# bystrogenomics/bystro-vcf

Hardware: AMD Instinct MI355X
Metric: variants/sec (higher is better)
Workload: dtype u8; 1 GPU; BASELINE configs[2]: 1KG-Phase3 chr1-shaped, 2504 samples, biallelic SNPs; rows_per_block=311296, resident_blocks_per_gpu=8, n_samples=2504, input=resident in HBM, blocks_in_flight=3, flags=default (--allowFilter PASS,.), class maps on

## Files before the change

### bystro-vcf_amd/__init__.py

```python
import ctypes as C
import os

import numpy as np

try:
    import torch
except ImportError:
    torch = None

_HERE = os.path.dirname(os.path.abspath(__file__))
LIB_PATH = os.environ.get("BVCF_LIB") or os.path.join(_HERE, "libbvcf.so")

if not os.path.exists(LIB_PATH):
    raise ImportError(
        "bystro-vcf_amd: %s not built (run `python -c 'import __graft_entry__ as g; g.build()'` "
        "or `make -C bystro-vcf_amd/csrc`); there is no fallback path" % LIB_PATH)

lib = C.CDLL(LIB_PATH)

ABI_VERSION = 9
DEVICE_PAD = 64
NO_CMAP = 0xFFFFFFFF

OK, E_ARG, E_HIP, E_NODEV, E_BUSY, E_EMPTY, E_TOO_BIG, E_CAPACITY, E_NOMEM, E_FATAL = 0, -1, -2, -3, -4, -5, -6, -7, -8, -9
LINE_OK, LINE_FIELDS, LINE_FILTER, LINE_NOALLELE = 0, 1, 2, 3
SITE_NAMES = ["SNP", "INS", "DEL", "MNP", "MULTIALLELIC"]
ALT_BASE, ALT_INS, ALT_DEL = 0, 1, 2
CLS_NONE, CLS_HET, CLS_HOM, CLS_MISSING = 0, 1, 2, 3
SAMPLE_STATS_COLUMNS = ["sample", "het", "hom", "missing", "transitions", "transversions", "heterozygosity", "homozygosity",
                        "missingness", "trTv"]

BENCH_EXPORTS = ["bvcf_bench_device", "bvcf_bench_device_slots", "bvcf_bench_stream_kernel"]

PLAN_EXPORTS = ["bvcf_plan_text_ranges", "bvcf_plan_bgzf_ranges", "bvcf_cut_text_range", "bvcf_find_bgzf_chain",
                "bvcf_plan_threads", "bvcf_plan_fd"]

EXPORTS = [
    "bvcf_create", "bvcf_destroy", "bvcf_last_error", "bvcf_version", "bvcf_reserve", "bvcf_set_sample_names", "bvcf_set_row_format", "bvcf_alloc_pinned", "bvcf_alloc_pinned_near", "bvcf_warmup",
    "bvcf_free_pinned", "bvcf_submit", "bvcf_submit_device", "bvcf_submit_bgzf", "bvcf_collect", "bvcf_sample_stats", "bvcf_counters", "bvcf_sum_counters",
    "bvcf_allreduce_counters", "bvcf_device_count", "bvcf_device_pci_bus_id", "bvcf_path", "bvcf_config_defaults", "bvcf_string_header", "bvcf_format_tsv", "bvcf_run_buffer", "bvcf_run_fd", "bvcf_decompress_fd", "bvcf_bgzf_inflate_device", "bvcf_bgzf_deflate_device", "bvcf_free",
    "bvcf_arrow_open", "bvcf_arrow_append", "bvcf_arrow_close",
]


class Params(C.Structure):
    _fields_ = [
        ("abi_version", C.c_uint32), ("device", C.c_int32), ("n_header_fields", C.c_uint32),
        ("eol_chars", C.c_uint32), ("eol_byte", C.c_uint8), ("want_class_maps", C.c_uint8),
        ("want_dosage", C.c_uint8), ("want_name_lists", C.c_uint8), ("allow_filter", C.c_char_p), ("exclude_filter", C.c_char_p),
        ("max_batch_bytes", C.c_uint64), ("max_lines", C.c_uint32), ("max_alleles", C.c_uint32),
        ("cmap_bytes", C.c_uint64), ("n_slots", C.c_uint32), ("path", C.c_uint32),
        ("packed_sites", C.c_uint32), ("render_sites", C.c_uint32), ("want_sample_stats", C.c_uint32),
        ("min_gq", C.c_uint32), ("min_dp", C.c_uint32),
    ]


class Config(C.Structure):
    _fields_ = [
        ("empty_field", C.c_char_p), ("field_delimiter", C.c_char_p), ("allow_filter", C.c_char_p),
        ("exclude_filter", C.c_char_p), ("keep_id", C.c_uint8), ("keep_info", C.c_uint8),
        ("keep_pos", C.c_uint8), ("keep_qual", C.c_uint8), ("normalize_header", C.c_uint8),
        ("leave_teardown_to_exit", C.c_uint8), ("reserved", C.c_uint8 * 2), ("device", C.c_int32), ("n_format_threads", C.c_uint32),
        ("max_batch_bytes", C.c_uint64), ("sample_list_path", C.c_char_p),
        ("dosage_path", C.c_char_p), ("no_out", C.c_uint8), ("out_bgzf", C.c_uint8), ("reserved3", C.c_uint8 * 2),
        ("n_devices", C.c_uint32), ("devices", C.POINTER(C.c_int32)), ("sample_stats_path", C.c_char_p),
        ("min_gq", C.c_uint32), ("min_dp", C.c_uint32),
    ]


class Result(C.Structure):
    _fields_ = [
        ("batch_seq", C.c_uint64), ("status", C.c_int32), ("n_lines", C.c_uint32), ("n_alleles", C.c_uint32),
        ("n_errs", C.c_uint32), ("n_cmap_bytes", C.c_uint64), ("cmap_stride", C.c_uint32),
        ("n_samples", C.c_uint32), ("lines", C.c_void_p), ("alleles", C.c_void_p), ("errs", C.c_void_p),
        ("cmap", C.c_void_p), ("need_lines", C.c_uint64), ("need_alleles", C.c_uint64),
        ("need_cmap_bytes", C.c_uint64), ("kernel_ms", C.c_float), ("reserved", C.c_uint32),
        ("n_lines_seen", C.c_uint64), ("dosage", C.c_void_p), ("dosage_stride", C.c_uint32), ("reserved2", C.c_uint32),
        ("name_lists", C.c_void_p), ("names", C.c_void_p), ("n_name_bytes", C.c_uint64),
        ("text", C.c_void_p), ("n_text_bytes", C.c_uint64), ("head_off", C.c_void_p),
        ("sites", C.c_void_p), ("n_full_lines", C.c_uint32), ("n_row_cuts", C.c_uint32),
        ("rows", C.c_void_p), ("n_row_bytes", C.c_uint64), ("row_cuts", C.c_void_p), ("n_ok_sites", C.c_uint64),
    ]


ROW_CUT_DTYPE = np.dtype([("line", "<u4"), ("slot", "<u4"), ("off", "<u8"), ("text_off", "<u4"), ("reserved", "<u4")])
NO_TEXT_OFF = 0xFFFFFFFF
LINE_DTYPE = np.dtype([
    ("off", "<u4"), ("len", "<u4"), ("fend", "<u4", (9,)), ("rec_first", "<u4"), ("n_rec", "<u4"),
    ("n_fields", "<u4"), ("gt_task", "<u4"), ("status", "u1"), ("site_type", "u1"), ("pad", "u1", (2,))])
ALLELE_DTYPE = np.dtype([
    ("pos", "<i8"), ("line", "<u4"), ("alt_idx", "<u4"), ("alt_off", "<u4"), ("alt_len", "<u4"), ("ac", "<u4"),
    ("an", "<u4"), ("n_het", "<u4"), ("n_hom", "<u4"), ("n_miss", "<u4"), ("cmap_off", "<u4"), ("ref", "u1"),
    ("alt_base", "u1"), ("kind", "u1"), ("site_type", "u1"), ("trtv", "u1"), ("flags", "u1"), ("pad", "u1", (2,)),
    ("gt_task", "<u4"), ("pad2", "<u4")])
ERR_DTYPE = np.dtype([("line", "<u4"), ("alt_no", "<u4"), ("code", "<u4"), ("pad", "<u4")])
SITE_DTYPE = np.dtype([("off", "<u4"), ("len", "<u4"), ("fend", "u1", (8,)), ("ref", "u1"), ("alt_base", "u1"), ("trtv", "u1"),
                       ("status", "u1"), ("full_idx", "<u4"), ("n_fields", "<u4"), ("reserved", "<u4")])
SITE_FULL = 0x80
NAMES_DTYPE = np.dtype([("off", "<u4", (3,)), ("len", "<u4", (3,))])
assert LINE_DTYPE.itemsize == 64 and ALLELE_DTYPE.itemsize == 64 and ERR_DTYPE.itemsize == 16 and SITE_DTYPE.itemsize == 32

lib.bvcf_create.argtypes = [C.POINTER(C.c_void_p), C.POINTER(Params)]
lib.bvcf_create.restype = C.c_int
lib.bvcf_destroy.argtypes = [C.c_void_p]
lib.bvcf_destroy.restype = None
lib.bvcf_last_error.argtypes = [C.c_void_p]
lib.bvcf_last_error.restype = C.c_char_p
lib.bvcf_version.restype = C.c_char_p
lib.bvcf_reserve.argtypes = [C.c_void_p, C.c_uint64, C.c_uint64, C.c_uint64]
lib.bvcf_set_sample_names.argtypes = [C.c_void_p, C.POINTER(C.c_char_p), C.POINTER(C.c_uint32), C.c_uint32, C.c_char_p]
lib.bvcf_alloc_pinned.argtypes = [C.c_size_t]
lib.bvcf_alloc_pinned.restype = C.c_void_p
lib.bvcf_free_pinned.argtypes = [C.c_void_p]
lib.bvcf_submit.argtypes = [C.c_void_p, C.c_void_p, C.c_size_t, C.c_uint64]
lib.bvcf_submit_device.argtypes = [C.c_void_p, C.c_void_p, C.c_size_t, C.c_uint64]
lib.bvcf_submit_bgzf.argtypes = [C.c_void_p, C.c_char_p, C.c_size_t, C.c_size_t, C.c_int, C.c_uint32, C.c_uint64]
lib.bvcf_collect.argtypes = [C.c_void_p, C.POINTER(Result)]
lib.bvcf_bench_device.argtypes = [C.c_void_p, C.POINTER(C.c_void_p), C.POINTER(C.c_size_t), C.c_int, C.c_int,
                                  C.POINTER(C.c_float), C.POINTER(C.c_float), C.POINTER(C.c_uint64)]
lib.bvcf_bench_device_slots.argtypes = [C.c_void_p, C.POINTER(C.c_void_p), C.POINTER(C.c_size_t), C.c_int, C.c_int,
                                        C.c_uint32, C.POINTER(C.c_float), C.POINTER(C.c_float), C.POINTER(C.c_uint64)]
lib.bvcf_counters.argtypes = [C.c_void_p, C.POINTER(C.c_uint64)]
lib.bvcf_path.argtypes = [C.c_void_p]
lib.bvcf_sum_counters.argtypes = [C.POINTER(C.c_void_p), C.c_int, C.POINTER(C.c_uint64)]
lib.bvcf_allreduce_counters.argtypes = [C.POINTER(C.c_void_p), C.c_int, C.POINTER(C.c_uint64), C.POINTER(C.c_int)]
lib.bvcf_device_count.restype = C.c_int
lib.bvcf_config_defaults.argtypes = [C.POINTER(Config)]
lib.bvcf_config_defaults.restype = None
lib.bvcf_string_header.argtypes = [C.POINTER(Config), C.c_char_p, C.c_size_t]
lib.bvcf_string_header.restype = C.c_size_t
lib.bvcf_format_tsv.argtypes = [C.POINTER(Config), C.POINTER(Result), C.c_void_p, C.POINTER(C.c_char_p),
                                C.POINTER(C.c_uint32), C.POINTER(C.c_void_p), C.POINTER(C.c_size_t),
                                C.POINTER(C.c_void_p), C.POINTER(C.c_size_t)]
lib.bvcf_run_buffer.argtypes = [C.POINTER(Config), C.c_char_p, C.c_size_t, C.POINTER(C.c_void_p),
                                C.POINTER(C.c_size_t), C.POINTER(C.c_void_p), C.POINTER(C.c_size_t),
                                C.POINTER(C.c_uint64)]
lib.bvcf_run_fd.argtypes = [C.POINTER(Config), C.c_int, C.c_int, C.c_int, C.POINTER(C.c_uint64)]
lib.bvcf_decompress_fd.argtypes = [C.c_int, C.c_int, C.c_uint32, C.c_char_p]
lib.bvcf_free.argtypes = [C.c_void_p]
lib.bvcf_free.restype = None


class RangePlan(C.Structure):
    _fields_ = [("data_off", C.c_uint64), ("range_bytes", C.c_uint64), ("spare_bytes", C.c_uint64), ("n_ranges", C.c_uint64)]


class TextCut(C.Structure):
    _fields_ = [("kind", C.c_int32), ("reserved", C.c_uint32), ("start", C.c_uint64), ("end", C.c_uint64), ("long_start", C.c_uint64)]


class ThreadBudget(C.Structure):
    _fields_ = [("readers", C.c_uint32), ("copy_threads", C.c_uint32), ("format_threads", C.c_uint32), ("busy_total", C.c_uint32)]


class PlanBlock(C.Structure):
    _fields_ = [("worker", C.c_uint32), ("piece", C.c_uint32), ("range", C.c_uint64), ("file_off", C.c_uint64),
                ("nbytes", C.c_uint64), ("own", C.c_uint64), ("first_off", C.c_uint32), ("bgzf", C.c_uint8),
                ("bgzf_flags", C.c_uint8), ("last_piece", C.c_uint8), ("reserved", C.c_uint8)]


CUT_LINES, CUT_NONE, CUT_LONG = 0, 1, 2
MODE_STREAM, MODE_TEXT_RANGES, MODE_BGZF_RANGES = 0, 1, 2
BGZF_SKIP_FIRST_LINE, BGZF_END_OF_STREAM = 1, 2
lib.bvcf_plan_text_ranges.argtypes = [C.c_uint64, C.c_uint64, C.c_uint64, C.c_uint64, C.POINTER(RangePlan)]
lib.bvcf_plan_bgzf_ranges.argtypes = [C.c_uint64, C.c_uint64, C.c_uint32, C.c_uint64, C.POINTER(RangePlan)]
lib.bvcf_cut_text_range.argtypes = [C.c_char_p, C.c_uint64, C.c_uint64, C.c_int, C.c_int, C.c_uint8, C.POINTER(TextCut)]
lib.bvcf_find_bgzf_chain.argtypes = [C.c_char_p, C.c_size_t, C.c_size_t]
lib.bvcf_find_bgzf_chain.restype = C.c_long
lib.bvcf_plan_threads.argtypes = [C.c_uint32, C.c_uint32, C.c_int, C.POINTER(ThreadBudget)]
lib.bvcf_plan_fd.argtypes = [C.c_int, C.c_int, C.c_uint32, C.c_uint64, C.c_int, C.POINTER(PlanBlock), C.c_size_t,
                             C.POINTER(C.c_size_t), C.POINTER(C.c_int), C.POINTER(RangePlan)]


def plan_fd(fd_in, n_workers, max_batch_bytes=0, device_inflate=1, fd_err=2, cap=1 << 16):
    out = (PlanBlock * cap)()
    n = C.c_size_t(0)
    mode = C.c_int(-1)
    plan = RangePlan()
    rc = lib.bvcf_plan_fd(fd_in, fd_err, n_workers, max_batch_bytes, device_inflate, out, cap, C.byref(n), C.byref(mode), C.byref(plan))
    assert n.value <= cap, "more blocks than room"
    return rc, mode.value, plan, [out[i] for i in range(n.value)]


class BvcfError(RuntimeError):
    def __init__(self, rc, msg):
        super().__init__("bvcf error %d: %s" % (rc, msg))
        self.rc = rc


def make_config(cfg=None, device=0, max_batch_bytes=0, n_format_threads=0):
    cfg = cfg or {}
    c = Config()
    lib.bvcf_config_defaults(C.byref(c))
    keep = [cfg.get("emptyField", "!").encode(), cfg.get("fieldDelimiter", ";").encode(),
            cfg.get("allow", "PASS,.").encode(), cfg.get("exclude", "").encode()]
    c.empty_field, c.field_delimiter, c.allow_filter, c.exclude_filter = keep
    c.keep_id = int(cfg.get("keepId", False))
    c.keep_info = int(cfg.get("keepInfo", False))
    c.keep_pos = int(cfg.get("keepPos", False))
    c.normalize_header = int(cfg.get("normalizeHeader", True))
    c.device = device
    c.max_batch_bytes = max_batch_bytes
    c.n_format_threads = n_format_threads
    if cfg.get("sample"):
        keep.append(cfg["sample"].encode())
        c.sample_list_path = keep[-1]
    if cfg.get("dosageOutput"):
        keep.append(str(cfg["dosageOutput"]).encode())
        c.dosage_path = keep[-1]
    c.no_out = int(cfg.get("noOut", False))
    c.out_bgzf = int(cfg.get("compressOutput", "none") == "bgzf")
    if cfg.get("devices"):
        arr = (C.c_int32 * len(cfg["devices"]))(*cfg["devices"])
        keep.append(arr)
        c.devices = arr
        c.n_devices = len(cfg["devices"])
    if cfg.get("sampleStats"):
        keep.append(str(cfg["sampleStats"]).encode())
        c.sample_stats_path = keep[-1]
    c.min_gq = int(cfg.get("minGQ", 0))
    c.min_dp = int(cfg.get("minDP", 0))
    c._keep = keep
    return c


def string_header(cfg=None):
    c = make_config(cfg)
    buf = C.create_string_buffer(512)
    n = lib.bvcf_string_header(C.byref(c), buf, len(buf))
    return buf.raw[:n].decode()


def run_buffer(vcf_bytes, cfg=None, device=0, max_batch_bytes=0, n_format_threads=0):
    c = make_config(cfg, device, max_batch_bytes, n_format_threads)
    out, log = C.c_void_p(), C.c_void_p()
    n_out, n_log, n_lines = C.c_size_t(), C.c_size_t(), C.c_uint64()
    rc = lib.bvcf_run_buffer(C.byref(c), vcf_bytes, len(vcf_bytes), C.byref(out), C.byref(n_out), C.byref(log),
                             C.byref(n_log), C.byref(n_lines))
    o = C.string_at(out, n_out.value) if out.value else b""
    e = C.string_at(log, n_log.value).decode(errors="replace") if log.value else ""
    lib.bvcf_free(out)
    lib.bvcf_free(log)
    return rc, o, e, n_lines.value


def run_fd(fd_in, fd_out, fd_err, cfg=None, device=0, max_batch_bytes=0):
    c = make_config(cfg, device, max_batch_bytes)
    n_lines = C.c_uint64()
    rc = lib.bvcf_run_fd(C.byref(c), fd_in, fd_out, fd_err, C.byref(n_lines))
    return rc, n_lines.value


def allreduce_counters(ctxs):
    arr = (C.c_void_p * len(ctxs))(*[x.h for x in ctxs])
    out = (C.c_uint64 * 8)()
    used = C.c_int(0)
    rc = lib.bvcf_allreduce_counters(arr, len(ctxs), out, C.byref(used))
    if rc:
        raise BvcfError(rc, lib.bvcf_last_error(ctxs[0].h).decode())
    return list(out), bool(used.value)


lib.bvcf_bgzf_inflate_device.argtypes = [C.c_int, C.c_char_p, C.c_size_t, C.c_void_p, C.c_size_t, C.POINTER(C.c_size_t)]


def bgzf_inflate_device(comp, cap=None, device=0):
    cap = cap if cap is not None else max(64, 66000 * (comp.count(b"\x1f\x8b\x08\x04") + 1))
    buf = C.create_string_buffer(cap)
    n = C.c_size_t()
    rc = lib.bvcf_bgzf_inflate_device(device, comp, len(comp), buf, cap, C.byref(n))
    return rc, (buf.raw[:n.value] if rc == 0 else b""), n.value


lib.bvcf_bgzf_deflate_device.argtypes = [C.c_int, C.c_char_p, C.c_size_t, C.c_int, C.c_void_p, C.c_size_t,
                                         C.POINTER(C.c_size_t)]
PIECE = 65280
BGZF_EOF = bytes.fromhex("1f8b08040000000000ff0600424302001b0003000000000000000000")


def bgzf_bound(n):
    return (n + PIECE - 1) // PIECE * 65311 + 28


def bgzf_deflate_device(data, add_eof=True, device=0):
    data = bytes(data)
    cap = bgzf_bound(len(data))
    buf = C.create_string_buffer(cap)
    n = C.c_size_t()
    rc = lib.bvcf_bgzf_deflate_device(device, data, len(data), int(bool(add_eof)), buf, cap, C.byref(n))
    if rc:
        raise BvcfError(rc, "bvcf_bgzf_deflate_device")
    return buf.raw[:n.value]


def decompress(data, n_threads=0):
    import tempfile
    with tempfile.TemporaryFile() as fi, tempfile.TemporaryFile() as fo:
        fi.write(data)
        fi.flush()
        fi.seek(0)
        kind = C.create_string_buffer(8)
        rc = lib.bvcf_decompress_fd(fi.fileno(), fo.fileno(), n_threads, kind)
        fo.seek(0)
        return rc, fo.read(), kind.value.decode()


def decompress_pipe(data, n_threads=16, piece=0, seed=0):
    import random
    import tempfile
    import threading
    r, w = os.pipe()
    rng = random.Random(seed)

    def feed():
        try:
            mv, off = memoryview(data), 0
            while off < len(mv):
                n = piece or rng.choice([1, 7, 4096, 65536, 100_000, 1 << 20, 3 << 20])
                off += os.write(w, mv[off:off + n])
        finally:
            os.close(w)

    t = threading.Thread(target=feed)
    t.start()
    try:
        with tempfile.TemporaryFile() as fo:
            kind = C.create_string_buffer(8)
            rc = lib.bvcf_decompress_fd(r, fo.fileno(), n_threads, kind)
            fo.seek(0)
            return rc, fo.read(), kind.value.decode()
    finally:
        os.close(r)
        t.join()

# ... 91 lines not shown
        L = self.lines[i]
        n = int(L["n_rec"])
        return [] if n == 0 else [i] + [int(L["rec_first"]) + j - 1 for j in range(1, n)]

    def line_head(self, i):
        L = self.lines[i]
        if self.head_off is None:
            return self.text[int(L["off"]):int(L["off"]) + int(L["len"])]
        n = min(int(L["fend"][7]), int(L["len"]))
        return self.text[int(self.head_off[i]):int(self.head_off[i]) + n]

    def name_list(self, slot, q):
        nl = self.name_lists[slot]
        return self.names[int(nl["off"][q]):int(nl["off"][q]) + int(nl["len"][q])]

    def classes(self, allele_row):
        off = int(allele_row["cmap_off"])
        ns = self.n_samples
        if int(allele_row["flags"]) & 2:
            words = self.cmap[off:off + 64].view("<u4")
            m = np.zeros((ns + 3) // 4, dtype=np.uint8)
            for e in words[1:1 + int(words[0])]:
                m[int(e) >> 8] = int(e) & 0xFF
        else:
            m = self.cmap[off:off + (ns + 3) // 4]
        return ((m[:, None] >> np.array([0, 2, 4, 6], dtype=np.uint8)) & 3).reshape(-1)[:ns]


class Ctx:

    def __init__(self, n_header_fields, allow="PASS,.", exclude="", device=0, eol_chars=1, eol_byte=b"\n",
                 max_batch_bytes=0, max_lines=0, max_alleles=0, cmap_bytes=0, n_slots=0, want_class_maps=True,
                 path=0, want_dosage=False, sample_names=None, delimiter=";", packed_sites=False, render_sites=False,
                 empty_field="!", keep_pos=False, keep_id=False, keep_info=False, sample_stats=False,
                 min_gq=0, min_dp=0):
        p = Params()
        p.abi_version = ABI_VERSION
        p.device = device
        p.n_header_fields = n_header_fields
        p.eol_chars = eol_chars
        p.eol_byte = eol_byte[0]
        p.want_class_maps = int(want_class_maps)
        p.want_dosage = int(want_dosage)
        self._keep = [allow.encode(), exclude.encode()]
        p.allow_filter, p.exclude_filter = self._keep
        p.max_batch_bytes = max_batch_bytes
        p.max_lines = max_lines
        p.max_alleles = max_alleles
        p.cmap_bytes = cmap_bytes
        p.n_slots = n_slots
        p.path = path
        p.packed_sites = int(packed_sites or render_sites)
        p.render_sites = int(render_sites)
        p.want_name_lists = int(sample_names is not None)
        p.want_sample_stats = int(sample_stats)
        p.min_gq = min_gq
        p.min_dp = min_dp
        self.n_samples = max(n_header_fields - 9, 0)
        self.h = C.c_void_p()
        rc = lib.bvcf_create(C.byref(self.h), C.byref(p))
        if rc:
            raise BvcfError(rc, lib.bvcf_last_error(None).decode())
        if render_sites:
            lib.bvcf_set_row_format.argtypes = [C.c_void_p, C.c_char_p, C.c_int, C.c_int, C.c_int]
            self._check(lib.bvcf_set_row_format(self.h, empty_field.encode(), int(keep_pos), int(keep_id), int(keep_info)))
        if sample_names is not None:
            enc = [x.encode() if isinstance(x, str) else x for x in sample_names]
            ptrs = (C.c_char_p * max(len(enc), 1))(*enc)
            lens = (C.c_uint32 * max(len(enc), 1))(*[len(x) for x in enc])
            self._check(lib.bvcf_set_sample_names(self.h, ptrs, lens, len(enc), delimiter.encode()))

    def close(self):
        if self.h:
            lib.bvcf_destroy(self.h)
            self.h = C.c_void_p()

    def __del__(self):
        try:
            self.close()
        except Exception:
            pass

    def _check(self, rc):
        if rc:
            raise BvcfError(rc, lib.bvcf_last_error(self.h).decode())

    def submit(self, block, seq=0):
        self._blk = block
        self._check(lib.bvcf_submit(self.h, block, len(block), seq))

    def submit_bgzf(self, comp, n_own, skip_first_line, first_off=0, seq=0):
        self._blk = comp
        self._check(lib.bvcf_submit_bgzf(self.h, comp, len(comp), n_own, int(skip_first_line), first_off, seq))

    def submit_device(self, dptr, nbytes, seq=0):
        self._check(lib.bvcf_submit_device(self.h, dptr, nbytes, seq))

    def reserve(self, lines, alleles, cmap_bytes):
        self._check(lib.bvcf_reserve(self.h, lines, alleles, cmap_bytes))

    def collect(self, tsv=None):
        r = Result()
        rc = lib.bvcf_collect(self.h, C.byref(r))
        if rc == E_CAPACITY:
            raise BvcfError(rc, "capacity: need lines=%d alleles=%d cmap=%d" % (r.need_lines, r.need_alleles, r.need_cmap_bytes))
        self._check(rc)
        if tsv is None:
            return Batch(r)
        block, cfg, names = tsv
        c = cfg if isinstance(cfg, Config) else make_config(cfg)
        buf = np.frombuffer(block, dtype=np.uint8)
        enc = [x.encode() if isinstance(x, str) else x for x in (names or [])]
        ptrs = (C.c_char_p * max(len(enc), 1))(*enc)
        lens = (C.c_uint32 * max(len(enc), 1))(*[len(x) for x in enc])
        out, log = C.c_void_p(), C.c_void_p()
        n_out, n_log = C.c_size_t(), C.c_size_t()
        rc = lib.bvcf_format_tsv(C.byref(c), C.byref(r), buf.ctypes.data if len(buf) else None, ptrs, lens, C.byref(out),
                                 C.byref(n_out), C.byref(log), C.byref(n_log))
        try:
            if rc:
                raise BvcfError(rc, "bvcf_format_tsv")
            text = C.string_at(out, n_out.value) if out.value else b""
            log_text = C.string_at(log, n_log.value).decode(errors="replace") if log.value else ""
        finally:
            lib.bvcf_free(out)
            lib.bvcf_free(log)
        b = Batch(r)
        b.tsv, b.log = text, log_text
        return b

    def process(self, block):
        self.submit(block)
        return self.collect()

    def bench_device(self, dptrs, nbytes, iters, slots=0):
        n = len(dptrs)
        ptrs = (C.c_void_p * n)(*dptrs)
        sizes = (C.c_size_t * n)(*nbytes)
        chain = (C.c_float * iters)()
        scan = (C.c_float * iters)()
        counts = (C.c_uint64 * 5)()
        self._check(lib.bvcf_bench_device_slots(self.h, ptrs, sizes, n, iters, slots, chain, scan, counts))
        return list(chain), list(scan), list(counts)

    def path(self):
        return lib.bvcf_path(self.h)

    def stream_kernel(self):
        lib.bvcf_bench_stream_kernel.argtypes = [C.c_void_p]
        lib.bvcf_bench_stream_kernel.restype = C.c_int
        k = lib.bvcf_bench_stream_kernel(self.h)
        return None if k < 0 else ("k_stream_gen" if k else "k_stream")

    def sample_stats(self, reset=False):
        out = np.zeros(6 * self.n_samples, dtype=np.uint64)
        lib.bvcf_sample_stats.argtypes = [C.c_void_p, C.c_void_p, C.c_int]
        self._check(lib.bvcf_sample_stats(self.h, out.ctypes.data if self.n_samples else None, int(reset)))
        return out.reshape(6, self.n_samples).T.copy()

    def counters(self):
        out = (C.c_uint64 * 8)()
        self._check(lib.bvcf_counters(self.h, out))
        return list(out)
```

### bystro-vcf_amd/csrc/bvcf_common.hip.h

```cpp
#pragma once

#include <hip/hip_runtime.h>
#include <stdint.h>

#include "../../include/bvcf.h"

namespace bvcf_dev {


constexpr int kWave = 64;
constexpr int kWavesPerWg = 4;
constexpr int kWgThreads = kWave * kWavesPerWg;
constexpr uint32_t kChunk = 1024;
constexpr uint32_t kMaxProducerWaves = 32768;
constexpr uint32_t kScanGroup = 1024;

typedef uint32_t u32x4 __attribute__((ext_vector_type(4)));
typedef u32x4 u32x4_u __attribute__((aligned(1)));

struct FilterTable {
  uint32_t allow_nil, allow_n;
  uint32_t deny_nil, deny_n;
  uint16_t allow_off[32], allow_len[32];
  uint16_t deny_off[32], deny_len[32];
  uint8_t text[2048];
};

struct BatchCounters {
  uint32_t n_lines;
  uint32_t n_alleles;
  uint32_t n_errs;
  uint32_t n_tasks;
  uint32_t lines_seen;
  uint32_t cmap_maps;
  uint32_t pad[2];
  uint32_t n_finish;
  uint32_t n_full;
  uint32_t n_real;
  uint32_t n_other_shape;
};

struct StreamEntry {
  uint32_t ls, len;
  uint32_t ac, an, n_het, n_hom, n_miss;
  uint32_t cmap_off;
};

struct GtTask {
  uint32_t line;
  uint32_t allele;
  uint32_t s_begin;
  uint32_t cend;
  uint32_t cmap_off;
  uint32_t pad[3];
};

struct GtResult {
  uint32_t ac, an, n_het, n_hom, n_miss;
  uint32_t n_fields;
  uint32_t regular;
  uint32_t pad;
};

struct KernelArgs {
  const uint8_t *buf;
  uint32_t nbytes;
  uint32_t cap;
  uint32_t n_header;
  uint32_t n_samples;
  uint32_t eol_chars;
  uint32_t eol_byte;
  uint32_t want_cmap;
  int8_t *dosage;
  uint32_t dosage_stride;
  uint32_t cmap_stride;
  uint32_t max_lines, max_alleles, max_errs, max_tasks;
  unsigned long long max_cmap;
  const FilterTable *filters;
  uint32_t *census;
  uint32_t *group_base;
  uint32_t *run_lines;
  uint32_t prod_waves;
  uint32_t *s2_groups;
  uint32_t *s2_groups_next;
  uint32_t *line_off;
  bvcf_line *lines;
  bvcf_allele *alleles;
  bvcf_site *sites;
  bvcf_err *errs;
  uint8_t *cmap;
  GtTask *tasks;
  GtResult *results;
  BatchCounters *counters;
  uint32_t fused;
  uint32_t gen_stream;
  uint32_t wide;
  uint32_t win_bytes;
  uint32_t win_tabs_cap;
  uint32_t *win_tabs;
  uint32_t tile_bytes;
  uint32_t tile_quota;
  uint32_t n_tiles;
  StreamEntry *entries;
  uint32_t *line_len;
  uint32_t *line_cmap;
  uint16_t *head_bits;
  uint32_t *line_bits;
  uint32_t *finish_items;
  uint32_t *real_tasks;
  uint32_t s1_fmode;
  uint32_t s1_fkey[4], s1_flen[4];
};
constexpr uint32_t kHasHeadBits = 0x80000000u;
constexpr uint32_t kNotRegular = 0x40000000u;


__device__ __forceinline__ int lane_id() { return threadIdx.x & (kWave - 1); }

__device__ __forceinline__ uint32_t wave_incl_scan(uint32_t v) {
  v += (uint32_t)__builtin_amdgcn_update_dpp(0, (int)v, 0x111, 0xF, 0xF, true);
  v += (uint32_t)__builtin_amdgcn_update_dpp(0, (int)v, 0x112, 0xF, 0xF, true);
  v += (uint32_t)__builtin_amdgcn_update_dpp(0, (int)v, 0x114, 0xF, 0xF, true);
  v += (uint32_t)__builtin_amdgcn_update_dpp(0, (int)v, 0x118, 0xF, 0xF, true);
  v += (uint32_t)__builtin_amdgcn_update_dpp(0, (int)v, 0x142, 0xA, 0xF, false);
  v += (uint32_t)__builtin_amdgcn_update_dpp(0, (int)v, 0x143, 0xC, 0xF, false);
  return v;
}

__device__ __forceinline__ uint32_t wave_incl_scan_max(uint32_t v) {
  v = max(v, (uint32_t)__builtin_amdgcn_update_dpp(0, (int)v, 0x111, 0xF, 0xF, true));
  v = max(v, (uint32_t)__builtin_amdgcn_update_dpp(0, (int)v, 0x112, 0xF, 0xF, true));
  v = max(v, (uint32_t)__builtin_amdgcn_update_dpp(0, (int)v, 0x114, 0xF, 0xF, true));
  v = max(v, (uint32_t)__builtin_amdgcn_update_dpp(0, (int)v, 0x118, 0xF, 0xF, true));
  v = max(v, (uint32_t)__builtin_amdgcn_update_dpp(0, (int)v, 0x142, 0xA, 0xF, false));
  v = max(v, (uint32_t)__builtin_amdgcn_update_dpp(0, (int)v, 0x143, 0xC, 0xF, false));
  return v;
}

__device__ __forceinline__ uint32_t lane_value(uint32_t v, int src) {
  return (uint32_t)__builtin_amdgcn_readlane((int)v, src);
}

__device__ __forceinline__ uint32_t wave_sum(uint32_t v) { return lane_value(wave_incl_scan(v), kWave - 1); }

__device__ __forceinline__ void wave_sum3(uint32_t a, uint32_t b, uint32_t c, uint32_t limit, uint32_t *sa,
                                          uint32_t *sb, uint32_t *sc) {
  if (limit < 65536u) {
    const uint32_t ab = wave_sum(a | (b << 16));
    *sa = ab & 0xFFFFu;
    *sb = ab >> 16;
  } else {
    *sa = wave_sum(a);
    *sb = wave_sum(b);
  }
  *sc = wave_sum(c);
}

__device__ __forceinline__ uint32_t wave_excl_scan(uint32_t v, uint32_t *total) {
  const uint32_t inc = wave_incl_scan(v);
  *total = lane_value(inc, kWave - 1);
  return inc - v;
}

__device__ __forceinline__ uint32_t bcast0(uint32_t v) { return (uint32_t)__builtin_amdgcn_readfirstlane((int)v); }

__device__ __forceinline__ uint32_t wave_in_wg() { return bcast0(threadIdx.x >> 6); }
__device__ __forceinline__ uint32_t wave_in_grid() { return blockIdx.x * kWavesPerWg + wave_in_wg(); }

__device__ __forceinline__ u32x4 load16(const uint8_t *buf, uint32_t off, uint32_t cap) {
  u32x4 v = {0u, 0u, 0u, 0u};
  if (off + 16u <= cap) v = *reinterpret_cast<const u32x4_u *>(buf + off);
  return v;
}

__device__ __forceinline__ u32x4 ld_stream(const uint8_t *p) {
  return __builtin_nontemporal_load(reinterpret_cast<const u32x4_u *>(p));
}

__device__ __forceinline__ u32x4 realign(u32x4 v, uint32_t next0, uint32_t r) {
  const uint32_t w4 = (uint32_t)__builtin_amdgcn_update_dpp((int)next0, (int)v.x, 0x130, 0xF, 0xF, false);
  u32x4 o;
  o.x = __builtin_amdgcn_alignbyte(v.y, v.x, r);
  o.y = __builtin_amdgcn_alignbyte(v.z, v.y, r);
  o.z = __builtin_amdgcn_alignbyte(v.w, v.z, r);
  o.w = __builtin_amdgcn_alignbyte(w4, v.w, r);
  return o;
}

__device__ __forceinline__ uint32_t zero_bytes(uint32_t x) {
  uint32_t t = (x & 0x7F7F7F7Fu) + 0x7F7F7F7Fu;
  return ~(t | x | 0x7F7F7F7Fu);
}

__device__ __forceinline__ uint32_t eq_mask4(uint32_t d, uint32_t c4) {
  uint32_t z = zero_bytes(d ^ c4) >> 7;
  return ((z * 0x00204081u) >> 21) & 0xFu;
}

__device__ __forceinline__ uint32_t eq_mask16(u32x4 v, uint32_t c) {
  const uint32_t c4 = c * 0x01010101u;
  uint32_t lo = __builtin_amdgcn_udot4(zero_bytes(v.x ^ c4), 0x08040201u, 0u, false);
  lo = __builtin_amdgcn_udot4(zero_bytes(v.y ^ c4), 0x80402010u, lo, false);
  uint32_t hi = __builtin_amdgcn_udot4(zero_bytes(v.z ^ c4), 0x08040201u, 0u, false);
  hi = __builtin_amdgcn_udot4(zero_bytes(v.w ^ c4), 0x80402010u, hi, false);
  return (lo >> 7) | (hi << 1);
}

__device__ __forceinline__ uint32_t bits_until(uint32_t end, uint32_t off) {
  const uint32_t n = min(end - min(end, off), 16u);
  return (1u << n) - 1u;
}


__device__ __forceinline__ uint32_t cmap_of(const KernelArgs &a, uint32_t mi, bool want) {
  return (want && ((unsigned long long)mi + 1ull) * a.cmap_stride <= a.max_cmap) ? mi * a.cmap_stride : BVCF_NO_CMAP;
}

}
```

### bystro-vcf_amd/csrc/bvcf_core.hip

```cpp
#include "bvcf_device.hip.h"
#include "../../include/bvcf_bench.h"
#include "bvcf_bgzf.h"
#include "bvcf_bgzf_out.h"

#include <dlfcn.h>
#include <rccl/rccl.h>
#include <stdio.h>
#include <stdlib.h>
#include <string.h>

#include <algorithm>
#include <mutex>
#include <string>
#include <thread>
#include <vector>

using namespace bvcf_dev;

namespace {

struct Slot {
  hipStream_t stream = nullptr;
  bool used_gen = false;
  hipEvent_t ev_k0 = nullptr, ev_k1 = nullptr, ev_ctr = nullptr;
  hipEvent_t ev_in = nullptr, ev_scan = nullptr;
  uint8_t *d_in = nullptr;
  uint32_t *d_census = nullptr, *d_group = nullptr, *d_line_off = nullptr;
  uint32_t group_words = 0;
  uint32_t *d_s2_groups = nullptr;
  uint32_t s2_parity = 0;
  bvcf_line *d_lines = nullptr;
  bvcf_allele *d_alleles = nullptr;
  bvcf_site *d_sites = nullptr, *h_sites = nullptr;
  uint64_t hcap_recs = 0, hcap_errs = 0;
  uint8_t *d_rows = nullptr, *h_rows = nullptr;
  uint64_t cap_rows = 0;
  bvcf_row_cut *d_row_cuts = nullptr, *h_row_cuts = nullptr;
  uint32_t cap_row_cuts = 0, cap_render_groups = 0;
  uint64_t cap_host_cuts = 0;
  unsigned long long *d_rgroup_bytes = nullptr, *d_rtotals = nullptr, *h_rtotals = nullptr;
  unsigned long long *d_rgroup_ctext = nullptr;
  uint8_t *d_cut_text = nullptr;
  uint64_t cap_cut_text = 0;
  bool cut_text_on = false;
  uint32_t *d_rgroup_full = nullptr;
  bvcf_err *d_errs = nullptr;
  uint8_t *d_cmap = nullptr;
  int8_t *d_dosage = nullptr;
  GtTask *d_tasks = nullptr;
  GtResult *d_results = nullptr;
  uint32_t *d_win_tabs = nullptr;
  uint32_t win_tabs_cap = 0;
  StreamEntry *d_entries = nullptr;
  uint32_t *d_line_len = nullptr, *d_line_cmap = nullptr, *d_line_bits = nullptr, *d_finish_items = nullptr;
  uint16_t *d_head_bits = nullptr;
  bvcf_names *d_name_lists = nullptr, *h_name_lists = nullptr;
  uint32_t *d_name_tot = nullptr;
  uint8_t *d_names = nullptr;
  char *h_names = nullptr;
  unsigned long long *d_name_total = nullptr, *h_name_total = nullptr;
  uint64_t cap_names = 0;
  uint8_t *d_comp = nullptr;
  uint64_t cap_comp = 0;
  uint32_t *d_bgzf = nullptr, *h_bgzf = nullptr;
  uint64_t cap_bgzf_blocks = 0;
  uint32_t *d_cuts = nullptr, *h_cuts = nullptr;
  uint8_t *h_text = nullptr;
  uint64_t cap_h_text = 0;
  uint32_t *d_head_off = nullptr, *h_head_off = nullptr;
  uint8_t *d_heads = nullptr;
  unsigned long long *d_head_total = nullptr, *h_head_total = nullptr;
  uint64_t cap_head_lines = 0;
  bool heads = false;
  hipEvent_t ev_cut = nullptr;
  bool await_cuts = false;
  bool is_bgzf = false;
  int bgzf_rc = 0;
  const char *bgzf_err = nullptr;
  uint32_t text_start = 0, text_total = 0;
  BatchCounters *d_counters = nullptr;
  BatchCounters *h_counters = nullptr;
  bvcf_line *h_lines = nullptr;
  bvcf_allele *h_alleles = nullptr;
  bvcf_err *h_errs = nullptr;
  uint8_t *h_cmap = nullptr;
  int8_t *h_dosage = nullptr;
  uint2 *d_ss_dense = nullptr, *d_ss_sparse = nullptr;
  uint64_t cap_ss_list = 0;
  uint32_t *d_ss_ctr = nullptr, *d_ss_part = nullptr, *d_ss_sp = nullptr;
  unsigned long long *d_ss_acc = nullptr;
  uint64_t cap_lines = 0, cap_alleles = 0, cap_cmap = 0, cap_census = 0;
  bool busy = false;
  uint64_t seq = 0;
  size_t nbytes = 0;
  const uint8_t *src = nullptr;
};

}

struct bvcf_ctx {
  bvcf_params p{};
  int device = 0;
  int n_cu = 0;
  int gt_grid = 0, stream_grid = 0;
  int gt_filter_grid = 0;
  hipStream_t scan_stream = nullptr;
  uint32_t stream_lds_pad = 0;
  bool fused = false;
  bool gen_mode = false;
  uint32_t last_real = 0xFFFFFFFFu, last_finish = 0xFFFFFFFFu;
  bool shape_seen = false;
  int gen_policy = -1;
  uint32_t gen_grid = 0;
  bool wide = false;
  bool gt_filter = false;
  uint64_t avg_line_bytes = 0;
  bool names_on = false;
  uint32_t *d_name_off = nullptr;
  uint8_t *d_name_text = nullptr;
  NameTable name_table{};
  bool sites = false;
  bool sites1 = false;
  bool sites2 = false;
  bool packed = false;
  bool sites2_tile_census = true;
  uint32_t s2_groups_cap = 0;
  int sites_grid = 0, sites1_grid = 0;
  uint32_t win_bytes = 64u << 10;
  uint32_t tile_bytes = 0, tile_quota = 0;
  bool render = false, row_fmt_set = false;
  uint8_t *d_row_fmt = nullptr;
  uint32_t row_tail_len = 0, row_keep_pos = 0, row_keep_id = 0, row_keep_info = 0;
  uint32_t n_samples = 0;
  uint32_t cmap_stride = 0;
  uint32_t dosage_stride = 0;
  bool ss_on = false;
  uint32_t ss_ns_pad = 0, ss_max_runs = 0, ss_stripes = 0;
  uint64_t max_lines = 0, max_alleles = 0, max_cmap = 0;
  uint64_t need_extras = 0;
  FilterTable *d_filters = nullptr;
  uint32_t s1_fmode = 0, s1_fkey[4] = {0, 0, 0, 0}, s1_flen[4] = {0, 0, 0, 0};
  std::vector<Slot> slots;
  size_t head = 0, tail = 0, in_flight = 0;
  uint64_t totals[8] = {0, 0, 0, 0, 0, 0, 0, 0};
  std::string err;
};

namespace {

thread_local std::string g_create_err;
thread_local std::string *g_err_sink = nullptr;

constexpr uint64_t kMaxBlockBytes = 0xFFF00000ull;

#define HIP_TRY(ctx, expr)                                                               \
  do {                                                                                   \
    hipError_t e_ = (expr);                                                              \
    if (e_ != hipSuccess) {                                                              \
      *(g_err_sink ? g_err_sink : &(ctx)->err) = std::string(#expr) + ": " + hipGetErrorString(e_); \
      return BVCF_E_HIP;                                                                 \
    }                                                                                    \
  } while (0)

bool is_space(char c) { return c == ' ' || c == '\t' || c == '\n' || c == '\v' || c == '\f' || c == '\r'; }

int fill_filter(const char *text, bool star_is_nil, uint32_t *nil, uint32_t *n, uint16_t *off, uint16_t *len,
                uint8_t *pool, uint32_t *pool_used) {
  *nil = 1;
  *n = 0;
  if (!text || !*text) return 0;
  if (star_is_nil && strcmp(text, "*") == 0) return 0;
  *nil = 0;
  size_t L = strlen(text), start = 0;
  for (size_t i = 0; i <= L; i++) {
    if (i != L && text[i] != ',') continue;
    size_t a = start, e = i;
    while (a < e && is_space(text[a])) a++;
    while (e > a && is_space(text[e - 1])) e--;
    if (*n >= 32 || *pool_used + (e - a) > 2048) return -1;
    off[*n] = (uint16_t)*pool_used;
    len[*n] = (uint16_t)(e - a);
    memcpy(pool + *pool_used, text + a, e - a);
    *pool_used += (uint32_t)(e - a);
    (*n)++;
    start = i + 1;
  }
  return 0;
}

void free_slot(Slot &s) {
  if (s.stream) hipStreamSynchronize(s.stream);
  hipFree(s.d_in);
  hipFree(s.d_census);
  hipFree(s.d_group);
  hipFree(s.d_s2_groups);
  hipFree(s.d_line_off);
  hipFree(s.d_lines);
  hipFree(s.d_alleles);
  hipFree(s.d_sites);
  hipHostFree(s.h_sites);
  hipFree(s.d_rows);
  hipHostFree(s.h_rows);
  hipFree(s.d_row_cuts);
  hipHostFree(s.h_row_cuts);
  hipFree(s.d_rgroup_bytes);
  hipFree(s.d_rgroup_full);
  hipFree(s.d_rgroup_ctext);
  hipFree(s.d_cut_text);
  hipFree(s.d_rtotals);
  hipHostFree(s.h_rtotals);
  hipFree(s.d_errs);
  hipFree(s.d_cmap);
  hipFree(s.d_dosage);
  hipFree(s.d_tasks);
  hipFree(s.d_results);
  hipFree(s.d_win_tabs);
  hipFree(s.d_entries);
  hipFree(s.d_line_len);
  hipFree(s.d_line_cmap);
  hipFree(s.d_line_bits);
  hipFree(s.d_finish_items);
  hipFree(s.d_head_bits);
  hipFree(s.d_name_lists);
  hipFree(s.d_name_tot);
  hipFree(s.d_names);
  hipFree(s.d_name_total);
  hipHostFree(s.h_name_lists);
  hipHostFree(s.h_names);
  hipHostFree(s.h_name_total);
  hipFree(s.d_comp);
  hipFree(s.d_bgzf);
  hipHostFree(s.h_bgzf);
  hipFree(s.d_cuts);
  hipHostFree(s.h_cuts);
  hipHostFree(s.h_text);
  hipFree(s.d_head_off);
  hipHostFree(s.h_head_off);
  hipFree(s.d_heads);
  hipFree(s.d_head_total);
  hipHostFree(s.h_head_total);
  if (s.ev_cut) hipEventDestroy(s.ev_cut);
  hipFree(s.d_counters);
  hipHostFree(s.h_counters);
  hipHostFree(s.h_lines);
  hipHostFree(s.h_alleles);
  hipHostFree(s.h_errs);
  hipHostFree(s.h_cmap);
  hipHostFree(s.h_dosage);
  hipFree(s.d_ss_dense);
  hipFree(s.d_ss_sparse);
  hipFree(s.d_ss_ctr);
  hipFree(s.d_ss_part);
  hipFree(s.d_ss_sp);
  hipFree(s.d_ss_acc);
  if (s.ev_k0) hipEventDestroy(s.ev_k0);
  if (s.ev_k1) hipEventDestroy(s.ev_k1);
  if (s.ev_in) hipEventDestroy(s.ev_in);
  if (s.ev_scan) hipEventDestroy(s.ev_scan);
  if (s.ev_ctr) hipEventDestroy(s.ev_ctr);
  if (s.stream) hipStreamDestroy(s.stream);
  s = Slot{};
}

int alloc_name_arena(bvcf_ctx *c, Slot &s, uint64_t want_bytes) {
  if (want_bytes <= s.cap_names) return BVCF_OK;
  hipFree(s.d_names);
  hipHostFree(s.h_names);
  s.d_names = nullptr;
  s.h_names = nullptr;
  s.cap_names = 0;
  HIP_TRY(c, hipMalloc(&s.d_names, want_bytes + 64));
  HIP_TRY(c, hipHostMalloc(&s.h_names, want_bytes + 64, hipHostMallocDefault));
  s.cap_names = want_bytes;
  return BVCF_OK;
}

int alloc_names(bvcf_ctx *c, Slot &s, uint64_t want_bytes) {
  if (!c->names_on) return BVCF_OK;
  hipFree(s.d_name_lists);
  hipFree(s.d_name_tot);
  hipHostFree(s.h_name_lists);
  s.d_name_lists = nullptr;
  s.d_name_tot = nullptr;
  s.h_name_lists = nullptr;
  HIP_TRY(c, hipMalloc(&s.d_name_lists, c->max_alleles * sizeof(bvcf_names)));
  HIP_TRY(c, hipMalloc(&s.d_name_tot, (c->max_alleles + 1) * sizeof(uint32_t)));
  HIP_TRY(c, hipHostMalloc(&s.h_name_lists, c->max_alleles * sizeof(bvcf_names), hipHostMallocDefault));
  if (!s.d_name_total) {
    HIP_TRY(c, hipMalloc(&s.d_name_total, sizeof(unsigned long long)));
    HIP_TRY(c, hipHostMalloc(&s.h_name_total, sizeof(unsigned long long), hipHostMallocDefault));
  }
  return alloc_name_arena(c, s, want_bytes);
}

NameArgs make_name_args(bvcf_ctx *c, Slot &s) {
  NameArgs na{};
  na.nt = c->name_table;
  na.lists = s.d_name_lists;
  na.tot = s.d_name_tot;
  na.out = s.d_names;
  na.cap = s.cap_names;
  na.total = s.d_name_total;
  return na;
}

int alloc_results(bvcf_ctx *c, Slot &s) {
  if (s.cap_lines == c->max_lines && s.cap_alleles == c->max_alleles && s.cap_cmap == c->max_cmap) return BVCF_OK;
  hipFree(s.d_line_off);
  hipFree(s.d_lines);
  hipFree(s.d_alleles);
  hipFree(s.d_sites);
  hipHostFree(s.h_sites);
  s.d_sites = nullptr;
  s.h_sites = nullptr;
  hipFree(s.d_errs);
  hipFree(s.d_cmap);
  hipFree(s.d_dosage);
  hipFree(s.d_tasks);
  hipFree(s.d_results);
  hipFree(s.d_win_tabs);
  s.d_win_tabs = nullptr;
  hipFree(s.d_line_len);
  hipFree(s.d_line_cmap);
  hipFree(s.d_line_bits);
  hipFree(s.d_finish_items);
  s.d_line_bits = nullptr;
  s.d_finish_items = nullptr;
  hipHostFree(s.h_lines);
  hipHostFree(s.h_alleles);
  hipHostFree(s.h_errs);
  hipHostFree(s.h_cmap);
  hipHostFree(s.h_dosage);
  s.d_dosage = nullptr;
  s.h_dosage = nullptr;
  s.d_line_off = nullptr;
  s.d_lines = nullptr;
  s.d_alleles = nullptr;
  s.d_errs = nullptr;
  s.d_cmap = nullptr;
  s.d_tasks = nullptr;
  s.d_results = nullptr;
  s.d_line_len = nullptr;
  s.d_line_cmap = nullptr;
  s.h_lines = nullptr;
  s.h_alleles = nullptr;
  s.h_errs = nullptr;
  s.h_cmap = nullptr;
  s.cap_lines = s.cap_alleles = s.cap_cmap = 0;
  HIP_TRY(c, hipMalloc(&s.d_line_off, (c->max_lines + 1) * sizeof(uint32_t)));
  HIP_TRY(c, hipMalloc(&s.d_lines, c->max_lines * sizeof(bvcf_line)));
  HIP_TRY(c, hipMalloc(&s.d_alleles, c->max_alleles * sizeof(bvcf_allele)));
  if (c->packed) {
    HIP_TRY(c, hipMalloc(&s.d_sites, (c->max_lines + 64) * sizeof(bvcf_site)));
    if (!c->render)
      HIP_TRY(c, hipHostMalloc(&s.h_sites, (c->max_lines + 64) * sizeof(bvcf_site), hipHostMallocDefault));
  }
  HIP_TRY(c, hipMalloc(&s.d_errs, c->max_alleles * sizeof(bvcf_err)));
  HIP_TRY(c, hipMalloc(&s.d_cmap, c->max_cmap + 64));
  HIP_TRY(c, hipMalloc(&s.d_tasks, c->max_alleles * sizeof(GtTask)));
  HIP_TRY(c, hipMalloc(&s.d_results, c->max_alleles * sizeof(GtResult)));
  if (c->wide) {
    s.win_tabs_cap = (uint32_t)std::min<uint64_t>(2 * (c->p.max_batch_bytes / c->win_bytes) + c->max_lines + 64, 0x7FFFFFFFu);
    HIP_TRY(c, hipMalloc(&s.d_win_tabs, (size_t)s.win_tabs_cap * sizeof(uint32_t)));
  }
  HIP_TRY(c, hipMalloc(&s.d_line_len, c->max_lines * sizeof(uint32_t)));
  HIP_TRY(c, hipMalloc(&s.d_line_cmap, c->max_lines * sizeof(uint32_t)));
  if (c->fused) {
    HIP_TRY(c, hipMalloc(&s.d_line_bits, c->max_lines * 8 * sizeof(uint32_t)));
    HIP_TRY(c, hipMalloc(&s.d_finish_items, (c->max_lines + c->max_alleles) * sizeof(uint32_t)));
  }
  if (c->packed) {
    s.hcap_recs = std::max<uint64_t>(4096, c->max_lines / 16);
    s.hcap_errs = std::max<uint64_t>(4096, c->max_lines / 16);
    HIP_TRY(c, hipHostMalloc(&s.h_lines, s.hcap_recs * sizeof(bvcf_line), hipHostMallocDefault));
    HIP_TRY(c, hipHostMalloc(&s.h_alleles, 2 * s.hcap_recs * sizeof(bvcf_allele), hipHostMallocDefault));
    HIP_TRY(c, hipHostMalloc(&s.h_errs, s.hcap_errs * sizeof(bvcf_err), hipHostMallocDefault));
    HIP_TRY(c, hipHostMalloc(&s.h_cmap, 4096, hipHostMallocDefault));
  } else {
    s.hcap_recs = s.hcap_errs = 0;
    HIP_TRY(c, hipHostMalloc(&s.h_lines, c->max_lines * sizeof(bvcf_line), hipHostMallocDefault));
    HIP_TRY(c, hipHostMalloc(&s.h_alleles, c->max_alleles * sizeof(bvcf_allele), hipHostMallocDefault));
    HIP_TRY(c, hipHostMalloc(&s.h_errs, c->max_alleles * sizeof(bvcf_err), hipHostMallocDefault));
    HIP_TRY(c, hipHostMalloc(&s.h_cmap, c->max_cmap + 64, hipHostMallocDefault));
  }
  if (c->dosage_stride) {
    HIP_TRY(c, hipMalloc(&s.d_dosage, c->max_alleles * c->dosage_stride + 64));
    HIP_TRY(c, hipHostMalloc(&s.h_dosage, c->max_alleles * c->dosage_stride + 64, hipHostMallocDefault));
  }
  {
    const int rc = alloc_names(c, s, std::max<uint64_t>(s.cap_names, c->p.max_batch_bytes / 2 + (1u << 20)));
    if (rc) return rc;
  }
  if (c->ss_on) {
    hipFree(s.d_ss_dense);
    hipFree(s.d_ss_sparse);
    s.d_ss_dense = s.d_ss_sparse = nullptr;
    s.cap_ss_list = 0;
    HIP_TRY(c, hipMalloc(&s.d_ss_dense, c->max_alleles * sizeof(uint2)));
    HIP_TRY(c, hipMalloc(&s.d_ss_sparse, c->max_alleles * sizeof(uint2)));
    s.cap_ss_list = c->max_alleles;
  }
  s.cap_lines = c->max_lines;
  s.cap_alleles = c->max_alleles;
  s.cap_cmap = c->max_cmap;
  return BVCF_OK;
}

int alloc_slot(bvcf_ctx *c, Slot &s) {
  HIP_TRY(c, hipStreamCreateWithFlags(&s.stream, hipStreamNonBlocking));
  HIP_TRY(c, hipEventCreate(&s.ev_k0));
  HIP_TRY(c, hipEventCreate(&s.ev_k1));
  HIP_TRY(c, hipEventCreateWithFlags(&s.ev_in, hipEventDisableTiming));
  HIP_TRY(c, hipEventCreateWithFlags(&s.ev_scan, hipEventDisableTiming));
  HIP_TRY(c, hipEventCreate(&s.ev_ctr));
  const uint64_t in_cap = c->p.max_batch_bytes + BVCF_DEVICE_PAD;
  HIP_TRY(c, hipMalloc(&s.d_in, in_cap));
  s.cap_census = std::max<uint64_t>((c->p.max_batch_bytes + kChunk - 1) / kChunk + 1, s1_state_words((uint32_t)c->p.max_batch_bytes));
  {
    const uint32_t nt = s2_n_tiles((uint32_t)c->p.max_batch_bytes) + 1u;
    s.cap_census = std::max<uint64_t>(s.cap_census, (uint64_t)s2_bundle_off(nt) + s2_n_bundles(nt) + 64u);
    c->s2_groups_cap = s2_n_groups(nt) + 2u;
  }
  HIP_TRY(c, hipMalloc(&s.d_census, s.cap_census * sizeof(uint32_t)));
  s.group_words = ((uint32_t)(s.cap_census / kScanGroup) + 2u + 3u) & ~3u;
  HIP_TRY(c, hipMalloc(&s.d_group, ((size_t)s.group_words + kMaxProducerWaves) * sizeof(uint32_t)));
  HIP_TRY(c, hipMalloc(&s.d_s2_groups, 2ull * c->s2_groups_cap * sizeof(uint32_t)));
  HIP_TRY(c, hipMemset(s.d_s2_groups, 0, 2ull * c->s2_groups_cap * sizeof(uint32_t)));
  s.s2_parity = 0;
  HIP_TRY(c, hipMalloc(&s.d_counters, sizeof(BatchCounters)));
  HIP_TRY(c, hipHostMalloc(&s.h_counters, sizeof(BatchCounters), hipHostMallocDefault));
  if (c->fused) {
    const uint64_t max_tiles = (c->p.max_batch_bytes + c->tile_bytes - 1) / c->tile_bytes + 1;
    HIP_TRY(c, hipMalloc(&s.d_entries, max_tiles * c->tile_quota * sizeof(StreamEntry)));
    HIP_TRY(c, hipMalloc(&s.d_head_bits, max_tiles * c->tile_quota * 16 * sizeof(uint16_t)));
  }
  if (c->ss_on) {
    const size_t table = (size_t)kSsCols * c->ss_ns_pad;
    HIP_TRY(c, hipMalloc(&s.d_ss_ctr, 4 * sizeof(uint32_t)));
    HIP_TRY(c, hipMalloc(&s.d_ss_part, (size_t)c->ss_max_runs * table * sizeof(uint32_t)));
    HIP_TRY(c, hipMalloc(&s.d_ss_sp, table * sizeof(uint32_t)));
    HIP_TRY(c, hipMalloc(&s.d_ss_acc, 6ull * c->ss_ns_pad * sizeof(unsigned long long)));
    HIP_TRY(c, hipMemset(s.d_ss_acc, 0, 6ull * c->ss_ns_pad * sizeof(unsigned long long)));
  }
  return alloc_results(c, s);
}

KernelArgs make_args(bvcf_ctx *c, Slot &s, const uint8_t *d_src, size_t nbytes) {
  KernelArgs a{};
  a.buf = d_src;
  a.nbytes = (uint32_t)nbytes;
  a.cap = (uint32_t)(nbytes + BVCF_DEVICE_PAD);
  a.n_header = c->p.n_header_fields;
  a.n_samples = c->n_samples;
  a.eol_chars = c->p.eol_chars;
  a.eol_byte = c->p.eol_byte;
  a.want_cmap = c->p.want_class_maps || c->ss_on;
  a.cmap_stride = c->cmap_stride;
  a.max_lines = (uint32_t)c->max_lines;
  a.max_alleles = (uint32_t)c->max_alleles;
  a.max_errs = (uint32_t)c->max_alleles;
  a.max_tasks = (uint32_t)c->max_alleles;
  a.max_cmap = c->max_cmap;
  a.filters = c->d_filters;
  a.census = s.d_census;
  a.group_base = s.d_group;
  a.run_lines = s.d_group + s.group_words;
  a.s2_groups = s.d_s2_groups + (s.s2_parity & 1u) * c->s2_groups_cap;
  a.s2_groups_next = s.d_s2_groups + ((s.s2_parity & 1u) ^ 1u) * c->s2_groups_cap;
  a.line_off = s.d_line_off;
  a.lines = s.d_lines;
  a.alleles = s.d_alleles;
  a.sites = c->packed ? s.d_sites : nullptr;
  a.errs = s.d_errs;
  a.cmap = s.d_cmap;
  a.dosage = s.d_dosage;
  a.dosage_stride = c->dosage_stride;
  a.tasks = s.d_tasks;
  a.results = s.d_results;
  a.counters = s.d_counters;
  a.fused = c->fused ? 1u : 0u;
  a.gen_stream = c->gen_mode ? 1u : 0u;
  a.prod_waves = (uint32_t)(c->gen_mode ? c->gen_grid : c->stream_grid) * kWavesPerWg;
  a.wide = c->wide ? 1u : 0u;
  a.win_bytes = c->win_bytes;
  a.win_tabs = s.d_win_tabs;
  a.win_tabs_cap = s.d_win_tabs ? s.win_tabs_cap : 0u;
  a.tile_bytes = c->tile_bytes;
  a.tile_quota = c->tile_quota;
  a.n_tiles = c->fused ? (uint32_t)((nbytes + c->tile_bytes - 1) / c->tile_bytes) : 0u;
  a.entries = s.d_entries;
  a.line_len = s.d_line_len;
  a.line_cmap = s.d_line_cmap;
  a.head_bits = s.d_head_bits;
  a.line_bits = s.d_line_bits;
  a.finish_items = s.d_finish_items;
  a.real_tasks = s.d_finish_items ? s.d_finish_items + c->max_lines : nullptr;
  a.s1_fmode = c->s1_fmode;
  for (int i = 0; i < 4; i++) {
    a.s1_fkey[i] = c->s1_fkey[i];
    a.s1_flen[i] = c->s1_flen[i];
  }
  return a;
}

void launch_names(bvcf_ctx *c, const KernelArgs &a, const NameArgs &na, hipStream_t st) {
  hipLaunchKernelGGL(k_name_len, dim3(c->n_cu * 4), dim3(kWgThreads), 0, st, a, na);
  hipLaunchKernelGGL(k_name_scan, dim3(1), dim3(1024), 0, st, a, na);
  hipLaunchKernelGGL(k_name_write, dim3(c->n_cu * 4), dim3(kWgThreads), 0, st, a, na);
}

void adapt_stream_kernel(bvcf_ctx *c, bool was_gen, const BatchCounters &ctr) {
  c->last_real = ctr.n_real;
  c->last_finish = ctr.n_finish;
  if (c->gen_policy >= 0 || !c->fused || ctr.n_lines < 16) return;
  c->shape_seen = true;
  if ((uint64_t)ctr.n_other_shape * 2u > ctr.n_lines) c->gen_mode = !was_gen;
}

SampleStatsArgs make_ss_args(bvcf_ctx *c, Slot &s) {
  SampleStatsArgs sa{};
  sa.dense = s.d_ss_dense;
  sa.sparse = s.d_ss_sparse;
  sa.ctr = s.d_ss_ctr;
  sa.part = s.d_ss_part;
  sa.sp = s.d_ss_sp;
  sa.acc = s.d_ss_acc;
  sa.list_cap = (uint32_t)s.cap_ss_list;
  sa.ns_pad = c->ss_ns_pad;
  sa.max_runs = c->ss_max_runs;
  sa.n_stripes = c->ss_stripes;
  return sa;
}

void launch_sample_stats(bvcf_ctx *c, const KernelArgs &a, hipStream_t st, Slot *slot) {
  if (!c->ss_on || !slot || !slot->d_ss_dense) return;
  const SampleStatsArgs sa = make_ss_args(c, *slot);
  hipMemsetAsync(sa.ctr, 0, 4 * sizeof(uint32_t), st);
  hipMemsetAsync(sa.sp, 0, (size_t)kSsCols * sa.ns_pad * sizeof(uint32_t), st);
  hipLaunchKernelGGL(k_ss_list, dim3(c->n_cu * kSsListWgs), dim3(kWgThreads), 0, st, a, sa);
  const uint32_t waves = c->ss_stripes * c->ss_max_runs;
  hipLaunchKernelGGL(k_ss_dense, dim3((waves + kWavesPerWg - 1) / kWavesPerWg), dim3(kWgThreads), 0, st, a, sa);
  hipLaunchKernelGGL(k_ss_sparse, dim3(c->n_cu * 8), dim3(kWgThreads), 0, st, a, sa);
}

void launch_chain(bvcf_ctx *c, const KernelArgs &a, hipStream_t st, hipEvent_t ev_gt0, hipEvent_t ev_gt1, Slot *slot = nullptr) {
  if (a.fused) {
    const bool split = c->scan_stream && slot && slot->ev_in && slot->ev_scan;
    hipStream_t ss = split ? c->scan_stream : st;
    if (split) {
      hipEventRecord(slot->ev_in, st);
      hipStreamWaitEvent(ss, slot->ev_in, 0);
    }
    hipMemsetAsync(a.counters, 0, sizeof(BatchCounters), ss);
    if (ev_gt0) hipEventRecord(ev_gt0, ss);
    if (a.gen_stream)
      hipLaunchKernelGGL(k_stream_gen, dim3(c->gen_grid), dim3(kWgThreads), gen_lds_bytes(a.n_samples), ss, a);
    else
      hipLaunchKernelGGL(k_stream, dim3(c->stream_grid), dim3(kWgThreads), c->stream_lds_pad, ss, a);
    if (ev_gt1) hipEventRecord(ev_gt1, ss);
    if (split) {
      hipEventRecord(slot->ev_scan, ss);
      hipStreamWaitEvent(st, slot->ev_scan, 0);
    }
    hipLaunchKernelGGL(k_order, dim3(c->n_cu * 4), dim3(kWgThreads), 0, st, a);
#ifdef BVCF_EXPERIMENTS
    static const int skip = getenv("BVCF_EXP_SKIP") ? atoi(getenv("BVCF_EXP_SKIP")) : 0;
    static const int head_wgs = getenv("BVCF_EXP_HEAD_WGS") ? atoi(getenv("BVCF_EXP_HEAD_WGS")) : 4;
    static const int gt_div = getenv("BVCF_EXP_GT_DIV") ? atoi(getenv("BVCF_EXP_GT_DIV")) : 1;
#else
    constexpr int skip = 0, head_wgs = 4, gt_div = 1;
#endif
    if (skip & 1) {
    } else if (c->p.n_slots > 1)
      hipLaunchKernelGGL(k_head_lean, dim3(c->n_cu * head_wgs), dim3(kWgThreads), 0, st, a);
    else
      hipLaunchKernelGGL(k_head, dim3(c->n_cu * head_wgs), dim3(kWgThreads), 0, st, a);
    const uint32_t gt_full = (uint32_t)c->gt_grid / (uint32_t)gt_div;
    const uint32_t gt_wgs = c->last_real == 0xFFFFFFFFu ? gt_full
                            : std::min<uint32_t>(gt_full, std::max<uint32_t>((uint32_t)c->n_cu / 4u, c->last_real / (2u * kWavesPerWg) + 1u));
    const uint32_t fin_full = (uint32_t)c->n_cu * 4u;
    const uint32_t fin_wgs = c->last_finish == 0xFFFFFFFFu ? fin_full
                             : std::min<uint32_t>(fin_full, std::max<uint32_t>((uint32_t)c->n_cu / 4u, c->last_finish / kWgThreads + 1u));
    if (!(skip & 2)) hipLaunchKernelGGL(k_gt, dim3(gt_wgs), dim3(kWgThreads), 0, st, a);
    if (!(skip & 4)) hipLaunchKernelGGL(k_finish, dim3(fin_wgs), dim3(kWgThreads), 0, st, a);
    if (a.dosage) hipLaunchKernelGGL(k_dosage, dim3(c->gt_grid), dim3(kWgThreads), 0, st, a);
    launch_sample_stats(c, a, st, slot);
    return;
  }
#ifdef BVCF_EXPERIMENTS
  if (c->sites1) {
    const uint32_t n_words = s1_state_words(a.nbytes);
    hipLaunchKernelGGL(k_s1_zero, dim3(std::min<uint32_t>((n_words + 255u) / 256u, (uint32_t)c->n_cu)), dim3(256), 0, st, a, n_words);
    if (ev_gt0) hipEventRecord(ev_gt0, st);
    const uint32_t n_tiles = s1_n_tiles(a.nbytes);
    static const uint32_t stagger_us = [] {
      const char *e = getenv("BVCF_S1_STAGGER_US");
      return e ? (uint32_t)atoi(e) : 0u;
    }();
    if (n_tiles)
      hipLaunchKernelGGL(k_sites1, dim3(s1_n_wgs(n_tiles)), dim3(kS1Threads), 0, st, a, n_tiles, (uint32_t)c->sites1_grid, stagger_us * 100u);
    if (ev_gt1) hipEventRecord(ev_gt1, st);
    return;
  }
#endif
  const uint32_t n_chunks = (a.nbytes + kChunk - 1) / kChunk;
  const uint32_t n_groups = (n_chunks + kScanGroup - 1) / kScanGroup;
  const uint32_t stream_grid = (uint32_t)std::min<uint64_t>((n_chunks + kWavesPerWg - 1) / kWavesPerWg,
                                                            (uint64_t)c->n_cu * 8);
  if (c->sites2 && c->sites2_tile_census) {
    const uint32_t n_tiles = s2_n_tiles(a.nbytes);
    if (a.sites) {
      const uint32_t grid = s2_n_bundles(n_tiles);
      hipLaunchKernelGGL(k_census_tiles, dim3(grid ? grid : 1), dim3(kWgThreads), 0, st, a, n_tiles, c->s2_groups_cap);
    } else {
      const uint32_t grid = (uint32_t)std::min<uint64_t>((n_tiles + kWavesPerWg - 1) / kWavesPerWg, (uint64_t)c->n_cu * 8);
      hipLaunchKernelGGL(k_count_tiles, dim3(grid ? grid : 1), dim3(kWgThreads), 0, st, a, n_tiles);
      hipLaunchKernelGGL(k_scan_flat, dim3(1), dim3(1024), 0, st, a, n_tiles);
    }
    if (ev_gt0) hipEventRecord(ev_gt0, st);
    if (a.sites)
      hipLaunchKernelGGL(k_sites2p, dim3(c->sites1_grid), dim3(kS1Threads), 0, st, a, n_tiles, 0u);
    else
      hipLaunchKernelGGL(k_sites2, dim3(c->sites1_grid), dim3(kS1Threads), 0, st, a, n_tiles, 0u);
    if (ev_gt1) hipEventRecord(ev_gt1, st);
    return;
  }
  hipLaunchKernelGGL(k_count_eol, dim3(stream_grid ? stream_grid : 1), dim3(kWgThreads), 0, st, a, n_chunks);
  hipLaunchKernelGGL(k_scan_groups, dim3(n_groups ? n_groups : 1), dim3(kWgThreads), 0, st, a, n_chunks);
  hipLaunchKernelGGL(k_scan_top, dim3(1), dim3(1024), 0, st, a, n_groups);
  if (c->sites2) {
    if (ev_gt0) hipEventRecord(ev_gt0, st);
    if (a.sites)
      hipLaunchKernelGGL(k_sites2p, dim3(c->sites1_grid), dim3(kS1Threads), 0, st, a, s2_n_tiles(a.nbytes), n_chunks);
    else
      hipLaunchKernelGGL(k_sites2, dim3(c->sites1_grid), dim3(kS1Threads), 0, st, a, s2_n_tiles(a.nbytes), n_chunks);
    if (ev_gt1) hipEventRecord(ev_gt1, st);
    return;
  }
#ifdef BVCF_EXPERIMENTS
  if (c->sites) {
    if (ev_gt0) hipEventRecord(ev_gt0, st);
    hipLaunchKernelGGL(k_sites, dim3(c->sites_grid), dim3(kSitesThreads), 0, st, a, n_chunks);
    if (ev_gt1) hipEventRecord(ev_gt1, st);
    return;
  }
#endif
  hipLaunchKernelGGL(k_scatter_eol, dim3(stream_grid ? stream_grid : 1), dim3(kWgThreads), 0, st, a, n_chunks);
  if (c->p.n_slots > 1)
    hipLaunchKernelGGL(k_head_lean, dim3(c->n_cu * 4), dim3(kWgThreads), 0, st, a);
  else
    hipLaunchKernelGGL(k_head, dim3(c->n_cu * 4), dim3(kWgThreads), 0, st, a);
  if (a.n_samples) {
    if (ev_gt0) hipEventRecord(ev_gt0, st);
    if (c->gt_filter) {
      const GtFilterArgs fa = {c->p.min_gq, c->p.min_dp};
      hipLaunchKernelGGL(k_gt_filter, dim3(c->gt_filter_grid), dim3(kWgThreads), 0, st, a, fa);
      if (ev_gt1) hipEventRecord(ev_gt1, st);
      hipLaunchKernelGGL(k_finish, dim3(c->n_cu * 4), dim3(kWgThreads), 0, st, a);
      if (a.dosage) hipLaunchKernelGGL(k_dosage_filter, dim3(c->gt_filter_grid), dim3(kWgThreads), 0, st, a, fa);
      launch_sample_stats(c, a, st, slot);
      return;
    }
    if (c->wide) {
      hipMemsetAsync(a.results, 0, (size_t)a.max_tasks * sizeof(GtResult), st);
      hipLaunchKernelGGL(k_gt_wide, dim3(c->gt_grid), dim3(kWgThreads), 0, st, a);
      if (a.win_tabs) {
        hipLaunchKernelGGL(k_tabs_wide, dim3(c->gt_grid), dim3(kWgThreads), 0, st, a);
        hipLaunchKernelGGL(k_gt_wide_general, dim3(c->gt_grid), dim3(kWgThreads), 0, st, a);
      }
    }
    hipLaunchKernelGGL(k_gt, dim3(c->gt_grid), dim3(kWgThreads), 0, st, a);
    if (ev_gt1) hipEventRecord(ev_gt1, st);
    hipLaunchKernelGGL(k_finish, dim3(c->n_cu * 4), dim3(kWgThreads), 0, st, a);
    if (a.dosage) hipLaunchKernelGGL(k_dosage, dim3(c->gt_grid), dim3(kWgThreads), 0, st, a);
    if (a.dosage && c->wide && a.win_tabs) hipLaunchKernelGGL(k_dosage_wide, dim3(c->gt_grid), dim3(kWgThreads), 0, st, a);
    launch_sample_stats(c, a, st, slot);
  } else {
    if (ev_gt0) hipEventRecord(ev_gt0, st);
    if (ev_gt1) hipEventRecord(ev_gt1, st);
  }
}

static const CrcTabs *crc_tabs_on_device() {
  static std::mutex mu;
  static const CrcTabs *on_dev[64] = {};
  int dev = 0;
  if (hipGetDevice(&dev) != hipSuccess || dev < 0 || dev >= 64) return nullptr;
  std::lock_guard<std::mutex> lk(mu);
  if (on_dev[dev]) return on_dev[dev];
  auto mul = [](uint32_t a, uint32_t b) {
    uint32_t p = 0;
    for (int i = 31; i >= 0; i--) {
      if ((a >> i) & 1u) p ^= b;
      b = (b & 1u) ? (b >> 1) ^ 0xEDB88320u : b >> 1;
    }
    return p;
  };
  auto xpow = [&](uint64_t n) {
    uint32_t r = 0x80000000u, b = 0x40000000u;
    for (; n; n >>= 1) {
      if (n & 1u) r = mul(r, b);
      b = mul(b, b);
    }
    return r;
  };
  static CrcTabs t;
  for (uint32_t i = 0; i < 256; i++) {
    uint32_t c = i;
    for (int k = 0; k < 8; k++) c = (c >> 1) ^ (0xEDB88320u & (0u - (c & 1u)));
    t.std4[0][i] = c;
  }
  for (uint32_t i = 0; i < 256; i++) {
    uint32_t c = t.std4[0][i];
    for (int j = 1; j < 4; j++) {
      c = t.std4[0][c & 0xFFu] ^ (c >> 8);
      t.std4[j][i] = c;
    }
  }
  const uint32_t k1008 = xpow(8u * 1008u);
  for (int j = 0; j < 4; j++)
    for (uint32_t i = 0; i < 256; i++) t.jump[j][i] = mul(k1008, t.std4[j][i]);
  for (uint32_t L = 0; L < 64; L++) t.lane_k[L] = xpow(8u * 16u * (63u - L));
  CrcTabs *d = nullptr;
  if (hipMalloc(&d, sizeof t) != hipSuccess) return nullptr;
  if (hipMemcpy(d, &t, sizeof t, hipMemcpyHostToDevice) != hipSuccess) {
    hipFree(d);
    return nullptr;
  }
  on_dev[dev] = d;
// ... 319 lines not shown
  if (kernel_ms) *kernel_ms = 0;
  if (n > r->max_text) return BVCF_E_ARG;
  if (!n) return BVCF_OK;
  const uint32_t np = (uint32_t)((n + kPiece - 1) / kPiece);
  hipError_t e;
  auto hip_fail = [&](const char *what) {
    *err = std::string(what) + ": " + hipGetErrorString(e);
    return BVCF_E_HIP;
  };
  if ((e = hipSetDevice(r->device)) != hipSuccess) return hip_fail("hipSetDevice");
  if ((e = hipMemcpyAsync(r->d_text, text, n, hipMemcpyHostToDevice, r->st)) != hipSuccess) return hip_fail("text to the device");
  hipEventRecord(r->e0, r->st);
  const uint32_t grid = std::min<uint32_t>(np, (uint32_t)r->grid);
  hipLaunchKernelGGL(k_deflate, dim3(grid), dim3(kDefThreads), 0, r->st, (const uint8_t *)r->d_text, (uint64_t)n, np, r->d_scratch,
                     r->d_slots, r->d_info, r->d_desc);
  hipLaunchKernelGGL(k_crc32, dim3(std::min<uint32_t>(np, (uint32_t)r->n_cu * 16u)), dim3(kWave), 0, r->st, (const uint8_t *)r->d_text,
                     (const BgzfDesc *)r->d_desc, np, r->crc_tabs, r->d_crc);
  hipLaunchKernelGGL(k_bgzf_scan, dim3(1), dim3(kDefThreads), 0, r->st, (const uint32_t *)r->d_info, np, r->d_offs);
  hipLaunchKernelGGL(k_bgzf_pack, dim3(std::min<uint32_t>(np, (uint32_t)r->n_cu * 8u)), dim3(kDefThreads), 0, r->st,
                     (const uint8_t *)r->d_text, (uint64_t)n, np, (const uint8_t *)r->d_slots, (const uint32_t *)r->d_info,
                     (const uint32_t *)r->d_crc, (const uint64_t *)r->d_offs, r->d_out);
  hipEventRecord(r->e1, r->st);
  if ((e = hipGetLastError()) != hipSuccess) return hip_fail("compressor kernels");
  if ((e = hipMemcpyAsync(r->h_total, r->d_offs + np, sizeof(uint64_t), hipMemcpyDeviceToHost, r->st)) != hipSuccess ||
      (e = hipStreamSynchronize(r->st)) != hipSuccess)
    return hip_fail("compressor");
  const uint64_t total = *r->h_total;
  *n_out = (size_t)total;
  if (kernel_ms) {
    float ms = 0;
    hipEventElapsedTime(&ms, r->e0, r->e1);
    *kernel_ms = ms;
  }
  if (total > cap) return BVCF_E_TOO_BIG;
  if ((e = hipMemcpyAsync(out, r->d_out, total, hipMemcpyDeviceToHost, r->st)) != hipSuccess ||
      (e = hipStreamSynchronize(r->st)) != hipSuccess)
    return hip_fail("members to the host");
  return BVCF_OK;
}

}

extern "C" {

#ifdef BVCF_EXPERIMENTS
const char *bvcf_version(void) { return "bvcf-mi355x 0.1 (gfx950) +experiments"; }
#else
const char *bvcf_version(void) { return "bvcf-mi355x 0.1 (gfx950)"; }
#endif

const char *bvcf_last_error(const bvcf_ctx *ctx) { return ctx ? ctx->err.c_str() : g_create_err.c_str(); }

void *bvcf_alloc_pinned(size_t nbytes) {
  void *p = nullptr;
  if (hipHostMalloc(&p, nbytes ? nbytes : 1, hipHostMallocPortable) != hipSuccess) return nullptr;
  return p;
}

void *bvcf_alloc_pinned_near(int device, size_t nbytes) {
  int n_dev = 0, was = -1;
  if (hipGetDeviceCount(&n_dev) != hipSuccess || device < 0 || device >= n_dev) return nullptr;
  if (hipGetDevice(&was) != hipSuccess) was = -1;
  if (hipSetDevice(device) != hipSuccess) return nullptr;
  void *p = bvcf_alloc_pinned(nbytes);
  if (was >= 0 && was != device) hipSetDevice(was);
  return p;
}

int bvcf_device_pci_bus_id(int device, char *out, int cap) {
  if (!out || cap < 16) return BVCF_E_ARG;
  int n_dev = 0;
  if (hipGetDeviceCount(&n_dev) != hipSuccess || device < 0 || device >= n_dev) return BVCF_E_NODEV;
  return hipDeviceGetPCIBusId(out, cap, device) == hipSuccess ? BVCF_OK : BVCF_E_HIP;
}

__global__ void k_warm(uint32_t *p) {
  if (p) *p = 1u;
}

int bvcf_warmup(int device) {
  int n_dev = 0;
  if (hipGetDeviceCount(&n_dev) != hipSuccess || n_dev <= 0 || device < 0 || device >= n_dev) return BVCF_E_NODEV;
  if (hipSetDevice(device) != hipSuccess || hipFree(nullptr) != hipSuccess) return BVCF_E_HIP;
  int per_cu = 0;
  if (hipOccupancyMaxActiveBlocksPerMultiprocessor(&per_cu, k_finish, kWgThreads, 0) != hipSuccess) return BVCF_E_HIP;
  hipLaunchKernelGGL(k_warm, dim3(1), dim3(64), 0, 0, (uint32_t *)nullptr);
  return hipDeviceSynchronize() == hipSuccess ? BVCF_OK : BVCF_E_HIP;
}

void bvcf_free_pinned(void *p) {
  if (p) hipHostFree(p);
}

void bvcf_destroy(bvcf_ctx *c) {
  if (!c) return;
  hipSetDevice(c->device);
  for (auto &s : c->slots) free_slot(s);
  if (c->scan_stream) hipStreamDestroy(c->scan_stream);
  hipFree(c->d_filters);
  hipFree(c->d_row_fmt);
  hipFree(c->d_name_off);
  hipFree(c->d_name_text);
  delete c;
}

int bvcf_create(bvcf_ctx **out, const bvcf_params *p) {
  if (!out || !p) return BVCF_E_ARG;
  *out = nullptr;
  if (p->abi_version != BVCF_ABI_VERSION || p->n_header_fields < 1 || p->eol_chars < 1 || p->eol_chars > 2) {
    g_create_err = "bad bvcf_params";
    return BVCF_E_ARG;
  }
  if (p->min_gq > BVCF_MAX_THRESHOLD || p->min_dp > BVCF_MAX_THRESHOLD) {
    g_create_err = "bad bvcf_params: min_gq / min_dp above 999999999";
    return BVCF_E_ARG;
  }
  int n_dev = 0;
  if (hipGetDeviceCount(&n_dev) != hipSuccess || n_dev <= 0 || p->device < 0 || p->device >= n_dev) {
    g_create_err = "no usable HIP device (libbvcf has no CPU fallback)";
    return BVCF_E_NODEV;
  }
  bvcf_ctx *c = new bvcf_ctx();
  c->p = *p;
  c->device = p->device;
  if (!c->p.max_batch_bytes) c->p.max_batch_bytes = 64ull << 20;
  if (c->p.max_batch_bytes >= kMaxBlockBytes) c->p.max_batch_bytes = kMaxBlockBytes - 1;
  if (!c->p.n_slots) c->p.n_slots = 3;
  if (!c->p.eol_byte) c->p.eol_byte = '\n';
  c->n_samples = p->n_header_fields > 9 ? p->n_header_fields - 9 : 0;
  c->cmap_stride = ((c->n_samples + 3) / 4 + 15) & ~15u;
  c->dosage_stride = p->want_dosage && c->n_samples ? ((c->n_samples + 15) & ~15u) : 0u;
  const uint64_t min_line = std::max<uint64_t>(48, 2ull * p->n_header_fields);
  const uint64_t slack = std::min<uint64_t>(4096, std::max<uint64_t>(64, (32ull << 20) / std::max<uint32_t>(c->cmap_stride, 1u)));
  c->max_lines = p->max_lines ? p->max_lines : c->p.max_batch_bytes / min_line + slack;
  c->max_alleles = p->max_alleles ? p->max_alleles : 2 * c->max_lines + 1024;
  if (c->max_alleles < c->max_lines + 64) c->max_alleles = c->max_lines + 64;
  c->max_cmap = p->cmap_bytes ? p->cmap_bytes : (c->max_lines + c->max_lines / 2) * (uint64_t)c->cmap_stride + (1ull << 20);
  if (c->max_cmap > 0xFFFFFF00ull) c->max_cmap = 0xFFFFFF00ull;
  if (c->max_cmap < 4096) c->max_cmap = 4096;
  c->max_cmap = (c->max_cmap + 63) & ~63ull;
  c->tile_bytes = 64u << 10;
  if (const char *e = getenv("BVCF_TILE_KB")) {
    const unsigned kb = (unsigned)atoi(e);
    if (kb >= 4 && kb <= 1024) c->tile_bytes = kb << 10;
  }
  uint32_t path = p->path;
  if (const char *e = getenv("BVCF_PATH")) path = (uint32_t)atoi(e);
  c->gt_filter = c->n_samples > 0 && (p->min_gq != 0 || p->min_dp != 0);
  if (c->gt_filter) path = 1;
  const bool many_samples = c->n_samples >= kWideSamples;
  c->fused = c->n_samples > 0 && (path == 2 || path == 3 || (path == 0 && p->n_header_fields >= 256 && !many_samples));
  c->wide = !c->fused && many_samples;
  if (const char *e = getenv("BVCF_GEN_STREAM")) c->gen_policy = atoi(e) != 0 ? 1 : 0;
  if (!c->fused || c->n_samples > 4u * kStageBytes) c->gen_policy = 0;
  c->gen_mode = c->gen_policy == 1;
  if (path == 3 && c->gen_policy < 0) {
    c->gen_mode = true;
    c->shape_seen = true;
  }
  if (const char *e = getenv("BVCF_WIDE")) c->wide = !c->fused && c->n_samples > 0 && atoi(e) != 0;
  if (c->gt_filter) c->wide = false;
  if (const char *e = getenv("BVCF_WIDE_WIN")) {
    const long v = atol(e);
    if (v >= 64 && v <= (64l << 20)) c->win_bytes = (uint32_t)v;
  }
  c->tile_quota = c->tile_bytes / (p->n_header_fields - 1 + p->eol_chars) + 2;
  auto fail = [&](int rc) {
    g_create_err = c->err;
    bvcf_destroy(c);
    return rc;
  };
  if (hipSetDevice(c->device) != hipSuccess) {
    c->err = "hipSetDevice failed";
    return fail(BVCF_E_HIP);
  }
  hipDeviceProp_t prop;
  if (hipGetDeviceProperties(&prop, c->device) != hipSuccess) {
    c->err = "hipGetDeviceProperties failed";
    return fail(BVCF_E_HIP);
  }
  c->n_cu = prop.multiProcessorCount;
  int per_cu = 0;
  if (hipOccupancyMaxActiveBlocksPerMultiprocessor(&per_cu, k_gt, kWgThreads, 0) != hipSuccess || per_cu < 1)
    per_cu = 4;
  c->gt_grid = c->n_cu * per_cu;
  per_cu = 0;
  if (hipOccupancyMaxActiveBlocksPerMultiprocessor(&per_cu, k_gt_filter, kWgThreads, 0) != hipSuccess || per_cu < 1)
    per_cu = 4;
  c->gt_filter_grid = c->n_cu * per_cu;
  per_cu = 0;
  if (hipOccupancyMaxActiveBlocksPerMultiprocessor(&per_cu, k_stream, kWgThreads, 0) != hipSuccess || per_cu < 1)
    per_cu = 3;
  if (c->p.n_slots > 1 && per_cu > 2) per_cu = 2;
#ifdef BVCF_EXPERIMENTS
  if (const char *e = getenv("BVCF_STREAM_WGS")) {
    const int w = atoi(e);
    if (w >= 1 && w <= 4) per_cu = w;
  }
#endif
  c->stream_grid = c->n_cu * per_cu;
#ifdef BVCF_EXPERIMENTS
  if (c->p.n_slots > 1 && getenv("BVCF_SCAN_STREAM") && atoi(getenv("BVCF_SCAN_STREAM")) == 1 &&
      hipStreamCreateWithFlags(&c->scan_stream, hipStreamNonBlocking) != hipSuccess) {
    c->err = "hipStreamCreate failed";
    return fail(BVCF_E_HIP);
  }
  if (const char *e = getenv("BVCF_EXP_STREAM_LDS")) c->stream_lds_pad = (uint32_t)atoi(e);
#endif
  per_cu = 0;
  if (hipOccupancyMaxActiveBlocksPerMultiprocessor(&per_cu, k_stream_gen, kWgThreads, gen_lds_bytes(c->n_samples)) != hipSuccess || per_cu < 1)
    per_cu = 2;
  per_cu = std::min(per_cu, 6);
#ifdef BVCF_EXPERIMENTS
  if (const char *e = getenv("BVCF_GEN_WGS")) {
    const int w = atoi(e);
    if (w >= 1 && w <= 8) per_cu = std::min(per_cu, w);
  }
#endif
  c->gen_grid = c->n_cu * per_cu;
  c->sites = c->n_samples == 0;
  c->sites2 = c->sites;
  if (const char *e = getenv("BVCF_SITES")) {
    const int m = atoi(e);
#ifdef BVCF_EXPERIMENTS
    c->sites = c->sites && m != 0;
    c->sites2 = c->sites && m == 2;
    c->sites1 = c->sites && m == 3;
#else
    c->sites = c->sites2 = c->sites && m != 0;
#endif
  }
  if (const char *e = getenv("BVCF_S2_CENSUS")) c->sites2_tile_census = strcmp(e, "chunk") != 0;
  c->packed = c->sites2 && p->packed_sites != 0;
  c->render = c->packed && p->render_sites != 0;
  per_cu = 0;
#ifdef BVCF_EXPERIMENTS
  if (hipOccupancyMaxActiveBlocksPerMultiprocessor(&per_cu, k_sites, kSitesThreads, 0) != hipSuccess || per_cu < 1)
    per_cu = 3;
  c->sites_grid = c->n_cu * per_cu;
  per_cu = 0;
#endif
  if (hipOccupancyMaxActiveBlocksPerMultiprocessor(&per_cu, k_sites2, kS1Threads, 0) != hipSuccess || per_cu < 1)
    per_cu = 2;
#ifdef BVCF_EXPERIMENTS
  if (const char *e = getenv("BVCF_SITES1_WGS")) {
    const int w = atoi(e);
    if (w >= 1 && w <= 8) per_cu = std::min(per_cu, w);
  }
  if (const char *e = getenv("BVCF_S2_WGS")) {
    const int w = atoi(e);
    if (w >= 1 && w <= 4) per_cu = std::min(per_cu, w);
  }
#endif
  c->sites1_grid = c->n_cu * per_cu;
  c->ss_on = p->want_sample_stats != 0 && c->n_samples > 0;
  if (c->ss_on) {
    c->ss_ns_pad = 4u * c->cmap_stride;
    c->ss_stripes = (c->ss_ns_pad + kSsStripeSamples - 1u) / kSsStripeSamples;
    c->ss_max_runs = (uint32_t)std::min<uint64_t>(4096, std::max<uint64_t>(1, (16ull << 20) / (4ull * kSsCols * c->ss_ns_pad)));
  }
  if (!p->cmap_bytes) {
    c->max_cmap += (uint64_t)c->stream_grid * kWavesPerWg * 2u * c->cmap_stride + c->max_lines / 16 * (uint64_t)c->cmap_stride;
    c->max_cmap = std::min<uint64_t>((c->max_cmap + 63) & ~63ull, 0xFFFFFF00ull);
  }

  FilterTable ft;
  memset(&ft, 0, sizeof ft);
  uint32_t used = 0;
  if (fill_filter(p->allow_filter, true, &ft.allow_nil, &ft.allow_n, ft.allow_off, ft.allow_len, ft.text, &used) ||
      fill_filter(p->exclude_filter, false, &ft.deny_nil, &ft.deny_n, ft.deny_off, ft.deny_len, ft.text, &used)) {
    c->err = "too many / too long FILTER values (32 values, 2048 bytes)";
    return fail(BVCF_E_ARG);
  }
  if (ft.deny_nil) {
    if (ft.allow_nil) {
      c->s1_fmode = 2;
    } else if (ft.allow_n <= 4) {
      c->s1_fmode = 1;
      for (uint32_t i = 0; i < ft.allow_n; i++) {
        const uint32_t l = ft.allow_len[i];
        if (l == 0 || l > 4) {
          c->s1_fmode = 0;
          break;
        }
        uint32_t k = 0;
        for (uint32_t q = 0; q < l; q++) k |= (uint32_t)ft.text[ft.allow_off[i] + q] << (8 * q);
        c->s1_fkey[i] = k;
        c->s1_flen[i] = l;
      }
      if (!c->s1_fmode)
        for (int i = 0; i < 4; i++) c->s1_flen[i] = 0;
    }
  }
  if (hipMalloc(&c->d_filters, sizeof ft) != hipSuccess ||
      hipMemcpy(c->d_filters, &ft, sizeof ft, hipMemcpyHostToDevice) != hipSuccess) {
    c->err = "filter table upload failed";
    return fail(BVCF_E_HIP);
  }
  c->slots.resize(c->p.n_slots);
  {
    std::vector<int> rcs(c->slots.size(), BVCF_OK);
    std::vector<std::string> errs(c->slots.size());
    std::vector<std::thread> th;
    for (size_t i = 1; i < c->slots.size(); i++)
      th.emplace_back([c, i, &rcs, &errs]() {
        g_err_sink = &errs[i];
// ... 486 lines not shown
    if (text_bytes > s.cap_h_text) {
      hipHostFree(s.h_text);
      s.h_text = nullptr;
      s.cap_h_text = 0;
      const uint64_t want = c->p.max_batch_bytes + BVCF_DEVICE_PAD;
      if (hipHostMalloc(&s.h_text, want, hipHostMallocDefault) != hipSuccess) {
        s.h_text = nullptr;
        c->err = "hipHostMalloc failed (text copy of a BGZF batch)";
        release();
        return BVCF_E_NOMEM;
      }
      s.cap_h_text = want;
    }
    HIP_TRY(c, hipMemcpyAsync(s.h_text, s.src, s.nbytes, hipMemcpyDeviceToHost, s.stream));
  }
  const bool names = c->names_on && s.d_name_lists;
  uint64_t name_bytes = 0;
  if (names && n_alleles) {
    name_bytes = *s.h_name_total;
    if (name_bytes >= 0xFFFFFFF0ull) {
      c->err = "the sample-name lists of one batch pass 4 GiB: submit smaller blocks";
      release();
      return BVCF_E_TOO_BIG;
    }
    if (name_bytes > s.cap_names) {
      const int rc = alloc_name_arena(c, s, name_bytes + name_bytes / 4 + (1u << 20));
      if (rc) {
        release();
        return rc;
      }
      KernelArgs a = make_args(c, s, s.src, s.nbytes);
      hipLaunchKernelGGL(k_name_write, dim3(c->n_cu * 4), dim3(kWgThreads), 0, s.stream, a, make_name_args(c, s));
    }
    HIP_TRY(c, hipMemcpyAsync(s.h_name_lists, s.d_name_lists, n_alleles * sizeof(bvcf_names), hipMemcpyDeviceToHost, s.stream));
    if (name_bytes) HIP_TRY(c, hipMemcpyAsync(s.h_names, s.d_names, name_bytes, hipMemcpyDeviceToHost, s.stream));
  }
  e = hipStreamSynchronize(s.stream);
  if (e != hipSuccess) {
    c->err = std::string("result copy failed: ") + hipGetErrorString(e);
    release();
    return BVCF_E_HIP;
  }
  auto verdict_of = [&](uint32_t i) -> uint32_t {
    if (!c->packed) return s.h_lines[i].status;
    if (c->render) {
      const bvcf_row_cut *lo = s.h_row_cuts, *hi = s.h_row_cuts + n_row_cuts;
      const bvcf_row_cut *it = std::lower_bound(lo, hi, i, [](const bvcf_row_cut &q, uint32_t v) { return q.line < v; });
      if (it == hi || it->line != i || it->slot >= n_first) return (uint32_t)BVCF_LINE_FIELDS;
      return s.h_lines[it->slot].status;
    }
    const bvcf_site &st = s.h_sites[i];
    if (!(st.status & BVCF_SITE_FULL)) return st.status;
    return st.full_idx < n_first ? s.h_lines[st.full_idx].status : (uint32_t)BVCF_LINE_FIELDS;
  };
  if (c->packed)
    for (uint32_t j = 0; j < n_first; j++)
      if (s.h_lines[j].rec_first >= extras_at) s.h_lines[j].rec_first = s.h_lines[j].rec_first - (uint32_t)extras_at + n_first;
  uint32_t n_errs = 0;
  for (uint32_t i = 0; i < ctr.n_errs; i++) {
    const bvcf_err &er = s.h_errs[i];
    if (er.line < ctr.n_lines && verdict_of(er.line) != BVCF_LINE_FIELDS) s.h_errs[n_errs++] = er;
  }
  r->status = BVCF_OK;
  r->n_lines = ctr.n_lines;
  r->n_alleles = c->packed ? n_first + ctr.n_alleles : (uint32_t)n_alleles;
  r->n_errs = n_errs;
  r->n_cmap_bytes = cmap_bytes;
  r->n_lines_seen = ctr.lines_seen;
  r->lines = s.h_lines;
  r->alleles = s.h_alleles;
  r->errs = s.h_errs;
  r->cmap = (c->ss_on && !c->p.want_class_maps) ? nullptr : s.h_cmap;
  r->dosage = c->dosage_stride ? s.h_dosage : nullptr;
  r->dosage_stride = c->dosage_stride;
  r->text = was_bgzf ? s.h_text : nullptr;
  r->n_text_bytes = was_bgzf ? text_bytes : 0;
  r->head_off = (was_bgzf && s.heads) ? s.h_head_off : nullptr;
  r->sites = (c->packed && !c->render) ? s.h_sites : nullptr;
  r->n_full_lines = c->packed ? n_first : 0u;
  r->rows = c->render ? s.h_rows : nullptr;
  r->n_row_bytes = row_bytes;
  r->row_cuts = c->render ? s.h_row_cuts : nullptr;
  r->n_row_cuts = (uint32_t)n_row_cuts;
  r->n_ok_sites = n_ok_sites;
  r->name_lists = names ? s.h_name_lists : nullptr;
  r->names = names ? s.h_names : nullptr;
  r->n_name_bytes = name_bytes;

  uint64_t ok = 0, ac0 = 0, recs = 0;
  if (c->render) {
    ok += n_ok_sites;
    recs += n_ok_sites;
  } else if (c->packed)
    for (uint32_t i = 0; i < ctr.n_lines; i++) {
      const bvcf_site &st = s.h_sites[i];
      if (!(st.status & BVCF_SITE_FULL)) {
        ok += st.status == BVCF_LINE_OK;
        recs += st.status == BVCF_LINE_OK;
      }
    }
  for (uint32_t i = 0; i < n_first; i++) {
    const bvcf_line &L = s.h_lines[i];
    if (L.status != BVCF_LINE_OK) continue;
    ok++;
    recs += L.n_rec;
    if (c->n_samples)
      for (uint32_t j = 0; j < L.n_rec; j++) ac0 += s.h_alleles[j ? L.rec_first + j - 1 : i].ac == 0;
  }
  if (ctr.lines_seen) c->avg_line_bytes = s.nbytes / ctr.lines_seen;
  c->totals[0] += ctr.lines_seen;
  c->totals[1] += ok;
  c->totals[2] += recs;
  c->totals[3] += ac0;
  c->totals[4] += n_errs;
  c->totals[5] += s.nbytes;
  c->totals[6] += r->n_cmap_bytes;
  c->totals[7] += (uint64_t)(ms * 1e6);
  release();
  return BVCF_OK;
}

int bvcf_sample_stats(bvcf_ctx *c, uint64_t *out, int reset) {
  if (!c) return BVCF_E_ARG;
  if (!c->p.want_sample_stats) {
    c->err = "bvcf_sample_stats: the ctx was created without bvcf_params.want_sample_stats";
    return BVCF_E_ARG;
  }
  const uint32_t ns = c->n_samples;
  if (out) memset(out, 0, 6ull * ns * sizeof(uint64_t));
  if (!c->ss_on) return BVCF_OK;
  HIP_TRY(c, hipSetDevice(c->device));
  std::vector<unsigned long long> t((size_t)6 * c->ss_ns_pad);
  for (auto &s : c->slots) {
    if (!s.d_ss_acc) continue;
    HIP_TRY(c, hipStreamSynchronize(s.stream));
    if (out) {
      HIP_TRY(c, hipMemcpyAsync(t.data(), s.d_ss_acc, t.size() * sizeof(unsigned long long), hipMemcpyDeviceToHost, s.stream));
      HIP_TRY(c, hipStreamSynchronize(s.stream));
      for (uint32_t col = 0; col < kSsCols; col++)
        for (uint32_t i = 0; i < ns; i++) out[(size_t)col * ns + i] += t[(size_t)col * c->ss_ns_pad + i];
      for (uint32_t i = 0; i < ns; i++) out[(size_t)kSsCols * ns + i] += t[(size_t)kSsCols * c->ss_ns_pad];
    }
    if (reset) {
      HIP_TRY(c, hipMemsetAsync(s.d_ss_acc, 0, t.size() * sizeof(unsigned long long), s.stream));
      HIP_TRY(c, hipStreamSynchronize(s.stream));
    }
  }
  return BVCF_OK;
}

int bvcf_path(const bvcf_ctx *c) { return c ? (c->fused ? 2 : 1) : BVCF_E_ARG; }
int bvcf_bench_stream_kernel(const bvcf_ctx *c) { return (c && c->fused) ? (c->gen_mode ? 1 : 0) : -1; }

int bvcf_counters(bvcf_ctx *c, uint64_t out[8]) {
  if (!c || !out) return BVCF_E_ARG;
  memcpy(out, c->totals, sizeof c->totals);
  return BVCF_OK;
}

int bvcf_sum_counters(bvcf_ctx *const *ctxs, int n, uint64_t out[8]) {
  if (!ctxs || n < 0 || !out) return BVCF_E_ARG;
  for (int k = 0; k < 8; k++) out[k] = 0;
  for (int i = 0; i < n; i++) {
    if (!ctxs[i]) return BVCF_E_ARG;
    for (int k = 0; k < 8; k++) out[k] += ctxs[i]->totals[k];
  }
  return BVCF_OK;
}

int bvcf_bgzf_inflate_device(int device, const uint8_t *comp, size_t n_comp, uint8_t *out, size_t cap, size_t *n_out) {
  if ((!comp && n_comp) || !n_out || (!out && cap)) return BVCF_E_ARG;
  *n_out = 0;
  int n_dev = 0;
  if (hipGetDeviceCount(&n_dev) != hipSuccess || device < 0 || device >= n_dev) return BVCF_E_NODEV;
  std::vector<bvcf_bgzf::Block> blocks;
  const long used = bvcf_bgzf::scan(comp, n_comp, &blocks);
  if (used < 0 || (size_t)used != n_comp) return BVCF_E_FATAL;
  if (n_comp >= 0xFFF00000ull) return BVCF_E_TOO_BIG;
  std::vector<BgzfDesc> desc(blocks.size());
  uint64_t total = 0;
  for (size_t i = 0; i < blocks.size(); i++) {
    desc[i].in_off = blocks[i].in_off;
    desc[i].in_len = blocks[i].in_len;
    desc[i].out_off = (uint32_t)total;
    desc[i].isize = blocks[i].isize;
    total += blocks[i].isize;
  }
  *n_out = (size_t)total;
  if (total > cap || total >= 0xFFF00000ull) return BVCF_E_TOO_BIG;
  if (blocks.empty()) return BVCF_OK;
  if (hipSetDevice(device) != hipSuccess) return BVCF_E_HIP;
  hipDeviceProp_t prop;
  if (hipGetDeviceProperties(&prop, device) != hipSuccess) return BVCF_E_HIP;
  uint8_t *d_comp = nullptr, *d_text = nullptr;
  BgzfDesc *d_desc = nullptr;
  uint32_t *d_status = nullptr, *d_crc = nullptr;
  const size_t nb = blocks.size();
  int rc = BVCF_OK;
  std::vector<uint32_t> status(nb), crc(nb);
  if (hipMalloc(&d_comp, n_comp + 64) != hipSuccess || hipMalloc(&d_text, total + 64) != hipSuccess ||
      hipMalloc(&d_desc, nb * sizeof(BgzfDesc)) != hipSuccess || hipMalloc(&d_status, nb * 4) != hipSuccess ||
      hipMalloc(&d_crc, nb * 4) != hipSuccess) {
    rc = BVCF_E_NOMEM;
  } else if (hipMemcpy(d_comp, comp, n_comp, hipMemcpyHostToDevice) != hipSuccess ||
             hipMemcpy(d_desc, desc.data(), nb * sizeof(BgzfDesc), hipMemcpyHostToDevice) != hipSuccess) {
    rc = BVCF_E_HIP;
  } else {
    if (!launch_inflate(prop.multiProcessorCount, d_comp, d_desc, (uint32_t)nb, d_text, d_status, d_crc, nullptr, false)) rc = BVCF_E_NOMEM;
    if (rc || hipDeviceSynchronize() != hipSuccess || hipMemcpy(status.data(), d_status, nb * 4, hipMemcpyDeviceToHost) != hipSuccess ||
        hipMemcpy(crc.data(), d_crc, nb * 4, hipMemcpyDeviceToHost) != hipSuccess ||
        (total && hipMemcpy(out, d_text, total, hipMemcpyDeviceToHost) != hipSuccess))
      rc = rc ? rc : BVCF_E_HIP;
  }
  hipFree(d_comp);
  hipFree(d_text);
  hipFree(d_desc);
  hipFree(d_status);
  hipFree(d_crc);
  if (rc) return rc;
  for (size_t i = 0; i < nb; i++)
    if (status[i] != kInfOk || crc[i] != blocks[i].crc) return BVCF_E_FATAL;
  return BVCF_OK;
}

int bvcf_bgzf_deflate_device(int device, const uint8_t *text, size_t n, int add_eof, uint8_t *out, size_t cap, size_t *n_out) {
  if ((!text && n) || !n_out || (!out && cap)) return BVCF_E_ARG;
  *n_out = 0;
  int n_dev = 0;
  if (hipGetDeviceCount(&n_dev) != hipSuccess || device < 0 || device >= n_dev) return BVCF_E_NODEV;
  using namespace bvcf_bgzf_out;
  const size_t part = std::min<size_t>(std::max<size_t>(n, 1), 1028 * kPiece);
  std::string err;
  DeflateRun *r = deflate_open(device, part, &err);
  if (!r) return BVCF_E_HIP;
  std::vector<uint8_t> tmp;
  size_t total = 0;
  int rc = BVCF_OK;
  for (size_t at = 0; at < n && rc == BVCF_OK; at += part) {
    const size_t k = std::min(part, n - at);
    uint8_t *dst = out + total;
    size_t room = total < cap ? cap - total : 0, got = 0;
    if (room < bound(k)) {
      tmp.resize(bound(k));
      dst = tmp.data();
      room = tmp.size();
    }
    rc = deflate_run(r, text + at, k, dst, room, &got, nullptr, &err);
    if (rc == BVCF_OK && dst == tmp.data() && total + got <= cap) memcpy(out + total, tmp.data(), got);
    total += got;
  }
  deflate_close(r);
  if (rc) return rc;
  if (add_eof) {
    if (total + sizeof kEofBlock <= cap) memcpy(out + total, kEofBlock, sizeof kEofBlock);
    total += sizeof kEofBlock;
  }
  *n_out = total;
  return total > cap ? BVCF_E_TOO_BIG : BVCF_OK;
}

int bvcf_device_count(void) {
  int n = 0;
  if (hipGetDeviceCount(&n) != hipSuccess) return 0;
  return n;
}

int bvcf_allreduce_counters(bvcf_ctx *const *ctxs, int n, uint64_t out[8], int *used_rccl) {
  if (used_rccl) *used_rccl = 0;
  if (!ctxs || n < 0 || !out) return BVCF_E_ARG;
  for (int i = 0; i < n; i++)
    if (!ctxs[i]) return BVCF_E_ARG;
  bool distinct = true;
  for (int i = 0; i < n && distinct; i++)
    for (int j = 0; j < i; j++)
      if (ctxs[i]->device == ctxs[j]->device) distinct = false;
  const char *force = getenv("BVCF_RCCL");
  const bool want = distinct && (n >= 2 || (n == 1 && force && *force == '1'));
  if (!want) return bvcf_sum_counters(ctxs, n, out);

  bvcf_ctx *c0 = ctxs[0];
  static void *lib = dlopen("librccl.so.1", RTLD_NOW | RTLD_GLOBAL);
  if (!lib) {
    c0->err = std::string("dlopen librccl.so.1: ") + dlerror();
    return BVCF_E_HIP;
  }
  auto p_init = (decltype(&ncclCommInitAll))dlsym(lib, "ncclCommInitAll");
  auto p_destroy = (decltype(&ncclCommDestroy))dlsym(lib, "ncclCommDestroy");
  auto p_allreduce = (decltype(&ncclAllReduce))dlsym(lib, "ncclAllReduce");
  auto p_gstart = (decltype(&ncclGroupStart))dlsym(lib, "ncclGroupStart");
  auto p_gend = (decltype(&ncclGroupEnd))dlsym(lib, "ncclGroupEnd");
  auto p_errstr = (decltype(&ncclGetErrorString))dlsym(lib, "ncclGetErrorString");
  if (!p_init || !p_destroy || !p_allreduce || !p_gstart || !p_gend || !p_errstr) {
    c0->err = "librccl.so.1 lacks an expected symbol";
    return BVCF_E_HIP;
  }
  std::vector<int> devs(n);
  std::vector<ncclComm_t> comms(n, nullptr);
  std::vector<uint64_t *> d_buf(n, nullptr);
  for (int i = 0; i < n; i++) devs[i] = ctxs[i]->device;
  int rc = BVCF_OK;
  auto nccl_fail = [&](ncclResult_t r, const char *what) {
    c0->err = std::string(what) + ": " + p_errstr(r);
    rc = BVCF_E_HIP;
  };
  ncclResult_t r = p_init(comms.data(), n, devs.data());
  if (r != ncclSuccess) {
// ... 129 lines not shown
```

### bystro-vcf_amd/csrc/bvcf_head.hip.h

```cpp
#pragma once

#include "bvcf_common.hip.h"
#include "bvcf_alleles.hip.h"
#include "bvcf_gtscan.hip.h"
#include "bvcf_stream.hip.h"

namespace bvcf_dev {


constexpr int kGroup = 16;
constexpr int kGroupsPerWg = kWgThreads / kGroup;
constexpr uint32_t kWindow = kGroup * 16;
#ifndef BVCF_HEAD_STAGE
#define BVCF_HEAD_STAGE 64
#endif
constexpr uint32_t kHeadStage = BVCF_HEAD_STAGE;

__device__ __forceinline__ int glane() { return threadIdx.x & (kGroup - 1); }

__device__ __forceinline__ uint32_t group_sum(uint32_t v) {
  v += (uint32_t)__builtin_amdgcn_update_dpp(0, (int)v, 0x128, 0xF, 0xF, false);
  v += (uint32_t)__builtin_amdgcn_update_dpp(0, (int)v, 0x124, 0xF, 0xF, false);
  v += (uint32_t)__builtin_amdgcn_update_dpp(0, (int)v, 0x122, 0xF, 0xF, false);
  v += (uint32_t)__builtin_amdgcn_update_dpp(0, (int)v, 0x121, 0xF, 0xF, false);
  return v;
}

__device__ __forceinline__ uint32_t group_excl_scan(uint32_t v, uint32_t *total) {
  uint32_t inc = v;
  inc += (uint32_t)__builtin_amdgcn_update_dpp(0, (int)inc, 0x111, 0xF, 0xF, true);
  inc += (uint32_t)__builtin_amdgcn_update_dpp(0, (int)inc, 0x112, 0xF, 0xF, true);
  inc += (uint32_t)__builtin_amdgcn_update_dpp(0, (int)inc, 0x114, 0xF, 0xF, true);
  inc += (uint32_t)__builtin_amdgcn_update_dpp(0, (int)inc, 0x118, 0xF, 0xF, true);
  *total = group_sum(v);
  return inc - v;
}

__device__ __forceinline__ uint32_t gbcast0(uint32_t v) { return __shfl(v, 0, kGroup); }

template <class B>
__device__ inline bool filter_in(const B &buf, Span f, const uint16_t *off, const uint16_t *len, uint32_t n,
                                 const uint8_t *text) {
#pragma nounroll
  for (uint32_t i = 0; i < n; i++) {
    if (len[i] != f.len) continue;
    bool eq = true;
#pragma nounroll
    for (uint32_t k = 0; k < f.len && eq; k++) eq = buf[f.off + k] == text[off[i] + k];
    if (eq) return true;
  }
  return false;
}

__device__ inline void write_allele(const KernelArgs &a, uint32_t idx, uint32_t line, uint32_t alt_idx,
                                    const AlleleEval &e, long long pos, uint8_t ref, uint8_t alt_base,
                                    uint8_t site_type, uint32_t task, uint32_t cmap_off, const GtResult *gr = nullptr) {
  bvcf_allele r;
  r.pos = pos;
  r.line = line;
  r.alt_idx = alt_idx;
  r.alt_off = e.alt_off;
  r.alt_len = e.mnp ? 1u : e.alt_len;
  r.ac = gr ? gr->ac : 0u;
  r.an = gr ? gr->an : 0u;
  r.n_het = gr ? gr->n_het : 0u;
  r.n_hom = gr ? gr->n_hom : 0u;
  r.n_miss = gr ? gr->n_miss : 0u;
  const bool sparse = cmap_off != BVCF_NO_CMAP && (cmap_off & 1u);
  r.cmap_off = cmap_off != BVCF_NO_CMAP ? cmap_off & ~15u : cmap_off;
  r.ref = ref;
  r.alt_base = alt_base;
  r.kind = e.mnp ? (uint8_t)BVCF_ALT_BASE : e.kind;
  r.site_type = site_type;
  r.trtv = (site_type == BVCF_SITE_MULTI || r.kind != BVCF_ALT_BASE) ? 0 : trtv_of(ref, alt_base);
  r.flags = ((!e.mnp && e.pos_text) ? BVCF_ALLELE_POS_TEXT : 0) | (sparse ? BVCF_ALLELE_CMAP_SPARSE : 0);
  r.pad[0] = r.pad[1] = 0;
  r.gt_task = task;
  r.pad2 = 0;
  a.alleles[idx] = r;
}

constexpr uint32_t kNoTask = 0xFFFFFFFFu;

__device__ __forceinline__ bool further_listed(uint32_t cm) { return cm != BVCF_NO_CMAP && (cm & 15u) != 0u && (cm & 15u) != kRawEnc; }
__device__ __forceinline__ uint32_t further_kmax(uint32_t cm) { return (cm & 1u) ? ((cm >> 1) & 7u) + 1u : 1u; }

__device__ inline void put_task(const KernelArgs &a, uint32_t ti, uint32_t line, uint32_t allele, uint32_t s_begin,
                                uint32_t cend, uint32_t cmap_off, uint32_t kind = 0u, uint32_t n_rec = 0u, uint32_t rec0 = 0u,
                                uint32_t rec1 = 0u) {
  if (ti < a.max_tasks) {
    GtTask t;
    t.line = line;
    t.allele = allele;
    t.s_begin = s_begin;
    t.cend = cend;
    t.cmap_off = cmap_off;
    t.pad[0] = kind | (n_rec << kTaskRecShift);
    t.pad[1] = rec0;
    t.pad[2] = rec1;
    a.tasks[ti] = t;
    if (a.wide && allele != 0 && cend >= s_begin) atomicMax(&a.counters->pad[1], cend - s_begin);
  }
}


constexpr uint32_t kLinesPerStep = kWgThreads;
constexpr uint32_t kHeadRow = kHeadStage / 4 + 1;
constexpr uint32_t kTabRow = 11;

#ifdef BVCF_EXP_TIMES
__device__ unsigned long long g_head_t[6][8192];
#define HSTAMP(k)                                                  \
  {                                                                \
    const unsigned long long now_ = __builtin_readcyclecounter();  \
    hph_[k] += now_ - hlast_;                                      \
    hlast_ = now_;                                                 \
  }
#else
#define HSTAMP(k)
#endif
#if defined(BVCF_EXP_TIMES) && BVCF_EXP_TIMES + 0 == 3
#define HSTAMP_A(k)
#define HSTAMP_B(k) HSTAMP(k)
#else
#define HSTAMP_A(k) HSTAMP(k)
#define HSTAMP_B(k)
#endif
template <bool kAllWindows>
__device__ __forceinline__ void k_head_body(const KernelArgs &a) {
#ifdef BVCF_EXP_TIMES
  unsigned long long hph_[6] = {0, 0, 0, 0, 0, 0}, hlast_ = __builtin_readcyclecounter();
#endif
  __shared__ uint32_t s_head[kLinesPerStep * kHeadRow];
  __shared__ uint32_t s_tab[kLinesPerStep * kTabRow];
  __shared__ uint32_t s_ls[kLinesPerStep], s_len[kLinesPerStep], s_found[kLinesPerStep], s_staged[kLinesPerStep],
      s_extra[kLinesPerStep];
  __shared__ uint32_t s_wave[kWavesPerWg][4];
  __shared__ uint32_t s_base[5];
  __shared__ FilterTable s_ft;
  {
    const uint32_t *src = reinterpret_cast<const uint32_t *>(a.filters);
    uint32_t *dst = reinterpret_cast<uint32_t *>(&s_ft);
    for (uint32_t i = threadIdx.x; i < sizeof(FilterTable) / 4; i += kWgThreads) dst[i] = src[i];
  }
  const int gl = glane();
  const int g = threadIdx.x / kGroup;
  const int lane = lane_id();
  const int w = threadIdx.x >> 6;
  const uint32_t n_lines = min(a.counters->n_lines, a.max_lines);
  const uint32_t stride = gridDim.x * kLinesPerStep;
  const uint32_t need = min(9u, a.n_header - 1u);
  const uint32_t ns = a.n_samples;
  const bool maps = a.want_cmap && ns > 0;

  for (uint32_t line0 = blockIdx.x * kLinesPerStep; line0 < n_lines; line0 += stride) {
    __syncthreads();
    HSTAMP_A(0);

    uint32_t my_ls = 0, my_len = 0;
    uint32_t my_line_ls = 0, my_line_len = 0;
    if (!kAllWindows) {
      const uint32_t l = line0 + threadIdx.x;
      if (l < n_lines) {
        my_line_ls = a.line_off[l];
        if (a.fused) {
          my_line_len = a.line_len[l];
        } else {
          const uint32_t le = a.line_off[l + 1];
          my_line_len = le - my_line_ls >= a.eol_chars ? le - my_line_ls - a.eol_chars : 0u;
        }
      }
    } else {
      const uint32_t l = line0 + (uint32_t)gl * kGroupsPerWg + g;
      if (l < n_lines) {
        my_ls = a.line_off[l];
        if (a.fused) {
          my_len = a.line_len[l];
        } else {
          const uint32_t le = a.line_off[l + 1];
          my_len = le - my_ls >= a.eol_chars ? le - my_ls - a.eol_chars : 0u;
        }
      }
    }
    constexpr uint32_t kRounds = kLinesPerStep / kGroupsPerWg;
    u32x4 v_win[kAllWindows ? kRounds : 1u];
    uint32_t r_ls[kAllWindows ? kRounds : 1u], r_len[kAllWindows ? kRounds : 1u];
    if (kAllWindows) {
#pragma unroll
      for (uint32_t r = 0; r < kRounds; r++) {
        r_ls[r] = __shfl(my_ls, r, kGroup);
        r_len[r] = __shfl(my_len, r, kGroup);
        v_win[r] = *reinterpret_cast<const u32x4_u *>(a.buf + min(r_ls[r] + 16u * gl, a.cap - 16u));
      }
    }
    auto tokenise = [&](uint32_t r, uint32_t ls, uint32_t len_flag, const u32x4 &v_first) {
      const uint32_t ll = r * kGroupsPerWg + g;
      const uint32_t line = line0 + ll;
      if (line >= n_lines) return;
      const uint32_t len = len_flag & ~kHasHeadBits;
      if (len_flag & kHasHeadBits) {
        const uint32_t rel = 16u * gl;
        if (rel < kHeadStage) {
          uint32_t *row = &s_head[ll * kHeadRow + rel / 4];
          row[0] = v_first.x;
          row[1] = v_first.y;
          row[2] = v_first.z;
          row[3] = v_first.w;
        }
        if (gl == 0) {
          s_ls[ll] = ls;
          s_len[ll] = len_flag;
          s_found[ll] = 0;
          s_staged[ll] = min(len, kHeadStage);
          s_extra[ll] = 0;
        }
        return;
      }
      const uint32_t cend = ls + len;
      uint32_t found = 0, base = ls;
      for (; base < cend && found < need; base += kWindow) {
        const uint32_t off = base + 16u * gl;
        u32x4 v = base == ls ? v_first : load16(a.buf, off, a.cap);
        const uint32_t rel = off - ls;
        if (rel < kHeadStage) {
          uint32_t *row = &s_head[ll * kHeadRow + rel / 4];
          row[0] = v.x;
          row[1] = v.y;
          row[2] = v.z;
          row[3] = v.w;
        }
        uint32_t m = eq_mask16(v, '\t') & bits_until(cend, off);
        uint32_t tot;
        uint32_t rk = found + group_excl_scan(__popc(m), &tot);
        while (m && rk < need) {
          s_tab[ll * kTabRow + rk] = off + __ffs(m) - 1;
          m &= m - 1;
          rk++;
        }
        found += tot;
      }
      const uint32_t staged = min(base - ls, kHeadStage);
      uint32_t extra = 0;
      if (ns == 0 && found >= need) {
        for (; base < cend; base += kWindow) {
          const uint32_t off = base + 16u * gl;
          u32x4 v = load16(a.buf, off, a.cap);
          extra += __popc(eq_mask16(v, '\t') & bits_until(cend, off));
        }
        extra = group_sum(extra);
      }
      if (gl == 0) {
        s_ls[ll] = ls;
        s_len[ll] = len;
        s_found[ll] = found;
        s_staged[ll] = staged;
        s_extra[ll] = extra;
      }
    };
    u32x4 pre_b0 = {0u, 0u, 0u, 0u}, pre_b1 = {0u, 0u, 0u, 0u};
    GtResult pre_res = GtResult{};
    bool pre_res_ok = false;
    if (kAllWindows) {
#pragma unroll
      for (uint32_t r = 0; r < kRounds; r++) tokenise(r, r_ls[kAllWindows ? r : 0], r_len[kAllWindows ? r : 0], v_win[kAllWindows ? r : 0]);
    } else {
      constexpr uint32_t kLanesPerHead = kHeadStage / 16u, kLinesPerRound = kWgThreads / kLanesPerHead;
      constexpr uint32_t kHeadRounds = kLinesPerStep / kLinesPerRound;
      static_assert(kHeadStage % 16u == 0 && kWgThreads % kLanesPerHead == 0 && kLinesPerStep % kLinesPerRound == 0, "head staging");
      s_ls[threadIdx.x] = my_line_ls;
      s_len[threadIdx.x] = my_line_len;
      s_found[threadIdx.x] = 0;
      s_staged[threadIdx.x] = min(my_line_len & ~kHasHeadBits, kHeadStage);
      s_extra[threadIdx.x] = 0;
      __syncthreads();
      u32x4 hv[kHeadRounds];
      const uint32_t hq = threadIdx.x % kLanesPerHead;
#pragma unroll
      for (uint32_t r = 0; r < kHeadRounds; r++) {
        const uint32_t ll = r * kLinesPerRound + threadIdx.x / kLanesPerHead;
        hv[r] = u32x4{0u, 0u, 0u, 0u};
        if (line0 + ll < n_lines && (s_len[ll] & kHasHeadBits)) hv[r] = load16(a.buf, s_ls[ll] + 16u * hq, a.cap);
      }
      {
        const uint32_t line = line0 + threadIdx.x;
        if (line < n_lines && (my_line_len & kHasHeadBits)) {
          const u32x4 *bits = reinterpret_cast<const u32x4 *>(a.line_bits + (size_t)line * 8u);
          pre_b0 = bits[0];
          pre_b1 = bits[1];
        }
        if (line < n_lines && a.fused && ns > 0 && line < a.max_tasks) {
          pre_res = a.results[line];
          pre_res_ok = true;
        }
      }
#pragma unroll
      for (uint32_t r = 0; r < kHeadRounds; r++) {
        const uint32_t ll = r * kLinesPerRound + threadIdx.x / kLanesPerHead;
        if (line0 + ll < n_lines && (s_len[ll] & kHasHeadBits)) {
          uint32_t *row = &s_head[ll * kHeadRow + 4u * hq];
          row[0] = hv[r].x;
          row[1] = hv[r].y;
          row[2] = hv[r].z;
          row[3] = hv[r].w;
        }
      }
      auto wants = [&](uint32_t r) -> bool {
        const uint32_t ll = r * kGroupsPerWg + g;
        return r < kRounds && line0 + ll < n_lines && !(s_len[ll] & kHasHeadBits);
      };
      u32x4 v_next = {0u, 0u, 0u, 0u};
      if (wants(0)) v_next = load16(a.buf, s_ls[g] + 16u * gl, a.cap);
#pragma nounroll
      for (uint32_t r = 0; r < kRounds; r++) {
        const u32x4 v_first = v_next;
        if (wants(r + 1u)) v_next = load16(a.buf, s_ls[(r + 1u) * kGroupsPerWg + g] + 16u * gl, a.cap);
        if (wants(r)) {
          const uint32_t ll = r * kGroupsPerWg + g;
          tokenise(r, s_ls[ll], s_len[ll], v_first);
        }
      }
    }
    __syncthreads();

    HSTAMP_A(1);
    const uint32_t ll = threadIdx.x;
    const uint32_t line = line0 + ll;
    const bool active = line < n_lines;
    const uint32_t ls = active ? s_ls[ll] : 0u, len_flag = active ? s_len[ll] : 0u;
    const uint32_t len = len_flag & ~kHasHeadBits;
    uint32_t found = active ? s_found[ll] : 0u;
    const uint32_t cend = ls + len;
    uint32_t *tab = &s_tab[ll * kTabRow];
    if (len_flag & kHasHeadBits) {
      u32x4 b0 = pre_b0, b1 = pre_b1;
      if (kAllWindows) {
        const u32x4 *bits = reinterpret_cast<const u32x4 *>(a.line_bits + (size_t)line * 8u);
        b0 = bits[0];
        b1 = bits[1];
      }
      const uint32_t w[8] = {b0.x, b0.y, b0.z, b0.w, b1.x, b1.y, b1.z, b1.w};
      const uint32_t base = ls & ~3u;
      uint32_t k = 0;
#pragma unroll
      for (uint32_t q = 0; q < 8; q++) {
        uint32_t m = w[q];
        while (m && k < 9u) {
          tab[k++] = base + 32u * q + (uint32_t)__ffs(m) - 1u;
          m &= m - 1u;
        }
      }
      found = k;
    }
    Bytes hb;
    hb.g = a.buf;
    hb.lds = as_lds(&s_head[ll * kHeadRow]);
    hb.lo = ls;
    hb.sub = ls;
    hb.n = active ? s_staged[ll] : 0u;

    uint32_t status = BVCF_LINE_OK;
    uint32_t n_fields = 0;
    if (active && found < need) {
      status = BVCF_LINE_FIELDS;
      n_fields = found + 1;
    } else if (active && ns == 0) {
      n_fields = found + s_extra[ll] + 1;
      if (n_fields != a.n_header) status = BVCF_LINE_FIELDS;
    }

    auto fspan = [&](uint32_t i) -> Span {
      Span sp;
      sp.off = i == 0 ? ls : tab[i - 1] + 1;
      const uint32_t e = i < need ? tab[i] : cend;
      sp.len = e - sp.off;
      return sp;
    };

    uint32_t rec_first = 0, n_rec = 0, site_type = 0, first_task = line;
    bool task_written = false, primary_written = false;

    AlleleCtx c;
    uint32_t mode = 0, n_commas = 0, bound = 0, s_begin = cend;
    if (active && status == BVCF_LINE_OK && a.n_header > 6) {
      const FilterTable *ft = &s_ft;
      Span f = fspan(6);
      if (!ft->allow_nil && !filter_in(hb, f, ft->allow_off, ft->allow_len, ft->allow_n, ft->text))
        status = BVCF_LINE_FILTER;
      else if (!ft->deny_nil && filter_in(hb, f, ft->deny_off, ft->deny_len, ft->deny_n, ft->text))
        status = BVCF_LINE_FILTER;
    }
    const bool eval = active && status == BVCF_LINE_OK;
    if (eval) {
      c.buf = hb;
      c.chrom = fspan(0);
      c.pos = fspan(1);
      c.ref = fspan(3);
      c.alt = fspan(4);
      c.int_pos = 0;
      c.pos_bad = false;
      c.line = line;
      s_begin = need == 9 ? tab[8] + 1 : cend;
      bool same = c.alt.len == c.ref.len;
      uint32_t tl = 0, b2 = 0;
#pragma nounroll
      for (uint32_t i = 0; i <= c.alt.len; i++) {
        const uint8_t ch = i < c.alt.len ? hb[c.alt.off + i] : (uint8_t)',';
        if (i < c.alt.len && same) same = ch == hb[c.ref.off + i];
        if (ch == ',') {
          n_commas += i < c.alt.len;
          b2 += (tl == c.ref.len && c.ref.len > 1) ? c.ref.len : 1u;
          tl = 0;
        } else {
          tl++;
        }
      }
      mode = same ? 0u : (c.alt.len == 1 ? 1u : (c.ref.len == 0 ? 3u : 2u));
      bound = mode == 1 ? 1u : (mode == 2 ? b2 : 0u);
    }

    HSTAMP_A(2);
    const uint32_t want_rec = bound > 1 ? bound - 1 : 0u;
    uint32_t res_fields = 0, res_miss = 0;
    if (eval && a.fused && ns > 0 && line < a.max_tasks) {
      if (!kAllWindows && pre_res_ok) {
        res_fields = pre_res.n_fields;
        res_miss = pre_res.n_miss;
      } else {
        res_fields = a.results[line].n_fields;
        res_miss = a.results[line].n_miss;
      }
    }
    const bool deferred = eval && a.fused && ns > 0 && line < a.max_tasks && res_fields == kDeferred;
    const uint32_t want_task = ((eval && ns > 0 && mode == 2) ? n_commas : 0u) + (deferred ? 1u : 0u);
    uint32_t lcm = BVCF_NO_CMAP, want_real = 0;
    if (a.fused && want_task > 0) {
      if (deferred) {
        want_real = want_task;
      } else {
        if (maps) lcm = a.line_cmap[line];
        if (further_listed(lcm)) {
          const uint32_t kmax = further_kmax(lcm);
          if (res_miss != 0u && n_commas + 1u > kmax) want_real = n_commas + 1u - kmax;
        } else {
          want_real = n_commas;
        }
      }
    }
    const unsigned long long fin_mask = __ballot(a.fused && deferred);
    uint32_t wt_rec, wt_task, wt_real;
    uint32_t extra_base = wave_excl_scan(want_rec, &wt_rec);
    uint32_t task_base = wave_excl_scan(want_task, &wt_task);
    uint32_t real_base = wave_excl_scan(want_real, &wt_real);
    uint32_t fin_at = __builtin_amdgcn_mbcnt_hi((uint32_t)(fin_mask >> 32), __builtin_amdgcn_mbcnt_lo((uint32_t)fin_mask, 0u));
    if (lane == 0) {
      s_wave[w][0] = wt_rec;
      s_wave[w][1] = wt_task;
      s_wave[w][2] = (uint32_t)__popcll(fin_mask);
      s_wave[w][3] = wt_real;
    }
    __syncthreads();
    if (threadIdx.x < 5) {
      const uint32_t col = threadIdx.x == 4 ? 1u : threadIdx.x;
      uint32_t sum = 0;
      for (int k = 0; k < kWavesPerWg; k++) sum += s_wave[k][col];
      if (threadIdx.x == 4 && !(a.fused && maps)) sum = 0;
      uint32_t *ctr = threadIdx.x == 0 ? &a.counters->n_alleles : (threadIdx.x == 1 ? &a.counters->n_tasks :
                      (threadIdx.x == 2 ? &a.counters->n_finish : (threadIdx.x == 3 ? &a.counters->n_real : &a.counters->cmap_maps)));
      uint32_t got = 0;
      if (sum) got = atomicAdd(ctr, sum);
      s_base[threadIdx.x == 2 ? 3 : (threadIdx.x == 3 ? 4 : (threadIdx.x == 4 ? 2 : threadIdx.x))] = got;
    }
    __syncthreads();
    uint32_t task_rank = task_base;
    for (int k = 0; k < w; k++) {
      extra_base += s_wave[k][0];
      task_rank += s_wave[k][1];
      fin_at += s_wave[k][2];
      real_base += s_wave[k][3];
    }
    real_base += s_base[4];
    if (a.fused && deferred && s_base[3] + fin_at < a.max_lines + a.max_alleles) a.finish_items[s_base[3] + fin_at] = line;
    extra_base += n_lines + s_base[0];
    task_base = n_lines + s_base[1] + task_rank;
    const uint32_t map_base = a.fused ? s_base[2] + task_rank : task_base;

    HSTAMP_A(3);
    HSTAMP_B(0);
    const bool has_tok = eval && (mode == 1 || mode == 2);
    if (eval) {
      if (mode == 0) log_err(a, line, 0, BVCF_ERR_SAME);
      if (mode == 3) log_err(a, line, 0, BVCF_ERR_EMPTY_REF);
    }
    const bool fits = (unsigned long long)extra_base + want_rec <= a.max_alleles;
    uint32_t cm0 = BVCF_NO_CMAP;
    uint32_t task0 = line;
    uint32_t tasks_used = 0, emitted = 0, stype_line = 0;
    bool dropped = false;
    if (eval) {
      if (ns > 0 && !a.fused) {
        cm0 = cmap_of(a, line, maps && has_tok);
        put_task(a, line, line, 1, s_begin, cend, cm0);
        task_written = true;
      }
      if (ns > 0 && a.fused) {
        if (deferred) {
          task0 = task_base;
          cm0 = cmap_of(a, map_base, maps);
          put_task(a, task0, line, 1, s_begin, cend, cm0);
          if (real_base < a.max_tasks) a.real_tasks[real_base] = task0;
          tasks_used = 1;
        } else if (maps) {
          cm0 = a.line_cmap[line];
        }
      }
      first_task = task0;
    }
    const bool final0 = eval && a.fused && ns > 0 && !deferred && line < a.max_tasks;
    {
      const uint32_t n_tok = has_tok ? (mode == 1 ? 1u : n_commas + 1u) : 0u;
      uint32_t n_pairs;
      const uint32_t pair0 = wave_excl_scan(n_tok, &n_pairs);
      const uint32_t lflags = mode | (deferred ? 4u : 0u) | (fits ? 8u : 0u) | (final0 ? 16u : 0u);
      uint32_t *const s_mark = &s_found[(uint32_t)w * kWave];
#pragma nounroll
      for (uint32_t q0 = 0; q0 < n_pairs; q0 += kWave) {
        const bool mine = n_tok && pair0 < q0 + kWave && pair0 + n_tok > q0;
        const uint32_t seg0 = pair0 > q0 ? pair0 - q0 : 0u;
        s_mark[lane] = 0u;
        __builtin_amdgcn_fence(__ATOMIC_RELEASE, "wavefront");
        __builtin_amdgcn_wave_barrier();
        if (mine) s_mark[seg0] = (uint32_t)lane + 1u;
        __builtin_amdgcn_fence(__ATOMIC_RELEASE, "wavefront");
        __builtin_amdgcn_wave_barrier();
        const uint32_t n_here = min(n_pairs - q0, (uint32_t)kWave);
        const bool pl = (uint32_t)lane < n_here;
        const uint32_t mk = wave_incl_scan_max(s_mark[lane]);
        const uint32_t o = (pl && mk) ? mk - 1u : (uint32_t)lane;
        auto from_owner = [&](uint32_t v) -> uint32_t { return (uint32_t)__builtin_amdgcn_ds_bpermute((int)(o * 4u), (int)v); };
        const uint32_t o_pair0 = from_owner(pair0), o_flags = from_owner(lflags), o_commas = from_owner(n_commas);
        const uint32_t o_extra = from_owner(extra_base), o_task = from_owner(task_base), o_map = from_owner(map_base);
        const uint32_t o_task0 = from_owner(task0), o_cm0 = from_owner(cm0);
        const uint32_t o_real = from_owner(real_base), o_miss = from_owner(res_miss);
        GtResult o_res = GtResult{};
        if (!kAllWindows) {
          o_res.ac = from_owner(pre_res.ac);
          o_res.an = from_owner(pre_res.an);
          o_res.n_het = from_owner(pre_res.n_het);
          o_res.n_hom = from_owner(pre_res.n_hom);
          o_res.n_miss = from_owner(pre_res.n_miss);
          o_res.n_fields = from_owner(pre_res.n_fields);
          o_res.regular = 1;
        }
        const uint32_t o_emitted = from_owner(emitted), o_used = from_owner(tasks_used), o_dropped = from_owner(dropped ? 1u : 0u);
        HSTAMP_B(1);
        const uint32_t k = q0 + (uint32_t)lane - o_pair0;
        const uint32_t o_mode = o_flags & 3u;
        const bool o_deferred = (o_flags & 4u) != 0, o_fits = (o_flags & 8u) != 0, o_final0 = (o_flags & 16u) != 0;
        const uint32_t oll = (uint32_t)w * kWave + o, o_line = line0 + oll;
        const uint32_t o_ls = s_ls[oll], o_cend = o_ls + (s_len[oll] & ~kHasHeadBits);
        const uint32_t *otab = &s_tab[oll * kTabRow];
        AlleleCtx c;
        c.buf.g = a.buf;
        c.buf.lds = as_lds(&s_head[oll * kHeadRow]);
        c.buf.lo = o_ls;
        c.buf.sub = o_ls;
        c.buf.n = pl ? s_staged[oll] : 0u;
        const Bytes &ob = c.buf;
        c.chrom = Span{o_ls, otab[0] - o_ls};
        c.pos = Span{otab[0] + 1u, otab[1] - otab[0] - 1u};
        c.ref = Span{otab[2] + 1u, otab[3] - otab[2] - 1u};
        c.alt = Span{otab[3] + 1u, (need > 4u ? otab[4] : o_cend) - otab[3] - 1u};
        c.int_pos = 0;
        c.pos_bad = false;
        c.line = o_line;
        const uint32_t o_sbegin = need == 9 ? otab[8] + 1u : o_cend;

        AlleleEval e = AlleleEval{};
        Span t = c.alt;
        const bool snp = o_mode == 1 && c.ref.len == 1u;
        if (pl && (snp || !eval_token_row<kHeadStage>(as_lds_words(&s_head[oll * kHeadRow]), c.buf.n, o_ls, c, k, o_mode == 1, &t, e))) {
          if (o_mode == 1) {
            eval_single(c, e);
          } else {
            uint32_t i = 0, seen = 0, start = 0;
#pragma nounroll
            for (; i < c.alt.len && seen < k; i++)
              if (ob[c.alt.off + i] == ',') {
                seen++;
                start = i + 1u;
              }
            uint32_t end = start;
#pragma nounroll
            while (end < c.alt.len && ob[c.alt.off + end] != ',') end++;
            t.off = c.alt.off + start;
            t.len = end - start;
            eval_token(c, t, e);
          }
        }
        HSTAMP_B(2);
        const uint32_t seg_lane = o_pair0 > q0 ? o_pair0 - q0 : 0u;
        auto seg_excl = [&](uint32_t v) -> uint32_t {
          const uint32_t ex = wave_incl_scan(v) - v;
          return ex - (uint32_t)__builtin_amdgcn_ds_bpermute((int)(seg_lane * 4u), (int)ex);
        };
        const uint32_t stop_me = (pl && e.stop) ? 1u : 0u;
        const uint32_t stops_before = seg_excl(stop_me);
        const bool dropped_me = o_dropped != 0u || stops_before != 0u;
        const bool live = pl && !dropped_me;
        const uint32_t n_me = live ? e.n : 0u;
        const uint32_t tk_me = (live && ns > 0 && k > 0 && e.n > 0) ? 1u : 0u;
        const uint32_t emitted_before = o_emitted + seg_excl(n_me);
        const uint32_t used_before = o_used + seg_excl(tk_me);
        uint32_t stype_me = 0;
        HSTAMP_B(3);
        uint32_t real_at = kNoTask, real_task = kNoTask;
        if (pl && a.fused && ns > 0 && k > 0 && o_mode == 2u) {
          if (o_deferred)
            real_at = o_real + k;
          else if (!further_listed(o_cm0))
            real_at = o_real + k - 1u;
          else if (o_miss != 0u && k >= further_kmax(o_cm0))
            real_at = o_real + k - further_kmax(o_cm0);
        }

        if (live) {
          if (e.err) log_err(a, o_line, (e.err == BVCF_ERR_POS) ? 0u : k + 1u, e.err, k);
          if (e.n) {
            uint32_t task = o_task0, cm_off = o_cm0;
            GtResult g0 = GtResult{};
            if (o_final0 && ns > 0) g0 = kAllWindows ? a.results[o_line] : o_res;
            const GtResult *gr = (k == 0 && o_final0) ? &g0 : nullptr;
            GtResult r = GtResult{};
            if (ns > 0 && k > 0) {
              task = o_task + used_before;
              bool resolved = false;
              const bool raw = a.fused && !o_deferred && o_cm0 != BVCF_NO_CMAP && (o_cm0 & 15u) == kRawEnc;
              if (a.fused && !o_deferred && further_listed(o_cm0) && task < a.max_tasks) {
                const uint32_t kmax = further_kmax(o_cm0);
                r.ac = 0;
                r.an = g0.an;
                r.n_het = r.n_hom = 0;
                r.n_miss = g0.n_miss;
                r.n_fields = g0.n_fields;
                r.regular = 1;
                r.pad = 0;
                if (k + 1u <= kmax) {
                  cm_off = ((o_cm0 & ~15u) + 64u * k) | 1u;
                  const uint32_t *list = reinterpret_cast<const uint32_t *>(a.cmap + (cm_off & ~15u));
                  const uint32_t n = min(list[0], (uint32_t)BVCF_CMAP_SPARSE_MAX);
#pragma nounroll
                  for (uint32_t i = 0; i < n; i++) {
                    const uint32_t b = list[1u + i] & 0xFFu, lo = b & 0x55u, hi = (b >> 1) & 0x55u;
                    r.n_het += __popc(lo & ~hi);
                    r.n_hom += __popc(hi & ~lo);
                  }
                  r.ac = r.n_het + 2u * r.n_hom;
                  resolved = true;
                } else if (o_miss == 0u) {
                  cm_off = BVCF_NO_CMAP;
                  resolved = true;
                }
                if (resolved) {
                  a.results[task] = r;
                  put_task(a, task, o_line, 0, o_cend, o_cend, BVCF_NO_CMAP);
                  gr = &r;
                }
              }
              const uint32_t t_rec = (a.fused && !o_deferred && o_fits) ? e.n : 0u;
              const uint32_t rec0 = emitted_before == 0u ? o_line : o_extra + emitted_before - 1u, rec1 = o_extra + emitted_before;
              if (raw) {
                resolved = true;
                cm_off = cmap_of(a, o_map + used_before, maps);
                put_task(a, task, o_line, k + 1, (o_cm0 & ~15u) + a.cmap_stride, o_cend, cm_off, kRawTask, t_rec, rec0, rec1);
                real_task = task;
              }
              if (!resolved) {
                cm_off = cmap_of(a, o_map + used_before, maps);
                put_task(a, task, o_line, k + 1, o_sbegin, o_cend, cm_off, 0u, t_rec, rec0, rec1);
                real_task = task;
              }
            }
            if (ns == 0) task = kNoTask;
            if (o_fits) {
              uint8_t stype;
              if (o_commas > 0)
                stype = BVCF_SITE_MULTI;
              else if (!e.mnp && e.kind == BVCF_ALT_DEL)
                stype = BVCF_SITE_DEL;
              else if (!e.mnp && e.kind == BVCF_ALT_INS)
                stype = BVCF_SITE_INS;
              else
                stype = e.n > 1 ? BVCF_SITE_MNP : BVCF_SITE_SNP;
              stype_me = stype;
              auto slot = [&](uint32_t j) -> uint32_t { return j == 0 ? o_line : o_extra + j - 1; };
              if (e.mnp) {
                uint32_t j = 0;
#pragma nounroll
                for (uint32_t i = 0; i < c.ref.len; i++) {
                  const uint8_t rb = ob[c.ref.off + i], ab = ob[t.off + i];
                  if (rb == ab) continue;
                  write_allele(a, slot(emitted_before + j), o_line, k, e, c.int_pos + (long long)i, rb, ab, stype, task, cm_off, gr);
                  j++;
                }
              } else {
                write_allele(a, slot(emitted_before), o_line, k, e, e.pos, e.ref, e.alt_base, stype, task, cm_off, gr);
              }
            }
          }
        }
        if (real_at < a.max_tasks) a.real_tasks[real_at] = real_task;
        HSTAMP_B(4);
// ... 133 lines not shown
```

### bystro-vcf_amd/csrc/bvcf_stream.hip.h

```cpp
#pragma once

#include <type_traits>

#include "bvcf_common.hip.h"
#include "bvcf_gtscan.hip.h"

namespace bvcf_dev {


constexpr uint32_t kNone = 0xFFFFFFFFu;
constexpr uint32_t kDeferred = 0xFFFFFFFEu;

__device__ inline uint32_t find_eol(const KernelArgs &a, uint32_t from, uint32_t limit) {
  const int lane = lane_id();
  const uint32_t last_off = (a.cap - 16u) & ~3u;
  for (uint32_t base = from & ~3u; base < limit; base += 4u * kChunk) {
    u32x4 v[4];
#pragma unroll
    for (int q = 0; q < 4; q++) v[q] = ld_stream(a.buf + min(base + q * kChunk + 16u * lane, last_off));
#pragma unroll
    for (int q = 0; q < 4; q++) {
      const uint32_t off = base + q * kChunk + 16u * lane;
      uint32_t m = eq_mask16(v[q], a.eol_byte) & bits_until(limit, off);
      if (off < from) m &= ~bits_until(from, off);
      const unsigned long long b = __ballot(m != 0);
      if (b) {
        const int src = __ffsll((long long)b) - 1;
        return lane_value(off + __ffs(m) - 1, src);
      }
    }
  }
  return kNone;
}

__device__ __forceinline__ uint32_t nth_bit(uint32_t m, uint32_t k) {
  for (uint32_t i = 0; i < k; i++) m &= m - 1;
  return __ffs(m) - 1;
}

__device__ __forceinline__ uint32_t head_window(const KernelArgs &a, u32x4 v, uint32_t base, uint32_t n_lanes,
                                                uint32_t *found_io, uint32_t *eolp) {
  const int lane = lane_id();
  const uint32_t need = 9;
  const uint32_t off = base + 16u * lane;
  uint32_t valid = bits_until(a.nbytes, off);
  if ((uint32_t)lane >= n_lanes) valid = 0;
  const uint32_t me = eq_mask16(v, a.eol_byte) & valid;
  uint32_t mt = eq_mask16(v, '\t') & valid;
  const unsigned long long be = __ballot(me != 0);
  uint32_t eol_here = kNone;
  if (be) {
    const int src = __ffsll((long long)be) - 1;
    eol_here = lane_value(off + __ffs(me) - 1, src);
    mt &= bits_until(eol_here, off);
  }
  uint32_t tot;
  const uint32_t cnt = __popc(mt);
  const uint32_t prefix = wave_excl_scan(cnt, &tot);
  if (*found_io + tot >= need) {
    const uint32_t target = need - 1 - *found_io;
    const bool mine = prefix <= target && target < prefix + cnt;
    const unsigned long long bm = __ballot(mine);
    const int src = __ffsll((long long)bm) - 1;
    const uint32_t pos = mine ? off + nth_bit(mt, target - prefix) : 0u;
    return lane_value(pos, src);
  }
  *found_io += tot;
  *eolp = eol_here;
  return kNone;
}

__device__ __forceinline__ uint32_t head_window16(const KernelArgs &a, u32x4 v, uint32_t start, uint32_t *mt_out) {
  const int lane = lane_id();
  const uint32_t need = 9;
  const uint32_t base = start & ~3u;
  if (lane == 0) v.x &= 0xFFFFFFFFu << (8u * (start & 3u));
  const uint32_t off = base + 16u * lane;
  uint32_t valid = bits_until(a.nbytes, off);
  if (lane >= 16) valid = 0;
  const uint32_t e4 = a.eol_byte * 0x01010101u;
  const uint32_t eol_any = (zero_bytes(v.x ^ e4) | zero_bytes(v.y ^ e4) | zero_bytes(v.z ^ e4) | zero_bytes(v.w ^ e4));
  if (__ballot(eol_any != 0 && lane < 16)) return kNone;
  const uint32_t mt = eq_mask16(v, '\t') & valid;
  *mt_out = mt;
  const uint32_t cnt = __popc(mt);
  uint32_t x = cnt;
  x += (uint32_t)__builtin_amdgcn_update_dpp(0, (int)x, 0x111, 0xF, 0xF, true);
  x += (uint32_t)__builtin_amdgcn_update_dpp(0, (int)x, 0x112, 0xF, 0xF, true);
  x += (uint32_t)__builtin_amdgcn_update_dpp(0, (int)x, 0x114, 0xF, 0xF, true);
  x += (uint32_t)__builtin_amdgcn_update_dpp(0, (int)x, 0x118, 0xF, 0xF, true);
  const uint32_t prefix = x - cnt;
  const bool mine = lane < 16 && prefix < need && need <= x;
  const unsigned long long bm = __ballot(mine);
  if (!bm) return kNone;
  const int src = __ffsll((long long)bm) - 1;
  const uint32_t pos = mine ? off + nth_bit(mt, need - 1 - prefix) : 0u;
  return lane_value(pos, src);
}

constexpr int kPipeChunks = 10;

#ifdef BVCF_EXP_TIMES
__device__ unsigned long long g_wave_t[2][32768];
__device__ unsigned long long g_phase_t[8][32768];
__device__ unsigned int g_wave_hw[2][32768];
#if BVCF_EXP_TIMES + 0 == 2
#define STAMP(k)
#else
#define STAMP(k)                                                   \
  {                                                                \
    const unsigned long long now_ = __builtin_readcyclecounter();  \
    ph_[k] += now_ - last_;                                        \
    last_ = now_;                                                  \
  }
#endif
#else
#define STAMP(k)
#endif
__global__ __launch_bounds__(kWgThreads) void k_stream(KernelArgs a) {
#ifdef BVCF_EXP_TIMES
  if ((threadIdx.x & 63) == 0) {
    g_wave_t[0][wave_in_grid()] = wall_clock64();
    g_wave_hw[0][wave_in_grid()] = __builtin_amdgcn_s_getreg((31 << 11) | 4);
    g_wave_hw[1][wave_in_grid()] = __builtin_amdgcn_s_getreg((31 << 11) | 20);
  }
  unsigned long long ph_[8] = {0, 0, 0, 0, 0, 0, 0, 0}, last_ = __builtin_readcyclecounter();
#endif
  __shared__ __attribute__((aligned(16))) uint8_t s_stage[kWavesPerWg][kStageBytes];
  __shared__ __attribute__((aligned(16))) RawList s_sparse[kWavesPerWg];
  uint8_t *stage = s_stage[wave_in_wg()];
  RawList *sparse = &s_sparse[wave_in_wg()];
  const int lane = lane_id();
  const uint32_t wave = wave_in_grid();
  const uint32_t n_waves = gridDim.x * kWavesPerWg;
  const uint32_t ns = a.n_samples;
  const uint32_t nb = a.nbytes;
  const uint32_t T = a.tile_bytes;
  const bool maps = a.want_cmap != 0;
  const uint32_t n_chunks = (ns * 4u + kChunk - 1u) / kChunk;
  const uint32_t table1 = (1u << 2) | (3u << 28);
  const bool pipelined = n_chunks >= 1 && n_chunks <= (uint32_t)kPipeChunks && a.eol_chars == 1;
  uint32_t cm_next = 0, cm_end = 0;
  uint32_t seen = 0;
  uint32_t n_other = 0;
  uint32_t n_listed = 0;

  const uint32_t q_tiles = a.n_tiles / n_waves, r_tiles = a.n_tiles % n_waves;
  const uint32_t per_wave = q_tiles + (r_tiles ? 1u : 0u);
  const uint32_t tile_lo = wave * q_tiles + min(wave, r_tiles);
  const uint32_t tile_hi = tile_lo + q_tiles + (wave < r_tiles ? 1u : 0u);
  const uint32_t r0 = tile_lo * T;
  const uint32_t r1 = (uint32_t)min((unsigned long long)tile_hi * T, (unsigned long long)nb);
  uint32_t tile = tile_lo, n_local = 0;
  uint32_t p = kNone;
  if (tile_lo < tile_hi) {
    p = 0;
    if (r0 > 0) {
      const uint32_t q = find_eol(a, r0 - 1, r1);
      p = q == kNone ? kNone : q + 1;
    }
  }

  const uint32_t lines_bound = (uint32_t)(((unsigned long long)per_wave * T) / (4ull * ns + 8ull)) + 2u;
  const uint32_t slots_per_wave = lines_bound + lines_bound / 4u;
// ... 87 lines not shown
          uint32_t sB = 0, peB = 0;
          bool b_ok = false;
          if (hv_ok) {
            const uint32_t t9 = head_window16(a, hv, peA + 1u, &mtB);
            if (t9 != kNone) {
              sB = t9 + 1;
              const unsigned long long pb = (unsigned long long)sB + 4ull * ns - 1ull;
              if (pb + 1ull <= nb) {
                peB = (uint32_t)pb;
                b_ok = true;
              }
            }
          }
          const bool hvc_ok = b_ok && peB + 1u < r1;
          hv = head_at(hvc_ok ? peB + 1u : sA);
          STAMP(1);
          const uint32_t cmA = bcast0(map_slot());
          uint8_t *cm = cmA != BVCF_NO_CMAP ? a.cmap + cmA : nullptr;
#ifdef BVCF_EXP_NO_SPARSE
          const bool sparse_ok = false;
#else
          const bool sparse_ok = cm != nullptr && a.cmap_stride >= 4u * kSparseWords;
#endif
          FastAcc acc = {0, 0, 0, 0, sparse_ok ? 0u : kDenseMode};
          if (cm && !sparse_ok) zero_stage(stage, nc);
          const uint32_t rA = sA & amask;
          const uint32_t w0 = __builtin_amdgcn_alignbyte(__builtin_amdgcn_readfirstlane(va[0].y),
                                                         __builtin_amdgcn_readfirstlane(va[0].x), rA);
          const uint32_t sep = (w0 >> 8) & 0xFFu;
          if (sep != '|' && sep != '/') acc.bad = 1;
          const uint32_t kref = 0x09300030u | (sep << 8);
          const uint32_t term_xor = (a.eol_byte ^ 0x09u) << 24;
          const uint32_t s_next = b_ok ? sB : sA;
          STAMP(2);
#pragma unroll
          for (int g = 0; g < kLoads; g++) {
            if ((uint32_t)g < nc) {
              const uint32_t nx = (uint32_t)g + 1u < nc
                                      ? (uint32_t)__builtin_amdgcn_readfirstlane(va[g + 1 < kPipeChunks ? g + 1 : g].x) : 0u;
              fast_chunk(realign(va[g], nx, rA), g, nc, ns, kref, table1, cm, stage, a.cmap_stride, term_xor, acc, sparse_ok ? sparse : nullptr);
            }
            va[g] = chunk_at(s_next, g);
          }
          STAMP(3);
          uint32_t enc = 0, n_slots = 1;
          const uint32_t raw_slots = (kRawAreaBytes + a.cmap_stride - 1u) / a.cmap_stride;
          auto raw_area = [&]() -> uint8_t * {
            const uint32_t reserve = (r1 - min(r1, peA)) / (4u * ns + 8u) + 2u;
            if (cm_next + 1u + raw_slots + reserve > cm_end || cmap_of(a, cm_next + raw_slots, true) == BVCF_NO_CMAP) return nullptr;
            return cm + a.cmap_stride;
          };
          if (sparse_ok && acc.n_sp < kDenseMode) {
            enc = finish_list(sparse, acc, cm, min(kListAlleles, a.cmap_stride / (4u * kSparseWords)), stage, nc, a.cmap_stride,
                              acc.n_sp > BVCF_CMAP_SPARSE_MAX ? raw_area() : nullptr);
          } else if (sparse_ok && acc.n_oth == 0u) {
            enc = 1u << 1;
          } else if (sparse_ok && acc.n_oth < kDenseMode) {
            enc = finish_dense(sparse, acc.n_oth, raw_area());
          }
          if (enc == kRawEnc) n_slots += raw_slots;
          if (__any(acc.bad != 0)) {
            s_begin = sA;
            p = pA;
            break;
          }
          finish_stats(acc, &st);
          seen++;
          commit(pA, peA, st, false, cmA == BVCF_NO_CMAP ? cmA : cmA | enc, bitsA, mtA, n_slots);
          p = peA + 1u;
          if (!b_ok) {
            s_begin = kNone;
            break;
          }
          pA = peA + 1u;
          sA = sB;
          peA = peB;
          hv_ok = hvc_ok;
          mtA = mtB;
#ifdef BVCF_EXP_NO_HEAD_BITS
          bitsA = false;
#else
          bitsA = true;
#endif
          STAMP(4);
        }
      };
      switch (n_chunks) {
        case 1: run_pipeline(std::integral_constant<int, 1>{}); break;
        case 2: run_pipeline(std::integral_constant<int, 2>{}); break;
        case 3: run_pipeline(std::integral_constant<int, 3>{}); break;
        case 4: run_pipeline(std::integral_constant<int, 4>{}); break;
        case 5: run_pipeline(std::integral_constant<int, 5>{}); break;
        case 6: run_pipeline(std::integral_constant<int, 6>{}); break;
        case 7: run_pipeline(std::integral_constant<int, 7>{}); break;
        case 8: run_pipeline(std::integral_constant<int, 8>{}); break;
        case 9: run_pipeline(std::integral_constant<int, 9>{}); break;
        default: run_pipeline(std::integral_constant<int, 10>{}); break;
      }
      static_assert(kPipeChunks == 10, "the dispatch above covers 1..10 chunks");
      if (s_begin == kNone) continue;
    } else if (pred + a.eol_chars <= nb) {
      const uint32_t pe = (uint32_t)pred;
      bool term = true;
      if (a.eol_chars == 2) term = a.buf[pe + 1] == a.eol_byte && a.buf[pe] != a.eol_byte;
      if (term) {
        const uint32_t cm_off = map_slot();
        uint8_t *cm = cm_off != BVCF_NO_CMAP ? a.cmap + cm_off : nullptr;
        if (gt_scan_fast(a, s_begin, ns, 1, cm, stage, a.eol_chars == 1, &st)) {
          seen++;
          commit(p, pe, st, false, cm_off);
          p = pe + a.eol_chars;
          continue;
        }
      }
    }

    {
      const uint32_t e = find_eol(a, s_begin, nb);
      if (e == kNone) break;
      seen++;
      if (e + 1 < s_begin + a.eol_chars) {
        p = e + 1;
        continue;
      }
      cend = e + 1 - a.eol_chars;
      const GtStats none = {0, 0, 0, 0, 0};
      if (cend - p + 1u >= a.n_header) {
        commit(p, cend, none, true, BVCF_NO_CMAP);
        n_other++;
      }
      p = cend + a.eol_chars;
    }
  }
  for (; tile < tile_hi; tile++) {
    if (lane == 0) a.census[tile] = n_local;
    n_listed += n_local;
    n_local = 0;
  }
  if (lane == 0) a.run_lines[wave] = n_listed;
  if (lane == 0 && seen) atomicAdd(&a.counters->lines_seen, seen);
  if (lane == 0 && n_other) atomicAdd(&a.counters->n_other_shape, n_other);
#ifdef BVCF_EXP_TIMES
  if (lane == 0) {
    g_wave_t[1][wave] = wall_clock64();
    for (int k = 0; k < 8; k++) g_phase_t[k][wave] = ph_[k];
  }
#endif
}

}
#include "bvcf_streamgen.hip.h"
namespace bvcf_dev {

__global__ __launch_bounds__(kWgThreads) void k_order(KernelArgs a) {
  __shared__ uint32_t s_part[2][kWavesPerWg];
  __shared__ uint32_t s_first[kWgThreads + 1];
  const int lane = lane_id();
  const uint32_t w = threadIdx.x >> 6;
  if (a.n_tiles == 0) {
    if (blockIdx.x == 0 && threadIdx.x == 0) a.counters->n_lines = 0;
    return;
  }
  const uint32_t pw = a.prod_waves;
  const uint32_t q_tiles = a.n_tiles / pw, r_tiles = a.n_tiles % pw;
  auto run_first = [&](uint32_t wv) -> uint32_t { return wv * q_tiles + min(wv, r_tiles); };
  const uint32_t per_wg = (pw + gridDim.x - 1u) / gridDim.x;
  const uint32_t w_lo = min(blockIdx.x * per_wg, pw), w_hi = min(w_lo + per_wg, pw);
  const uint32_t t_lo = run_first(w_lo), t_hi = run_first(w_hi);
  uint32_t sum = 0;
  {
    const uint32_t n4 = w_lo / 4u;
    const u32x4 *c4 = reinterpret_cast<const u32x4 *>(a.run_lines);
    for (uint32_t i = threadIdx.x; i < n4; i += kWgThreads) {
      const u32x4 v = c4[i];
      sum += v.x + v.y + v.z + v.w;
    }
    if (threadIdx.x < (w_lo & 3u)) sum += a.run_lines[n4 * 4u + threadIdx.x];
  }
  sum = wave_sum(sum);
  if (lane == 0) s_part[0][w] = sum;
  __syncthreads();
  uint32_t base = 0;
  for (uint32_t i = 0; i < kWavesPerWg; i++) base += s_part[0][i];
  if (w_hi == pw && w_lo < pw && t_lo >= t_hi && threadIdx.x == 0) {
    uint32_t rest = 0;
    for (uint32_t i = w_lo; i < w_hi; i++) rest += a.run_lines[i];
    a.counters->n_lines = base + rest;
  }
  if (t_lo >= t_hi) return;
  for (uint32_t c0 = t_lo; c0 < t_hi; c0 += kWgThreads) {
    const uint32_t n_here = min(t_hi - c0, (uint32_t)kWgThreads);
    const uint32_t cnt = threadIdx.x < n_here ? min(a.census[c0 + threadIdx.x], a.tile_quota) : 0u;
    uint32_t wtot;
    const uint32_t pre = wave_excl_scan(cnt, &wtot);
    __syncthreads();
    if (lane == 0) s_part[1][w] = wtot;
    __syncthreads();
    uint32_t wbase = 0, total = 0;
    for (uint32_t i = 0; i < kWavesPerWg; i++) {
      if (i < w) wbase += s_part[1][i];
      total += s_part[1][i];
    }
    s_first[threadIdx.x] = wbase + pre;
    if (threadIdx.x == 0) s_first[kWgThreads] = total;
    __syncthreads();
    const uint32_t pairs = n_here * a.tile_quota;
    for (uint32_t i = threadIdx.x; i < pairs; i += kWgThreads) {
      const uint32_t tl = i / a.tile_quota, k = i % a.tile_quota;
      const uint32_t first = s_first[tl];
      const uint32_t next = tl + 1u < kWgThreads ? s_first[tl + 1u] : s_first[kWgThreads];
      if (k >= next - first) continue;
      const uint32_t g = base + first + k;
      if (g >= a.max_lines) continue;
      const size_t ei = (size_t)(c0 + tl) * a.tile_quota + k;
      const StreamEntry en = a.entries[ei];
      a.line_off[g] = en.ls;
      a.line_len[g] = en.len & ~kNotRegular;
      a.line_cmap[g] = en.cmap_off;
      if (en.len & kHasHeadBits) {
        const u32x4 *src = reinterpret_cast<const u32x4 *>(a.head_bits + ei * 16u);
        u32x4 *dst = reinterpret_cast<u32x4 *>(a.line_bits + (size_t)g * 8u);
        dst[0] = src[0];
        dst[1] = src[1];
      }
      if (g < a.max_tasks) {
        GtResult r;
        r.ac = en.ac;
        r.an = en.an;
        r.n_het = en.n_het;
        r.n_hom = en.n_hom;
        r.n_miss = en.n_miss;
        r.n_fields = en.n_miss == kDeferred ? kDeferred : a.n_header - 9u;
        r.regular = (en.n_miss == kDeferred || (en.len & kNotRegular)) ? 0u : 1u;
        r.pad = 0;
        a.results[g] = r;
      }
    }
    base += s_first[kWgThreads];
  }
  if (t_hi == a.n_tiles && threadIdx.x == 0) a.counters->n_lines = base;
}


}
```

### include/bvcf_bench.h

```cpp
#ifndef BVCF_BENCH_H
#define BVCF_BENCH_H

#include "bvcf.h"

#ifdef __cplusplus
extern "C" {
#endif

int bvcf_bench_device(bvcf_ctx *ctx, const void *const *dblocks, const size_t *nbytes, int n_blocks, int iters,
                      float *chain_ms, float *gt_ms, uint64_t counts[5]);
int bvcf_bench_device_slots(bvcf_ctx *ctx, const void *const *device_blocks, const size_t *nbytes, int n_blocks, int iters,
                            uint32_t slots_in_use, float *chain_ms, float *scan_ms, uint64_t counts[5]);

int bvcf_bench_stream_kernel(const bvcf_ctx *ctx);

#ifdef __cplusplus
}
#endif
#endif
```

### include/bvcf_plan.h

```cpp
#ifndef BVCF_PLAN_H
#define BVCF_PLAN_H

#include <stddef.h>
#include <stdint.h>

#ifdef __cplusplus
extern "C" {
#endif

typedef struct {
  uint64_t data_off;
  uint64_t range_bytes;
  uint64_t spare_bytes;
  uint64_t n_ranges;
} bvcf_range_plan;

int bvcf_plan_text_ranges(uint64_t file_size, uint64_t data_off, uint64_t max_batch_bytes, uint64_t first_line_bytes,
                          bvcf_range_plan *out);
int bvcf_plan_bgzf_ranges(uint64_t file_size, uint64_t data_off, uint32_t n_workers, uint64_t max_batch_bytes,
                          bvcf_range_plan *out);

enum {
  BVCF_CUT_LINES = 0,
  BVCF_CUT_NONE = 1,
  BVCF_CUT_LONG = 2
};
typedef struct {
  int32_t kind;
  uint32_t reserved;
  uint64_t start, end, long_start;
} bvcf_text_cut;
int bvcf_cut_text_range(const uint8_t *window, uint64_t n, uint64_t own_len, int is_first, int is_last, uint8_t eol,
                        bvcf_text_cut *out);

long bvcf_find_bgzf_chain(const uint8_t *buf, size_t n, size_t from);

typedef struct {
  uint32_t readers;
  uint32_t copy_threads;
  uint32_t format_threads;
  uint32_t busy_total;
} bvcf_thread_budget;
enum { BVCF_MODE_STREAM = 0, BVCF_MODE_TEXT_RANGES = 1, BVCF_MODE_BGZF_RANGES = 2 };
int bvcf_plan_threads(uint32_t cpus, uint32_t n_workers, int mode, bvcf_thread_budget *out);

typedef struct {
  uint32_t worker;
  uint32_t piece;
  uint64_t range;
  uint64_t file_off;
  uint64_t nbytes;
  uint64_t own;
  uint32_t first_off;
  uint8_t bgzf;
  uint8_t bgzf_flags;
  uint8_t last_piece;
  uint8_t reserved;
} bvcf_plan_block;

int bvcf_plan_fd(int fd_in, int fd_err, uint32_t n_workers, uint64_t max_batch_bytes, int device_inflate,
                 bvcf_plan_block *out, size_t cap, size_t *n_out, int *mode_out, bvcf_range_plan *plan_out);

#ifdef __cplusplus
}
#endif
#endif
```

Measured before the change: 489.5 million variants/s.

## Resolve simple biallelic SNP lines in k_order and compact leftovers for head kernel

The ordering kernel now evaluates lines with head bits through a fast path that writes the line and allele records directly for simple SNPs (or filter failures). Only declined lines are compacted into a left_lines list for the head tokeniser, which walks that list and sizes its grid from the previous batch's leftover count. This removes most head-kernel work for uniform biallelic SNP data, at the cost of extra work and atomics in k_order, a duplicated record-building path that must match the full tokeniser, and a grid size that depends on the previous batch.

```diff
diff --git a/bystro-vcf_amd/__init__.py b/bystro-vcf_amd/__init__.py
--- a/bystro-vcf_amd/__init__.py
+++ b/bystro-vcf_amd/__init__.py
@@ -30,10 +30,10 @@
 SAMPLE_STATS_COLUMNS = ["sample", "het", "hom", "missing", "transitions", "transversions", "heterozygosity", "homozygosity",
                         "missingness", "trTv"]
 
-BENCH_EXPORTS = ["bvcf_bench_device", "bvcf_bench_device_slots", "bvcf_bench_stream_kernel"]
+BENCH_EXPORTS = ["bvcf_bench_device", "bvcf_bench_device_slots", "bvcf_bench_stream_kernel", "bvcf_bench_head_left"]
 
 PLAN_EXPORTS = ["bvcf_plan_text_ranges", "bvcf_plan_bgzf_ranges", "bvcf_cut_text_range", "bvcf_find_bgzf_chain",
-                "bvcf_plan_threads", "bvcf_plan_fd"]
+                "bvcf_plan_threads", "bvcf_plan_fd", "bvcf_head_fast_line"]
 
 EXPORTS = [
     "bvcf_create", "bvcf_destroy", "bvcf_last_error", "bvcf_version", "bvcf_reserve", "bvcf_set_sample_names", "bvcf_set_row_format", "bvcf_alloc_pinned", "bvcf_alloc_pinned_near", "bvcf_warmup",
@@ -180,6 +180,21 @@
     rc = lib.bvcf_plan_fd(fd_in, fd_err, n_workers, max_batch_bytes, device_inflate, out, cap, C.byref(n), C.byref(mode), C.byref(plan))
     assert n.value <= cap, "more blocks than room"
     return rc, mode.value, plan, [out[i] for i in range(n.value)]
+
+
+HEAD_FAST_DECLINE, HEAD_FAST_PASS, HEAD_FAST_FILTER = 0, 1, 2
+HAS_HEAD_BITS, NOT_REGULAR, DEFERRED = 0x80000000, 0x40000000, 0xFFFFFFFE
+
+
+def head_fast_line(head, ls, len_flags, counts, cmap_off, tab_bits, line, n_header, allow="PASS,.", exclude=""):
+    lib.bvcf_head_fast_line.argtypes = [C.c_char_p, C.c_uint32, C.c_uint32, C.c_uint32, C.POINTER(C.c_uint32), C.c_uint32,
+                                        C.POINTER(C.c_uint32), C.c_uint32, C.c_uint32, C.c_char_p, C.c_char_p, C.c_void_p, C.c_void_p]
+    L = np.zeros(1, dtype=LINE_DTYPE)
+    A = np.zeros(1, dtype=ALLELE_DTYPE)
+    v = lib.bvcf_head_fast_line(bytes(head), len(head), ls, len_flags, (C.c_uint32 * 5)(*counts), cmap_off,
+                                (C.c_uint32 * 8)(*tab_bits), line, n_header, allow.encode(), exclude.encode(),
+                                L.ctypes.data, A.ctypes.data)
+    return v, (L[0] if v != HEAD_FAST_DECLINE else None), (A[0] if v == HEAD_FAST_PASS else None)
 
 
 class BvcfError(RuntimeError):
@@ -577,6 +592,12 @@
         k = lib.bvcf_bench_stream_kernel(self.h)
         return None if k < 0 else ("k_stream_gen" if k else "k_stream")
 
+    def head_left(self):
+        lib.bvcf_bench_head_left.argtypes = [C.c_void_p]
+        lib.bvcf_bench_head_left.restype = C.c_long
+        n = lib.bvcf_bench_head_left(self.h)
+        return None if n < 0 else int(n)
+
     def sample_stats(self, reset=False):
         out = np.zeros(6 * self.n_samples, dtype=np.uint64)
         lib.bvcf_sample_stats.argtypes = [C.c_void_p, C.c_void_p, C.c_int]
diff --git a/bystro-vcf_amd/csrc/bvcf_common.hip.h b/bystro-vcf_amd/csrc/bvcf_common.hip.h
--- a/bystro-vcf_amd/csrc/bvcf_common.hip.h
+++ b/bystro-vcf_amd/csrc/bvcf_common.hip.h
@@ -38,6 +38,7 @@
   uint32_t n_full;
   uint32_t n_real;
   uint32_t n_other_shape;
+  uint32_t n_left;
 };
 
 struct StreamEntry {
@@ -108,6 +109,8 @@
   uint32_t *line_bits;
   uint32_t *finish_items;
   uint32_t *real_tasks;
+  uint32_t *left_lines;
+  uint32_t head_fast;
   uint32_t s1_fmode;
   uint32_t s1_fkey[4], s1_flen[4];
 };
diff --git a/bystro-vcf_amd/csrc/bvcf_core.hip b/bystro-vcf_amd/csrc/bvcf_core.hip
--- a/bystro-vcf_amd/csrc/bvcf_core.hip
+++ b/bystro-vcf_amd/csrc/bvcf_core.hip
@@ -1,5 +1,6 @@
 #include "bvcf_device.hip.h"
 #include "../../include/bvcf_bench.h"
+#include "../../include/bvcf_plan.h"
 #include "bvcf_bgzf.h"
 #include "bvcf_bgzf_out.h"
 
@@ -53,6 +54,7 @@
   uint32_t win_tabs_cap = 0;
   StreamEntry *d_entries = nullptr;
   uint32_t *d_line_len = nullptr, *d_line_cmap = nullptr, *d_line_bits = nullptr, *d_finish_items = nullptr;
+  uint32_t *d_left_lines = nullptr;
   uint16_t *d_head_bits = nullptr;
   bvcf_names *d_name_lists = nullptr, *h_name_lists = nullptr;
   uint32_t *d_name_tot = nullptr;
@@ -109,6 +111,8 @@
   bool fused = false;
   bool gen_mode = false;
   uint32_t last_real = 0xFFFFFFFFu, last_finish = 0xFFFFFFFFu;
+  uint32_t last_left = 0xFFFFFFFFu;
+  bool head_fast = true;
   bool shape_seen = false;
   int gen_policy = -1;
   uint32_t gen_grid = 0;
@@ -220,6 +224,7 @@
   hipFree(s.d_line_cmap);
   hipFree(s.d_line_bits);
   hipFree(s.d_finish_items);
+  hipFree(s.d_left_lines);
   hipFree(s.d_head_bits);
   hipFree(s.d_name_lists);
   hipFree(s.d_name_tot);
@@ -324,8 +329,10 @@
   hipFree(s.d_line_cmap);
   hipFree(s.d_line_bits);
   hipFree(s.d_finish_items);
+  hipFree(s.d_left_lines);
   s.d_line_bits = nullptr;
   s.d_finish_items = nullptr;
+  s.d_left_lines = nullptr;
   hipHostFree(s.h_lines);
   hipHostFree(s.h_alleles);
   hipHostFree(s.h_errs);
@@ -368,6 +375,7 @@
   if (c->fused) {
     HIP_TRY(c, hipMalloc(&s.d_line_bits, c->max_lines * 8 * sizeof(uint32_t)));
     HIP_TRY(c, hipMalloc(&s.d_finish_items, (c->max_lines + c->max_alleles) * sizeof(uint32_t)));
+    HIP_TRY(c, hipMalloc(&s.d_left_lines, c->max_lines * sizeof(uint32_t)));
   }
   if (c->packed) {
     s.hcap_recs = std::max<uint64_t>(4096, c->max_lines / 16);
@@ -495,6 +503,8 @@
   a.line_bits = s.d_line_bits;
   a.finish_items = s.d_finish_items;
   a.real_tasks = s.d_finish_items ? s.d_finish_items + c->max_lines : nullptr;
+  a.left_lines = s.d_left_lines;
+  a.head_fast = c->head_fast ? 1u : 0u;
   a.s1_fmode = c->s1_fmode;
   for (int i = 0; i < 4; i++) {
     a.s1_fkey[i] = c->s1_fkey[i];
@@ -512,6 +522,7 @@
 void adapt_stream_kernel(bvcf_ctx *c, bool was_gen, const BatchCounters &ctr) {
   c->last_real = ctr.n_real;
   c->last_finish = ctr.n_finish;
+  c->last_left = ctr.n_left;
   if (c->gen_policy >= 0 || !c->fused || ctr.n_lines < 16) return;
   c->shape_seen = true;
   if ((uint64_t)ctr.n_other_shape * 2u > ctr.n_lines) c->gen_mode = !was_gen;
@@ -570,11 +581,15 @@
 #else
     constexpr int skip = 0, head_wgs = 4, gt_div = 1;
 #endif
+    const uint32_t head_full = (uint32_t)c->n_cu * (uint32_t)head_wgs;
+    const uint32_t head_grid = (c->last_left == 0xFFFFFFFFu || !c->head_fast)
+                                   ? head_full
+                                   : std::min<uint32_t>(head_full, std::max<uint32_t>((uint32_t)c->n_cu / 4u, c->last_left / kWgThreads + 1u));
     if (skip & 1) {
     } else if (c->p.n_slots > 1)
-      hipLaunchKernelGGL(k_head_lean, dim3(c->n_cu * head_wgs), dim3(kWgThreads), 0, st, a);
+      hipLaunchKernelGGL(k_head_lean, dim3(head_grid), dim3(kWgThreads), 0, st, a);
     else
-      hipLaunchKernelGGL(k_head, dim3(c->n_cu * head_wgs), dim3(kWgThreads), 0, st, a);
+      hipLaunchKernelGGL(k_head, dim3(head_grid), dim3(kWgThreads), 0, st, a);
     const uint32_t gt_full = (uint32_t)c->gt_grid / (uint32_t)gt_div;
     const uint32_t gt_wgs = c->last_real == 0xFFFFFFFFu ? gt_full
                             : std::min<uint32_t>(gt_full, std::max<uint32_t>((uint32_t)c->n_cu / 4u, c->last_real / (2u * kWavesPerWg) + 1u));
@@ -1200,6 +1215,7 @@
   c->fused = c->n_samples > 0 && (path == 2 || path == 3 || (path == 0 && p->n_header_fields >= 256 && !many_samples));
   c->wide = !c->fused && many_samples;
   if (const char *e = getenv("BVCF_GEN_STREAM")) c->gen_policy = atoi(e) != 0 ? 1 : 0;
+  if (const char *e = getenv("BVCF_HEAD_FAST")) c->head_fast = atoi(e) != 0;
   if (!c->fused || c->n_samples > 4u * kStageBytes) c->gen_policy = 0;
   c->gen_mode = c->gen_policy == 1;
   if (path == 3 && c->gen_policy < 0) {
@@ -1992,6 +2008,38 @@
 int bvcf_path(const bvcf_ctx *c) { return c ? (c->fused ? 2 : 1) : BVCF_E_ARG; }
 int bvcf_bench_stream_kernel(const bvcf_ctx *c) { return (c && c->fused) ? (c->gen_mode ? 1 : 0) : -1; }
 
+long bvcf_bench_head_left(const bvcf_ctx *c) { return (c && c->fused && c->last_left != 0xFFFFFFFFu) ? (long)c->last_left : -1; }
+
+int bvcf_head_fast_line(const uint8_t *head, uint32_t head_bytes, uint32_t ls, uint32_t len_flags, const uint32_t counts[5],
+                        uint32_t cmap_off, const uint32_t tab_bits[8], uint32_t line, uint32_t n_header, const char *allow_filter,
+                        const char *exclude_filter, bvcf_line *out_line, bvcf_allele *out_allele) {
+  if (!head || !counts || !tab_bits || !out_line || !out_allele) return -1;
+  FilterTable ft;
+  memset(&ft, 0, sizeof ft);
+  uint32_t used = 0;
+  if (fill_filter(allow_filter, true, &ft.allow_nil, &ft.allow_n, ft.allow_off, ft.allow_len, ft.text, &used) ||
+      fill_filter(exclude_filter, false, &ft.deny_nil, &ft.deny_n, ft.deny_off, ft.deny_len, ft.text, &used))
+    return -1;
+  HeadFastHostBytes hb;
+  memset(&hb, 0, sizeof hb);
+  memcpy(hb.b, head, std::min<size_t>(head_bytes, kHeadFastBytes + 16));
+  StreamEntry en;
+  en.ls = ls;
+  en.len = len_flags;
+  en.ac = counts[0];
+  en.an = counts[1];
+  en.n_het = counts[2];
+  en.n_hom = counts[3];
+  en.n_miss = counts[4];
+  en.cmap_off = cmap_off;
+  HeadFastHostOut out;
+  memset(&out, 0, sizeof out);
+  const int v = head_fast_eval(en, tab_bits, hb, line, n_header, &ft, out);
+  if (v != kHeadFastDecline) memcpy(out_line, out.Lw, sizeof out.Lw);
+  if (v == kHeadFastPass) memcpy(out_allele, out.Aw, sizeof out.Aw);
+  return v;
+}
+
 int bvcf_counters(bvcf_ctx *c, uint64_t out[8]) {
   if (!c || !out) return BVCF_E_ARG;
   memcpy(out, c->totals, sizeof c->totals);
diff --git a/bystro-vcf_amd/csrc/bvcf_head.hip.h b/bystro-vcf_amd/csrc/bvcf_head.hip.h
--- a/bystro-vcf_amd/csrc/bvcf_head.hip.h
+++ b/bystro-vcf_amd/csrc/bvcf_head.hip.h
@@ -148,19 +148,22 @@
   const int lane = lane_id();
   const int w = threadIdx.x >> 6;
   const uint32_t n_lines = min(a.counters->n_lines, a.max_lines);
+  const uint32_t n_walk = a.fused ? min(a.counters->n_left, n_lines) : n_lines;
+  auto line_at = [&](uint32_t at) -> uint32_t { return a.fused ? a.left_lines[at] : at; };
   const uint32_t stride = gridDim.x * kLinesPerStep;
   const uint32_t need = min(9u, a.n_header - 1u);
   const uint32_t ns = a.n_samples;
   const bool maps = a.want_cmap && ns > 0;
 
-  for (uint32_t line0 = blockIdx.x * kLinesPerStep; line0 < n_lines; line0 += stride) {
+  for (uint32_t line0 = blockIdx.x * kLinesPerStep; line0 < n_walk; line0 += stride) {
     __syncthreads();
     HSTAMP_A(0);
 
     uint32_t my_ls = 0, my_len = 0;
     uint32_t my_line_ls = 0, my_line_len = 0;
+    const uint32_t my_line = line0 + threadIdx.x < n_walk ? line_at(line0 + threadIdx.x) : n_lines;
     if (!kAllWindows) {
-      const uint32_t l = line0 + threadIdx.x;
+      const uint32_t l = my_line;
       if (l < n_lines) {
         my_line_ls = a.line_off[l];
         if (a.fused) {
@@ -171,7 +174,8 @@
         }
       }
     } else {
-      const uint32_t l = line0 + (uint32_t)gl * kGroupsPerWg + g;
+      const uint32_t at = line0 + (uint32_t)gl * kGroupsPerWg + g;
+      const uint32_t l = at < n_walk ? line_at(at) : n_lines;
       if (l < n_lines) {
         my_ls = a.line_off[l];
         if (a.fused) {
@@ -195,8 +199,7 @@
     }
     auto tokenise = [&](uint32_t r, uint32_t ls, uint32_t len_flag, const u32x4 &v_first) {
       const uint32_t ll = r * kGroupsPerWg + g;
-      const uint32_t line = line0 + ll;
-      if (line >= n_lines) return;
+      if (line0 + ll >= n_walk) return;
       const uint32_t len = len_flag & ~kHasHeadBits;
       if (len_flag & kHasHeadBits) {
         const uint32_t rel = 16u * gl;
@@ -279,10 +282,10 @@
       for (uint32_t r = 0; r < kHeadRounds; r++) {
         const uint32_t ll = r * kLinesPerRound + threadIdx.x / kLanesPerHead;
         hv[r] = u32x4{0u, 0u, 0u, 0u};
-        if (line0 + ll < n_lines && (s_len[ll] & kHasHeadBits)) hv[r] = load16(a.buf, s_ls[ll] + 16u * hq, a.cap);
+        if (line0 + ll < n_walk && (s_len[ll] & kHasHeadBits)) hv[r] = load16(a.buf, s_ls[ll] + 16u * hq, a.cap);
       }
       {
-        const uint32_t line = line0 + threadIdx.x;
+        const uint32_t line = my_line;
         if (line < n_lines && (my_line_len & kHasHeadBits)) {
           const u32x4 *bits = reinterpret_cast<const u32x4 *>(a.line_bits + (size_t)line * 8u);
           pre_b0 = bits[0];
@@ -296,7 +299,7 @@
 #pragma unroll
       for (uint32_t r = 0; r < kHeadRounds; r++) {
         const uint32_t ll = r * kLinesPerRound + threadIdx.x / kLanesPerHead;
-        if (line0 + ll < n_lines && (s_len[ll] & kHasHeadBits)) {
+        if (line0 + ll < n_walk && (s_len[ll] & kHasHeadBits)) {
           uint32_t *row = &s_head[ll * kHeadRow + 4u * hq];
           row[0] = hv[r].x;
           row[1] = hv[r].y;
@@ -306,7 +309,7 @@
       }
       auto wants = [&](uint32_t r) -> bool {
         const uint32_t ll = r * kGroupsPerWg + g;
-        return r < kRounds && line0 + ll < n_lines && !(s_len[ll] & kHasHeadBits);
+        return r < kRounds && line0 + ll < n_walk && !(s_len[ll] & kHasHeadBits);
       };
       u32x4 v_next = {0u, 0u, 0u, 0u};
       if (wants(0)) v_next = load16(a.buf, s_ls[g] + 16u * gl, a.cap);
@@ -324,7 +327,7 @@
 
     HSTAMP_A(1);
     const uint32_t ll = threadIdx.x;
-    const uint32_t line = line0 + ll;
+    const uint32_t line = my_line;
     const bool active = line < n_lines;
     const uint32_t ls = active ? s_ls[ll] : 0u, len_flag = active ? s_len[ll] : 0u;
     const uint32_t len = len_flag & ~kHasHeadBits;
@@ -556,7 +559,7 @@
         const uint32_t k = q0 + (uint32_t)lane - o_pair0;
         const uint32_t o_mode = o_flags & 3u;
         const bool o_deferred = (o_flags & 4u) != 0, o_fits = (o_flags & 8u) != 0, o_final0 = (o_flags & 16u) != 0;
-        const uint32_t oll = (uint32_t)w * kWave + o, o_line = line0 + oll;
+        const uint32_t oll = (uint32_t)w * kWave + o, o_line = from_owner(line);
         const uint32_t o_ls = s_ls[oll], o_cend = o_ls + (s_len[oll] & ~kHasHeadBits);
         const uint32_t *otab = &s_tab[oll * kTabRow];
         AlleleCtx c;
diff --git a/bystro-vcf_amd/csrc/bvcf_headfast.hip.h b/bystro-vcf_amd/csrc/bvcf_headfast.hip.h
--- /dev/null
+++ b/bystro-vcf_amd/csrc/bvcf_headfast.hip.h
@@ -0,0 +1,151 @@
+#pragma once
+
+#include <stddef.h>
+
+#include "bvcf_common.hip.h"
+
+namespace bvcf_dev {
+
+constexpr uint32_t kHeadFastBytes = 64;
+constexpr uint32_t kHeadFastFilter = 16;
+constexpr uint32_t kHfNoTask = 0xFFFFFFFFu;
+constexpr uint32_t kHfDeferred = 0xFFFFFFFEu;
+
+enum { kHeadFastDecline = 0, kHeadFastPass = 1, kHeadFastFilterFail = 2 };
+
+static_assert(sizeof(bvcf_line) == 64 && sizeof(bvcf_allele) == 64, "records are written as sixteen words");
+static_assert(offsetof(bvcf_line, fend) == 8 && offsetof(bvcf_line, rec_first) == 44 && offsetof(bvcf_line, n_rec) == 48 &&
+                  offsetof(bvcf_line, n_fields) == 52 && offsetof(bvcf_line, gt_task) == 56 && offsetof(bvcf_line, status) == 60 &&
+                  offsetof(bvcf_line, site_type) == 61,
+              "bvcf_line words");
+static_assert(offsetof(bvcf_allele, line) == 8 && offsetof(bvcf_allele, alt_idx) == 12 && offsetof(bvcf_allele, alt_off) == 16 &&
+                  offsetof(bvcf_allele, alt_len) == 20 && offsetof(bvcf_allele, ac) == 24 && offsetof(bvcf_allele, n_miss) == 40 &&
+                  offsetof(bvcf_allele, cmap_off) == 44 && offsetof(bvcf_allele, ref) == 48 && offsetof(bvcf_allele, alt_base) == 49 &&
+                  offsetof(bvcf_allele, kind) == 50 && offsetof(bvcf_allele, site_type) == 51 && offsetof(bvcf_allele, trtv) == 52 &&
+                  offsetof(bvcf_allele, flags) == 53 && offsetof(bvcf_allele, gt_task) == 56,
+              "bvcf_allele words");
+
+__host__ __device__ __forceinline__ bool hf_is_actg(uint32_t c) {
+  const uint32_t d = c - 'A';
+  return d < 20u && ((0x80045u >> (d & 31u)) & 1u);
+}
+
+__host__ __device__ __forceinline__ uint32_t hf_trtv(uint32_t ref, uint32_t alt) {
+  const uint32_t x = ((ref ^ alt) >> 1) & 3u;
+  return (hf_is_actg(ref) && hf_is_actg(alt)) ? (x == 3u ? 1u : 2u) : 0u;
+}
+
+__host__ __device__ __forceinline__ uint32_t hf_next_bit(unsigned long long x[4]) {
+  uint32_t pos = 256u;
+  bool done = false;
+#pragma unroll
+  for (uint32_t q = 0; q < 4; q++) {
+    const bool take = !done && x[q] != 0ull;
+    if (take) {
+      pos = 64u * q + (uint32_t)__builtin_ctzll(x[q]);
+      x[q] &= x[q] - 1ull;
+    }
+    done = done || take;
+  }
+  return pos;
+}
+
+__host__ __device__ __forceinline__ uint32_t hf_byte16(const uint32_t v[4], uint32_t k) {
+  const uint32_t w = k < 8u ? (k < 4u ? v[0] : v[1]) : (k < 12u ? v[2] : v[3]);
+  return (w >> (8u * (k & 3u))) & 0xFFu;
+}
+
+__host__ __device__ inline bool hf_filter_in(const uint32_t f[4], uint32_t n, const uint16_t *off, const uint16_t *len, uint32_t cnt,
+                                             const uint8_t *text) {
+  bool hit = false;
+  for (uint32_t i = 0; i < cnt; i++) {
+    const uint32_t kl = len[i];
+    if (kl > kHeadFastFilter) continue;
+    bool eq = kl == n;
+    for (uint32_t k = 0; k < kl; k++) eq = eq && hf_byte16(f, k) == text[off[i] + k];
+    hit = hit || eq;
+  }
+  return hit;
+}
+
+template <class H, class Out>
+__host__ __device__ inline int head_fast_eval(const StreamEntry &en, const uint32_t bits[8], const H &head, uint32_t g, uint32_t n_header,
+                                              const FilterTable *ft, Out &out) {
+  if (!(en.len & kHasHeadBits) || (en.len & kNotRegular) || en.n_miss == kHfDeferred || n_header <= 9u) return kHeadFastDecline;
+  const uint32_t ls = en.ls, len = en.len & ~(kHasHeadBits | kNotRegular), sh = ls & 3u;
+  unsigned long long x[4];
+#pragma unroll
+  for (uint32_t q = 0; q < 4; q++) x[q] = ((unsigned long long)bits[2 * q + 1] << 32) | bits[2 * q];
+  uint32_t t[9];
+#pragma unroll
+  for (uint32_t i = 0; i < 9; i++) t[i] = hf_next_bit(x) - sh;
+  if (t[8] + sh >= 256u) return kHeadFastDecline;
+  if (t[6] >= kHeadFastBytes || t[8] >= len) return kHeadFastDecline;
+  if (t[3] - t[2] != 2u || t[4] - t[3] != 2u) return kHeadFastDecline;
+  const uint32_t f_off = t[5] + 1u, f_len = t[6] - f_off;
+  if (f_len > kHeadFastFilter) return kHeadFastDecline;
+  const uint32_t ref = head.byte(t[2] + 1u), alt = head.byte(t[3] + 1u);
+  uint32_t fv[4];
+  head.bytes16(f_off, fv);
+  if (!hf_is_actg(alt) || alt == ref) return kHeadFastDecline;
+  bool pass = true;
+  if (!ft->allow_nil && !hf_filter_in(fv, f_len, ft->allow_off, ft->allow_len, ft->allow_n, ft->text))
+    pass = false;
+  else if (!ft->deny_nil && hf_filter_in(fv, f_len, ft->deny_off, ft->deny_len, ft->deny_n, ft->text))
+    pass = false;
+  uint32_t Lw[16];
+  Lw[0] = ls;
+  Lw[1] = len;
+#pragma unroll
+  for (uint32_t i = 0; i < 9; i++) Lw[2 + i] = t[i];
+  Lw[11] = 0;
+  Lw[12] = pass ? 1u : 0u;
+  Lw[13] = pass ? n_header : 0u;
+  Lw[14] = g;
+  Lw[15] = pass ? (uint32_t)BVCF_LINE_OK | ((uint32_t)BVCF_SITE_SNP << 8) : (uint32_t)BVCF_LINE_FILTER;
+  out.line(Lw);
+  if (!pass) return kHeadFastFilterFail;
+  uint32_t Aw[16];
+  const uint32_t cm = en.cmap_off;
+  const bool sparse = cm != BVCF_NO_CMAP && (cm & 1u);
+  Aw[0] = Aw[1] = 0;
+  Aw[2] = g;
+  Aw[3] = 0;
+  Aw[4] = 0;
+  Aw[5] = 1;
+  Aw[6] = en.ac;
+  Aw[7] = en.an;
+  Aw[8] = en.n_het;
+  Aw[9] = en.n_hom;
+  Aw[10] = en.n_miss;
+  Aw[11] = cm != BVCF_NO_CMAP ? cm & ~15u : cm;
+  Aw[12] = ref | (alt << 8) | ((uint32_t)BVCF_ALT_BASE << 16) | ((uint32_t)BVCF_SITE_SNP << 24);
+  Aw[13] = hf_trtv(ref, alt) | ((BVCF_ALLELE_POS_TEXT | (sparse ? BVCF_ALLELE_CMAP_SPARSE : 0u)) << 8);
+  Aw[14] = g;
+  Aw[15] = 0;
+  out.allele(Aw);
+  return kHeadFastPass;
+}
+
+struct HeadFastHostBytes {
+  uint8_t b[kHeadFastBytes + 16];
+  __host__ __device__ uint32_t byte(uint32_t rel) const { return b[rel]; }
+  __host__ __device__ void bytes16(uint32_t rel, uint32_t out[4]) const {
+#pragma unroll
+    for (uint32_t q = 0; q < 4; q++)
+      out[q] = (uint32_t)b[rel + 4 * q] | ((uint32_t)b[rel + 4 * q + 1] << 8) | ((uint32_t)b[rel + 4 * q + 2] << 16) |
+               ((uint32_t)b[rel + 4 * q + 3] << 24);
+  }
+};
+
+struct HeadFastHostOut {
+  uint32_t Lw[16], Aw[16];
+  void line(const uint32_t w[16]) {
+    for (int i = 0; i < 16; i++) Lw[i] = w[i];
+  }
+  void allele(const uint32_t w[16]) {
+    for (int i = 0; i < 16; i++) Aw[i] = w[i];
+  }
+};
+
+}
diff --git a/bystro-vcf_amd/csrc/bvcf_stream.hip.h b/bystro-vcf_amd/csrc/bvcf_stream.hip.h
--- a/bystro-vcf_amd/csrc/bvcf_stream.hip.h
+++ b/bystro-vcf_amd/csrc/bvcf_stream.hip.h
@@ -4,12 +4,14 @@
 
 #include "bvcf_common.hip.h"
 #include "bvcf_gtscan.hip.h"
+#include "bvcf_headfast.hip.h"
 
 namespace bvcf_dev {
 
 
 constexpr uint32_t kNone = 0xFFFFFFFFu;
 constexpr uint32_t kDeferred = 0xFFFFFFFEu;
+static_assert(kDeferred == kHfDeferred, "head_fast_eval's copy");
 
 __device__ inline uint32_t find_eol(const KernelArgs &a, uint32_t from, uint32_t limit) {
   const int lane = lane_id();
@@ -403,6 +405,29 @@
 #include "bvcf_streamgen.hip.h"
 namespace bvcf_dev {
 
+struct HeadFastDeviceBytes {
+  const uint8_t *p;
+  uint32_t room;
+  __device__ __forceinline__ uint32_t byte(uint32_t rel) const { return rel < room ? p[rel] : 0u; }
+  __device__ __forceinline__ void bytes16(uint32_t rel, uint32_t out[4]) const {
+    const u32x4 v = load16(p, rel, room);
+    out[0] = v.x;
+    out[1] = v.y;
+    out[2] = v.z;
+    out[3] = v.w;
+  }
+};
+
+struct HeadFastDeviceOut {
+  u32x4 *lp, *ap;
+  __device__ __forceinline__ static void put(u32x4 *d, const uint32_t w[16]) {
+#pragma unroll
+    for (uint32_t q = 0; q < 4; q++) d[q] = u32x4{w[4 * q], w[4 * q + 1], w[4 * q + 2], w[4 * q + 3]};
+  }
+  __device__ __forceinline__ void line(const uint32_t w[16]) { put(lp, w); }
+  __device__ __forceinline__ void allele(const uint32_t w[16]) { put(ap, w); }
+};
+
 __global__ __launch_bounds__(kWgThreads) void k_order(KernelArgs a) {
   __shared__ uint32_t s_part[2][kWavesPerWg];
   __shared__ uint32_t s_first[kWgThreads + 1];
@@ -455,36 +480,70 @@
     s_first[threadIdx.x] = wbase + pre;
     if (threadIdx.x == 0) s_first[kWgThreads] = total;
     __syncthreads();
-    const uint32_t pairs = n_here * a.tile_quota;
-    for (uint32_t i = threadIdx.x; i < pairs; i += kWgThreads) {
-      const uint32_t tl = i / a.tile_quota, k = i % a.tile_quota;
-      const uint32_t first = s_first[tl];
-      const uint32_t next = tl + 1u < kWgThreads ? s_first[tl + 1u] : s_first[kWgThreads];
-      if (k >= next - first) continue;
-      const uint32_t g = base + first + k;
-      if (g >= a.max_lines) continue;
-      const size_t ei = (size_t)(c0 + tl) * a.tile_quota + k;
-      const StreamEntry en = a.entries[ei];
-      a.line_off[g] = en.ls;
-      a.line_len[g] = en.len & ~kNotRegular;
-      a.line_cmap[g] = en.cmap_off;
-      if (en.len & kHasHeadBits) {
-        const u32x4 *src = reinterpret_cast<const u32x4 *>(a.head_bits + ei * 16u);
-        u32x4 *dst = reinterpret_cast<u32x4 *>(a.line_bits + (size_t)g * 8u);
-        dst[0] = src[0];
-        dst[1] = src[1];
-      }
-      if (g < a.max_tasks) {
-        GtResult r;
-        r.ac = en.ac;
-        r.an = en.an;
-        r.n_het = en.n_het;
-        r.n_hom = en.n_hom;
-        r.n_miss = en.n_miss;
-        r.n_fields = en.n_miss == kDeferred ? kDeferred : a.n_header - 9u;
-        r.regular = (en.n_miss == kDeferred || (en.len & kNotRegular)) ? 0u : 1u;
-        r.pad = 0;
-        a.results[g] = r;
+    const uint32_t n_round = s_first[kWgThreads];
+    for (uint32_t j0 = 0; j0 < n_round; j0 += kWgThreads) {
+      const uint32_t j = j0 + threadIdx.x;
+      const uint32_t g = base + j;
+      const bool live = j < n_round && g < a.max_lines;
+      bool left = false;
+      if (live) {
+        uint32_t lo = 0;
+#pragma unroll
+        for (uint32_t s = kWgThreads / 2u; s >= 1u; s >>= 1)
+          if (s_first[lo + s] <= j) lo += s;
+        const uint32_t tl = lo, k = j - s_first[lo];
+        const size_t ei = (size_t)(c0 + tl) * a.tile_quota + k;
+        const u32x4 *ep = reinterpret_cast<const u32x4 *>(a.entries + ei);
+        const u32x4 *bp = reinterpret_cast<const u32x4 *>(a.head_bits + ei * 16u);
+        const u32x4 e0 = ep[0], e1 = ep[1];
+        const u32x4 b0 = bp[0], b1 = bp[1];
+        StreamEntry en;
+        en.ls = e0.x;
+        en.len = e0.y;
+        en.ac = e0.z;
+        en.an = e0.w;
+        en.n_het = e1.x;
+        en.n_hom = e1.y;
+        en.n_miss = e1.z;
+        en.cmap_off = e1.w;
+        if (g < a.max_tasks) {
+          GtResult r;
+          r.ac = en.ac;
+          r.an = en.an;
+          r.n_het = en.n_het;
+          r.n_hom = en.n_hom;
+          r.n_miss = en.n_miss;
+          r.n_fields = en.n_miss == kDeferred ? kDeferred : a.n_header - 9u;
+          r.regular = (en.n_miss == kDeferred || (en.len & kNotRegular)) ? 0u : 1u;
+          r.pad = 0;
+          a.results[g] = r;
+        }
+        int verdict = kHeadFastDecline;
+        if (a.head_fast && (en.len & kHasHeadBits) && g < a.max_alleles && g < a.max_tasks) {
+          const uint32_t bits[8] = {b0.x, b0.y, b0.z, b0.w, b1.x, b1.y, b1.z, b1.w};
+          const HeadFastDeviceBytes head = {a.buf + en.ls, a.cap - min(a.cap, en.ls)};
+          HeadFastDeviceOut out = {reinterpret_cast<u32x4 *>(a.lines + g), reinterpret_cast<u32x4 *>(a.alleles + g)};
+          verdict = head_fast_eval(en, bits, head, g, a.n_header, a.filters, out);
+          if (verdict == kHeadFastFilterFail) a.alleles[g].gt_task = kHfNoTask;
+        }
+        if (verdict == kHeadFastDecline) {
+          left = true;
+          a.line_off[g] = en.ls;
+          a.line_len[g] = en.len & ~kNotRegular;
+          a.line_cmap[g] = en.cmap_off;
+          if (en.len & kHasHeadBits) {
+            u32x4 *dst = reinterpret_cast<u32x4 *>(a.line_bits + (size_t)g * 8u);
+            dst[0] = bp[0];
+            dst[1] = bp[1];
+          }
+        }
+      }
+      const unsigned long long lm = __ballot(left);
+      if (lm) {
+        uint32_t at = 0;
+        if (lane == 0) at = atomicAdd(&a.counters->n_left, (uint32_t)__popcll(lm));
+        at = bcast0(at) + __builtin_amdgcn_mbcnt_hi((uint32_t)(lm >> 32), __builtin_amdgcn_mbcnt_lo((uint32_t)lm, 0u));
+        if (left) a.left_lines[at] = g;
       }
     }
     base += s_first[kWgThreads];
diff --git a/include/bvcf_bench.h b/include/bvcf_bench.h
--- a/include/bvcf_bench.h
+++ b/include/bvcf_bench.h
@@ -14,6 +14,8 @@
 
 int bvcf_bench_stream_kernel(const bvcf_ctx *ctx);
 
+long bvcf_bench_head_left(const bvcf_ctx *ctx);
+
 #ifdef __cplusplus
 }
 #endif
diff --git a/include/bvcf_plan.h b/include/bvcf_plan.h
--- a/include/bvcf_plan.h
+++ b/include/bvcf_plan.h
@@ -3,6 +3,8 @@
 
 #include <stddef.h>
 #include <stdint.h>
+
+#include "bvcf.h"
 
 #ifdef __cplusplus
 extern "C" {
@@ -61,6 +63,10 @@
 int bvcf_plan_fd(int fd_in, int fd_err, uint32_t n_workers, uint64_t max_batch_bytes, int device_inflate,
                  bvcf_plan_block *out, size_t cap, size_t *n_out, int *mode_out, bvcf_range_plan *plan_out);
 
+int bvcf_head_fast_line(const uint8_t *head, uint32_t head_bytes, uint32_t ls, uint32_t len_flags, const uint32_t counts[5],
+                        uint32_t cmap_off, const uint32_t tab_bits[8], uint32_t line, uint32_t n_header, const char *allow_filter,
+                        const char *exclude_filter, bvcf_line *out_line, bvcf_allele *out_allele);
+
 #ifdef __cplusplus
 }
 #endif
```

Result: faster. 501.1 million variants/s, median of 6 (+2.4%).
